# Luka140/paig_reproduction

Measured on AMD Instinct MI355X. Metric: video-seqs/sec (train step) spring_color B=100 @ 1/2/4/8 MI355X, higher is better.
Workload: dtype fp32; 1 GPU; spring_color PhysicsNet train step (get_batch gather+fwd+loss+bwd+allreduce+RMSprop), B=100/rank, 32x32x3, seq_len 50 (4 in / 6 pred / 40 extrap); global_batch=100, seq_len=50, parallelism=dp1, conv_math=split, split_graph=False, optimizer_in_graph=True, byte_targets=True, dataset_seqs=800

## Files before the change

include/paig_hip.h:

```cpp
#ifndef PAIG_HIP_H
#define PAIG_HIP_H
#include <stddef.h>

#ifdef __cplusplus
extern "C" {
#endif

#define PAIG_ABI_VERSION 12
const char* paig_last_error(void);
int paig_abi_version(void);
int paig_f16_range_status(int clear);

int paig_conv2d_fwd(const float* in, long long in_fs, int in_grp, long long in_gs, float* out, long long out_fs,
                    const float* aux, long long aux_fs, const float* w, const float* bias, int F, int Cin, int Cout,
                    int H, int W, int ks, int flags, void* stream);
#define PAIG_XMAX_SLOTS 2048
int paig_conv2d_fwd_ex(const float* in, long long in_fs, int in_grp, long long in_gs, float* out, long long out_fs,
                       const float* aux, long long aux_fs, const float* w, const float* bias, int F, int Cin,
                       int Cout, int H, int W, int ks, int flags, float* xmax, int xmax_n, void* stream);
int paig_conv2d_fwd_pw(const float* in, long long in_fs, int in_grp, long long in_gs, float* out, long long out_fs,
                       const float* aux, long long aux_fs, const float* w, const float* bias, int F, int Cin,
                       int Cout, int H, int W, int ks, int flags, float* xmax, int xmax_n, float* pool_out,
                       long long pool_fs, const void* wprep, void* stream);
int paig_conv2d_fwd_pwc(const float* in, long long in_fs, int in_grp, long long in_gs, float* out, long long out_fs,
                        const float* aux, long long aux_fs, const float* w, const float* bias, int F, int Cin,
                        int Cout, int H, int W, int ks, int flags, float* xmax, int xmax_n, float* pool_out,
                        long long pool_fs, unsigned char* pool_code, long long pool_code_fs, const void* wprep,
                        void* stream);
long long paig_conv_wprep_size(int cin, int cout, int ks);
int paig_conv_wprep(int n, const float* const* w, const int* cin, const int* cout, const int* ks, const int* dg,
                    void* const* out, void* stream);
int paig_conv_wprep_defer(int n, const float* const* w, const int* cin, const int* cout, const int* ks, const int* dg,
                          void* const* out, void* stream);
int paig_conv_wprep_flush(void* stream);
int paig_debug_fwd_block_cap(int cap);
int paig_conv2d_mfma_supported(int what, int Cin, int Cout, int H, int W, int ks, int flags);
int paig_conv2d_wgrad(const float* x, long long x_fs, int x_grp, long long x_gs, const float* dy, long long dy_fs,
                      float* slab, int nblk_max, int* nblk_out, int F, int Cin, int Cout, int H, int W, int ks,
                      int flags, void* stream);
int paig_conv2d_wgrad_ex(const float* x, long long x_fs, int x_grp, long long x_gs, const float* dy, long long dy_fs,
                         float* slab, int nblk_max, int* nblk_out, int F, int Cin, int Cout, int H, int W, int ks,
                         int flags, const float* xmax, int xmax_n, void* stream);
int paig_conv2d_bwd_supported(int Cin, int Cout, int H, int W, int ks, int flags);
int paig_conv2d_bwd(const float* x, long long x_fs, int x_grp, long long x_gs, const float* dy, long long dy_fs,
                    float* dx, long long dx_fs, const float* aux, long long aux_fs, const float* w, float* slab,
                    int nblk_max, int* nblk_out, int F, int Cin, int Cout, int H, int W, int ks, int flags,
                    const float* xmax, int xmax_n, const float* dpool, long long dpool_fs,
                    const unsigned char* pcode, long long pcode_fs, const void* wprep, void* stream);

size_t paig_unet_workspace(int net, int F, int H, int K, int math);
int paig_unet_fwd(int net, int F, int H, int K, int math, const float* x, long long x_fs, int x_grp, long long x_gs,
                  const float* const* w, const float* const* b, float* logits, void* ws, size_t ws_bytes,
                  void* stream);
int paig_unet_bwd(int net, int F, int H, int K, int math, const float* x, long long x_fs, int x_grp, long long x_gs,
                  const float* const* w, const float* logits, const float* dlogits, float* const* dwb, void* ws,
                  size_t ws_bytes, void* stream);
#define PAIG_UNET_HEAD_FUSED 1
#define PAIG_UNET_SEPARATE_BWD 2
#define PAIG_UNET_INFERENCE 4
#define PAIG_UNET_EXT_WPREP 8
#define PAIG_UNET_STANDALONE_UP 16
#define PAIG_UNET_STANDALONE_POOL 32
#define PAIG_PROBE_CONV_FWD 0
#define PAIG_PROBE_CONV_BWD 1
#define PAIG_PROBE_CONV_WGRAD 2
#define PAIG_PROBE_CONV_DGRAD 3
typedef void (*paig_unet_probe_fn)(void* ctx, int event, int op, int conv, int kind, int cin, int cout, int H,
                                   int flags);
size_t paig_unet_workspace_ex(int net, int F, int H, int K, int math, int flags);
long long paig_unet_buffer(int net, int F, int H, int K, int math, int flags, int which, int buf);
int paig_unet_query(int net, int K, int what);
int paig_unet_fwd_ex(int net, int F, int H, int K, int math, int flags, const float* x, long long x_fs, int x_grp,
                     long long x_gs, const float* const* w, const float* const* b, float* logits,
                     const void* const* wprep_fwd, const void* const* wprep_dg, void* ws, size_t ws_bytes,
                     paig_unet_probe_fn probe, void* probe_ctx, void* stream);
int paig_unet_bwd_ex(int net, int F, int H, int K, int math, int flags, const float* x, long long x_fs, int x_grp,
                     long long x_gs, const float* const* w, const float* logits, const float* dlogits,
                     float* const* dwb, int n_extra, const float* const* extra_src, const int* extra_nblk,
                     const int* extra_len, float* const* extra_dst, const void* const* wprep_dg, void* ws,
                     size_t ws_bytes, paig_unet_probe_fn probe, void* probe_ctx, void* stream);

int paig_conv2d_wgrad_pf(const float* x, long long x_fs, int x_grp, long long x_gs, const float* dy, long long dy_fs,
                         const float* dpool, long long dpool_fs, const unsigned char* pcode, long long pcode_fs,
                         float* slab, int nblk_max, int* nblk_out, int F, int Cin, int Cout, int H, int W, int ks,
                         int flags, const float* xmax, int xmax_n, void* stream);

int paig_maxpool2_fwd(const float* x, long long x_fs, float* y, long long y_fs, int F, int C, int H, int W,
                      void* stream);
int paig_maxpool2_fwd_codes(const float* x, long long x_fs, float* y, long long y_fs, unsigned char* code,
                            long long code_fs, int F, int C, int H, int W, void* stream);
int paig_maxpool2_bwd_relu(const float* x, long long x_fs, const float* dy, long long dy_fs, float* dx, long long dx_fs,
                           int F, int C, int H, int W, void* stream);
int paig_upsample2_fwd(const float* s, long long s_fs, float* u, long long u_fs, int F, int C, int Hs, int Ws, int Ho,
                       int Wo, void* stream);
int paig_upsample2_bwd(const float* du, long long du_fs, const float* s, long long s_fs, float* ds, long long ds_fs,
                       int F, int C, int Hs, int Ws, int Ho, int Wo, int relu_mask, void* stream);

int paig_mask_softmax_fwd(const float* logits, const float* x, long long x_fs, int x_grp, long long x_gs, float* masks,
                          float* objs, float* pobjs, int F, int K, int C, int H, int W, void* stream);
int paig_mask_softmax_bwd(const float* logits, const float* x, long long x_fs, int x_grp, long long x_gs,
                          const float* masks, const float* dobjs, float* dlogits, int F, int K, int C, int H, int W,
                          int flags, void* stream);
int paig_head_mask_blocks(int F, int H, int W);
int paig_head_mask_fwd(const float* x12, const float* w, const float* b, const float* x, long long x_fs, int x_grp,
                       long long x_gs, float* masks, float* objs, int F, int K, int H, int W, void* stream);
int paig_head_mask_bwd(const float* x12, const float* w, const float* b, const float* x, long long x_fs, int x_grp,
                       long long x_gs, const float* masks, const float* dobjs, float* dx12, float* slab, int F, int K,
                       int H, int W, void* stream);
int paig_head_mask_fwd_ex(const float* xl, const float* w, const float* b, const float* x, long long x_fs, int x_grp,
                          long long x_gs, float* masks, float* objs, float* pobjs, int F, int K, int CI, int H, int W,
                          int flags, void* stream);
int paig_head_mask_bwd_ex(const float* xl, const float* w, const float* b, const float* x, long long x_fs, int x_grp,
                          long long x_gs, const float* masks, const float* dobjs, float* dxl, float* slab, int F, int K,
                          int CI, int H, int W, int flags, void* stream);
int paig_pos_head_fwd(const float* h3, float* pos, int N, int K, float half, void* stream);
int paig_pos_head_bwd(const float* h3, const float* dpos, float* dh3, int N, int K, float half, void* stream);

size_t paig_gemm_workspace(int M, int N, int K);
int paig_gemm_defer_epilogue(int on);
int paig_gemm_flush(void* stream);
int paig_gemm(int ta, int tb, int M, int N, int K, float alpha, const float* A, long long lda, const float* B,
              long long ldb, float beta, float* C, long long ldc, const float* bias, int act, int auxm,
              const float* aux, long long ldaux, float* rowsum, float* ws, size_t ws_floats, void* stream);
int paig_gemm_ex(int ta, int tb, int M, int N, int K, float alpha, const float* A, long long lda, const float* B,
                 long long ldb, float beta, float* C, long long ldc, const float* bias, int act, int auxm,
                 const float* aux, long long ldaux, float* rowsum, float* ws, size_t ws_floats, int math,
                 void* stream);
size_t paig_gemm_parts_size(int M, int N, int K, int math);
int paig_gemm_parts(int ta, int tb, int M, int N, int K, const float* A, long long lda, const float* B,
                    long long ldb, float* part, size_t part_floats, int math, void* stream);
size_t paig_colsum_workspace(int M, int N);
int paig_colsum(const float* X, int M, int N, long long ld, float* out, int accumulate, float* ws, void* stream);
int paig_slab_reduce(const float* slab, int nblk, long long ld, int len, float* out, int accumulate, void* stream);
int paig_slab_reduce_multi(int ntask, const float* const* src, const int* nblk, const int* len, float* const* dst,
                           int accumulate, void* stream);
int paig_axpby(const float* x, float* y, long long n, float a, float b, void* stream);

int paig_vfn_fwd(const float* W1, const float* b1, const float* W2, const float* b2, float* hout, float* y,
                 float* ypost, int P, void* stream);
int paig_vfn_bwd_blocks(int P);
int paig_vfn_bwd(const float* d, const float* y, int sig, const float* h, const float* W2, float* dW1, float* db1,
                 float* dW2, float* db2, float* part, int P, void* stream);
int paig_vfn_fwd_multi(int n, const float* const* W1, const float* const* b1, const float* const* W2,
                       const float* const* b2, float* const* hout, float* const* y, float* const* ypost, const int* P,
                       void* stream);
int paig_vfn_bwd_multi(int n, const float* const* d, const float* const* y, const int* sig, const float* const* h,
                       const float* const* W2, float* const* dW1, float* const* db1, float* const* dW2,
                       float* const* db2, float* const* part, const int* P, void* stream);
int paig_vfn_bwd1_multi(int n, const float* const* d, const float* const* y, const int* sig, const float* const* h,
                        const float* const* W2, float* const* dW1, float* const* db1, float* const* dW2,
                        float* const* db2, float* const* part, const int* P, void* stream);

int paig_velmlp_fwd(const float* pos, int B, int Te, int K, int S, const float* W0, const float* b0, const float* W2,
                    const float* b2, const float* W4, const float* b4, float* X, float* h1, float* h2, float* vel,
                    void* stream);
int paig_velmlp_vfn_fwd(const float* pos, int B, int Te, int K, int S, const float* W0, const float* b0,
                        const float* W2, const float* b2, const float* W4, const float* b4, float* X, float* h1,
                        float* h2, float* vel, int n, const float* const* vW1, const float* const* vb1,
                        const float* const* vW2, const float* const* vb2, float* const* hout, float* const* y,
                        float* const* ypost, const int* P, void* stream);
int paig_velmlp_bwd_blocks(int rows);
int paig_velmlp_slab_len(int S);
int paig_velmlp_bwd(const float* dvel, const float* X, const float* h1, const float* h2, const float* W0,
                    const float* W2, const float* W4, float* dX, float* slab, int rows, int S, void* stream);

int paig_head_fwd(const float* h2, const float* W3, const float* b3, float* h3, float* pos, int F, int K, int IN,
                  float half, void* stream);
int paig_head_bwd_blocks(int rows);
int paig_head_bwd(const float* h2, const float* h3, const float* dpos, const float* W3, float* dh2, float* slab, int F,
                  int K, int IN, float half, void* stream);
int paig_head_bwd_vel(const float* h2, const float* h3, const float* dpos, const float* W3, float* dh2, float* slab,
                      int F, int K, int IN, float half, const float* dX, const float* dpos0, int B, int Te, int S,
                      int alt, void* stream);
int paig_head_bwd_vel_vfn2(const float* h2, const float* h3, const float* dpos, const float* W3, float* dh2,
                           float* slab, int F, int K, int IN, float half, const float* dX, const float* dpos0, int B,
                           int Te, int S, int alt, int n, const float* const* d, const float* const* y,
                           const int* sig, const float* const* h, const float* const* W2, float* const* dW1,
                           float* const* db1, float* const* dW2, float* const* db2, float* const* part, const int* P,
                           void* stream);

int paig_dense_tail_fwd(const float* part, int S, const float* b1, float* h1, const float* W2, float* W2t,
                        const float* b2, float* h2, const float* W3, const float* b3, float* h3, float* pos, int F,
                        int K, int IN, float half, void* stream);
int paig_head_l2_bwd_blocks(int rows);
int paig_head_l2_bwd(const float* h2, const float* h3, const float* dpos, const float* W3, float* dh2, float* slab,
                     int F, int K, int IN, float half, const float* dX, const float* dpos0, int B, int Te, int S,
                     int alt, const float* W2, const float* h1, float* dh1, int n, const float* const* d,
                     const float* const* y, const int* sig, const float* const* h, const float* const* vW2,
                     float* const* dW1, float* const* db1, float* const* dW2, float* const* db2, float* const* part,
                     const int* P, void* stream);

size_t paig_localiser_workspace(int F, int K, int n1, int IN, int math);
int paig_localiser_fwd(const float* x1, const float* W1, const float* b1, const float* W2, const float* b2,
                       const float* W3, const float* b3, float* h1, float* h2, float* h3, float* pos, int F, int K,
                       int n1, int IN, float half, int math, void* ws, size_t ws_bytes, void* stream);
int paig_localiser_bwd(const float* dpos, const float* x1, const float* h1, const float* h2, const float* h3,
                       const float* W1, const float* W2, const float* W3, float* dl1, float* dl2, float* dl3,
                       float* dx1, int F, int K, int n1, int IN, float half, int math, void* ws, size_t ws_bytes,
                       void* stream);
int paig_velmlp_rollout_fwd(int cell, const float* pos, int B, int Te, int K, int S, const float* W0, const float* b0,
                            const float* W2, const float* b2, const float* W4, const float* b4, float* X, float* h1,
                            float* h2, float* vel0, const float* dt, const double* p0, const double* p1, float* pvs,
                            int R, void* stream);
size_t paig_velmlp_rollout_bwd_workspace(int B, int K, int S);
int paig_velmlp_rollout_bwd(int cell, const float* pvs, const float* dpos_roll, const float* dpvs, const float* dt,
                            const double* p0, const double* p1, const float* X, const float* h1, const float* h2,
                            const float* W0, const float* W2, const float* W4, float* dpos, float* dmlp,
                            double* gparam0, double* gparam1, int B, int Te, int K, int S, int R, void* ws,
                            size_t ws_bytes, void* stream);

int paig_vel_pack(const float* pos, float* X, int B, int Te, int K, int S, int alt, void* stream);
int paig_vel_unpack_add(const float* dX, const float* dpos0, float* dpos, int B, int Te, int K, int S, int alt,
                        void* stream);

int paig_rollout_fwd(int cell, const float* pos0, long long pos0_ld, const float* vel0, const float* dt,
                     const double* p0, const double* p1, float* pvs, int B, int D, int R, void* stream);
int paig_rollout_bwd_blocks(int B);
int paig_rollout_bwd(int cell, const float* pvs, const float* dpos_roll, const float* dpvs, const float* dt,
                     const double* p0, const double* p1, float* dpos0, float* dvel0, double* part, double* gparam0,
                     double* gparam1, int accumulate, int B, int D, int R, void* stream);

int paig_decoder_fwd(const float* pos, long long pos_outer, long long pos_inner, int pos_grp, const float* tmpl,
                     const float* cont, const float* bg, float* out, long long out_fs, const float* tgt,
                     long long tgt_fs, int tgt_grp, long long tgt_gs, float* sse, int F, int K, int h, int H,
                     void* stream);
int paig_decoder_fwd_rollout(int cell, const float* pos0, long long pos0_ld, const float* vel0, const float* dt,
                             const double* p0, const double* p1, float* pvs, int B, int D, int R, const float* pos,
                             long long pos_outer, long long pos_inner, int pos_grp, const float* tmpl,
                             const float* cont, const float* bg, float* out, long long out_fs, const float* tgt,
                             long long tgt_fs, int tgt_grp, long long tgt_gs, float* sse, int F, int K, int h, int H,
                             void* stream);
int paig_decoder_fwd_t8(const float* pos, long long pos_outer, long long pos_inner, int pos_grp, const float* tmpl,
                        const float* cont, const float* bg, float* out, long long out_fs, const unsigned char* tgt,
                        const long long* tgt_idx, long long tgt_fs, int tgt_grp, long long tgt_gs, float* sse, int F,
                        int K, int h, int H, void* stream);
int paig_decoder_bwd_blocks(int F, int pos_grp, int live, int K, int h, int H);
size_t paig_decoder_slab_len(int K, int h, int H);
size_t paig_decoder_bwd_scratch(int F, int K, int h, int H);
int paig_decoder_bwd(const float* pos, long long pos_outer, long long pos_inner, int pos_grp, const float* tmpl,
                     const float* cont, const float* bg, const float* tgt, long long tgt_fs, int tgt_grp,
                     long long tgt_gs, const float* dsse, const float* dout, long long dout_fs, float* dpos,
                     float* slab, float* scratch, int F, int live, int K, int h, int H, void* stream);
int paig_decoder_bwd_ex(const float* pos, long long pos_outer, long long pos_inner, int pos_grp, const float* tmpl,
                        const float* cont, const float* bg, const float* tgt, const unsigned char* tgt8,
                        const long long* tgt_idx, long long tgt_fs, int tgt_grp, long long tgt_gs, const float* dsse,
                        int lw_mode, const float* dt, const float* de, const float* dr, float ae, int lB, int lTe,
                        int lR, int lpred, const float* dout, long long dout_fs, float* dpos, float* slab,
                        float* scratch, int F, int live, int K, int h, int H, void* stream);
int paig_decoder_bwd_t8(const float* pos, long long pos_outer, long long pos_inner, int pos_grp, const float* tmpl,
                        const float* cont, const float* bg, const unsigned char* tgt, const long long* tgt_idx,
                        long long tgt_fs, int tgt_grp, long long tgt_gs, const float* dsse, const float* dout,
                        long long dout_fs, float* dpos, float* slab, float* scratch, int F, int live, int K, int h,
                        int H, void* stream);

int paig_decoder_fwd_sigma(const float* pos, long long pos_outer, long long pos_inner, int pos_grp, const float* tmpl,
                           const float* cont, const float* bg, float* out, long long out_fs, const float* tgt,
                           long long tgt_fs, int tgt_grp, long long tgt_gs, float* sse, int F, int K, int h, int H,
                           double sigma, void* stream);
int paig_decoder_fwd_rollout_sigma(int cell, const float* pos0, long long pos0_ld, const float* vel0, const float* dt,
                                   const double* p0, const double* p1, float* pvs, int B, int D, int R,
                                   const float* pos, long long pos_outer, long long pos_inner, int pos_grp,
                                   const float* tmpl, const float* cont, const float* bg, float* out, long long out_fs,
                                   const float* tgt, long long tgt_fs, int tgt_grp, long long tgt_gs, float* sse, int F,
                                   int K, int h, int H, double sigma, void* stream);
int paig_decoder_fwd_t8_sigma(const float* pos, long long pos_outer, long long pos_inner, int pos_grp,
                              const float* tmpl, const float* cont, const float* bg, float* out, long long out_fs,
                              const unsigned char* tgt, const long long* tgt_idx, long long tgt_fs, int tgt_grp,
                              long long tgt_gs, float* sse, int F, int K, int h, int H, double sigma, void* stream);
int paig_decoder_bwd_blocks_sigma(int F, int pos_grp, int live, int K, int h, int H, double sigma);
size_t paig_decoder_bwd_scratch_sigma(int F, int K, int h, int H, double sigma);
int paig_decoder_bwd_ex_sigma(const float* pos, long long pos_outer, long long pos_inner, int pos_grp,
                              const float* tmpl, const float* cont, const float* bg, const float* tgt,
                              const unsigned char* tgt8, const long long* tgt_idx, long long tgt_fs, int tgt_grp,
                              long long tgt_gs, const float* dsse, int lw_mode, const float* dt, const float* de,
                              const float* dr, float ae, int lB, int lTe, int lR, int lpred, const float* dout,
                              long long dout_fs, float* dpos, float* slab, float* scratch, int F, int live, int K,
                              int h, int H, double sigma, void* stream);
int paig_decoder_parts_sigma(const float* pos, long long pos_inner, const float* tmpl, const float* cont,
                             const float* bg, float* contents, float* masks, int F, int K, int h, int H, double sigma,
                             void* stream);

int paig_sigma_from_u(const float* u, double* sigma_dev, void* stream);
int paig_sigma_grad(const double* dsig_a, int na, const double* dsig_b, int nb, const float* u, float* gu,
                    int accumulate, void* stream);
int paig_decoder_fwd_sigma_dev(const float* pos, long long pos_outer, long long pos_inner, int pos_grp,
                               const float* tmpl, const float* cont, const float* bg, float* out, long long out_fs,
                               const float* tgt, long long tgt_fs, int tgt_grp, long long tgt_gs, float* sse, int F,
                               int K, int h, int H, const double* sigma_dev, void* stream);
int paig_decoder_fwd_rollout_sigma_dev(int cell, const float* pos0, long long pos0_ld, const float* vel0,
                                       const float* dt, const double* p0, const double* p1, float* pvs, int B, int D,
                                       int R, const float* pos, long long pos_outer, long long pos_inner, int pos_grp,
                                       const float* tmpl, const float* cont, const float* bg, float* out,
                                       long long out_fs, const float* tgt, long long tgt_fs, int tgt_grp,
                                       long long tgt_gs, float* sse, int F, int K, int h, int H,
                                       const double* sigma_dev, void* stream);
int paig_decoder_fwd_t8_sigma_dev(const float* pos, long long pos_outer, long long pos_inner, int pos_grp,
                                  const float* tmpl, const float* cont, const float* bg, float* out, long long out_fs,
                                  const unsigned char* tgt, const long long* tgt_idx, long long tgt_fs, int tgt_grp,
                                  long long tgt_gs, float* sse, int F, int K, int h, int H, const double* sigma_dev,
                                  void* stream);
int paig_decoder_bwd_blocks_sigma_dev(int F, int K, int h, int H);
size_t paig_decoder_bwd_scratch_sigma_dev(int F, int K, int h, int H);
int paig_decoder_bwd_ex_sigma_dev(const float* pos, long long pos_outer, long long pos_inner, int pos_grp,
                                  const float* tmpl, const float* cont, const float* bg, const float* tgt,
                                  const unsigned char* tgt8, const long long* tgt_idx, long long tgt_fs, int tgt_grp,
                                  long long tgt_gs, const float* dsse, int lw_mode, const float* dt, const float* de,
                                  const float* dr, float ae, int lB, int lTe, int lR, int lpred, const float* dout,
                                  long long dout_fs, float* dpos, float* slab, float* scratch, int F, int live, int K,
                                  int h, int H, const double* sigma_dev, double* dsig, void* stream);
int paig_decoder_parts_sigma_dev(const float* pos, long long pos_inner, const float* tmpl, const float* cont,
                                 const float* bg, float* contents, float* masks, int F, int K, int h, int H,
                                 const double* sigma_dev, void* stream);

int paig_decoder_parts(const float* pos, long long pos_inner, const float* tmpl, const float* cont, const float* bg,
                       float* contents, float* masks, int F, int K, int h, int H, void* stream);
int paig_stn_fwd(const float* U, const float* theta, float* out, int N, int C, int Hi, int Wi, int Ho, int Wo,
                 void* stream);
int paig_stn_bwd(const float* U, const float* theta, const float* dout, float* dU, float* dtheta, int N, int C,
                 int Hi, int Wi, int Ho, int Wo, void* stream);
int paig_stn_fwd_f64(const float* U, const double* theta, float* out, int N, int C, int Hi, int Wi, int Ho, int Wo,
                     void* stream);
int paig_stn_bwd_f64(const float* U, const double* theta, const float* dout, float* dU, double* dtheta, int N, int C,
                     int Hi, int Wi, int Ho, int Wo, void* stream);
int paig_relu_mask(const float* y, float* d, long long n, void* stream);

int paig_loss_reduce(const float* sse_rec, const float* sse_roll, int B, int Te, int R, int pred, float ae,
                     float* pred_out, float* extrap_out, float* recons_out, void* stream);
int paig_loss_bwd(const float* dpred, const float* dext, const float* drec, float ae, float* wrec, float* wroll, int B,
                  int Te, int R, int pred, void* stream);
int paig_frame_sse(const float* a, long long a_fs, int a_grp, long long a_gs, const float* b, long long b_fs, int b_grp,
                   long long b_gs, float* sse, int F, int n, void* stream);
int paig_frame_sse_bwd(const float* a, long long a_fs, int a_grp, long long a_gs, const float* b, long long b_fs,
                       int b_grp, long long b_gs, const float* w, float* da, int F, int n, void* stream);

int paig_gather_u8_f32(const unsigned char* src, const long long* idx, float* out, int B, long long row, void* stream);
int paig_gather_u8_f32_ex(const unsigned char* src, const long long* idx, float* out, int B, long long row,
                          long long head, long long* idx_out, void* stream);

int paig_synth_integrate(int phys, const double* p0, const double* v0, long long m, int K, int T, int sub, double dt,
                         double size, double radius, double c0, double c1, double* pos, int* valid, void* stream);
int paig_synth_raster(const double* pos, const long long* rows, long long n, int T, int K, int size, double radius,
                      const float* bg, unsigned char* out, void* stream);
int paig_synth_raster_ex(const double* pos, const long long* rows, long long m, long long n, int T, int K, int size,
                         double radius, const float* bg, unsigned char* out, void* stream);
int paig_synth_draw(int phys, long long seed, long long stream_id, long long round, long long m, int K, int half,
                    double size, double radius, double c0, double c1, double vmax, double* p0, double* v0, double* u,
                    void* stream);
int paig_synth_background(long long seed, long long stream_id, long long round, long long n, int size, float* bg,
                          void* stream);
int paig_synth_compact(const int* valid, long long m, long long* rows, long long n, int* count, long long* totals,
                       void* stream);

int paig_rmsprop_f32(float* p, const float* g, float* sa, long long n, float lr, float alpha, float eps, void* stream);
int paig_rmsprop_mixed(float* p32, const float* g32, float* s32, long long n32, double* p64, const double* g64,
                       double* s64, long long n64, double lr, double alpha, double eps, void* stream);
int paig_rmsprop_f64(double* p, const double* g, double* sa, long long n, double lr, double alpha, double eps,
                     void* stream);
int paig_adam_f32(float* p, const float* g, float* m, float* v, long long n, float lr, float b1, float b2, float eps,
                  float bc1, float bc2sqrt, void* stream);
int paig_adam_f64(double* p, const double* g, double* m, double* v, long long n, double lr, double b1, double b2,
                  double eps, double bc1, double bc2sqrt, void* stream);
int paig_sgd_f32(float* p, const float* g, float* buf, long long n, float lr, float mom, int first, void* stream);
int paig_sgd_f64(double* p, const double* g, double* buf, long long n, double lr, double mom, int first, void* stream);

#define PAIG_GN_COLS 5
#define PAIG_GN_GROUPS 8
#define PAIG_GN_NORM 0
#define PAIG_GN_COEF 1
#define PAIG_GN_NONFINITE 2
#define PAIG_GN_TOTAL_SQ 3
#define PAIG_GN_GROUP0 4
#define PAIG_GN_SQ0 12
#define PAIG_GN_MAX_SEGMENTS 4096
int paig_grad_norm_chunk(void);
size_t paig_grad_norm_scratch(long long nchunks);
int paig_grad_norm(const float* g32, long long n32, const double* g64, long long n64, const long long* seg, int nseg,
                   long long nchunks, const unsigned char* mask, double max_norm, double* stats, void* scratch,
                   size_t scratch_bytes, void* stream);
int paig_rmsprop_mixed_clip(float* p32, const float* g32, float* s32, long long n32, double* p64, const double* g64,
                            double* s64, long long n64, double lr, double lr64, double alpha, double eps,
                            const double* coef, void* stream);
int paig_adam_f32_clip(float* p, const float* g, float* m, float* v, long long n, float lr, float b1, float b2,
                       float eps, float bc1, float bc2sqrt, const double* coef, void* stream);
int paig_adam_f64_clip(double* p, const double* g, double* m, double* v, long long n, double lr, double b1, double b2,
                       double eps, double bc1, double bc2sqrt, const double* coef, void* stream);
int paig_sgd_f32_clip(float* p, const float* g, float* buf, long long n, float lr, float mom, int first,
                      const double* coef, void* stream);
int paig_sgd_f64_clip(double* p, const double* g, double* buf, long long n, double lr, double mom, int first,
                      const double* coef, void* stream);

#ifdef __cplusplus
}
#endif
#endif
```

paig_reproduction_amd/_lib.py:

```python
import ctypes
import os

import torch

_HERE = os.path.dirname(os.path.abspath(__file__))
LIB_PATH = os.path.join(_HERE, "libpaig_hip.so")
XMAX_SLOTS = 2048

AB_PATH = os.environ.get("PAIG_AB_LIB")
ABI_VERSION = 12

P = ctypes.c_void_p
I = ctypes.c_int
LL = ctypes.c_longlong
F32 = ctypes.c_float
F64 = ctypes.c_double
SZ = ctypes.c_size_t

SIGNATURES = {
    "paig_last_error": (ctypes.c_char_p, []),
    "paig_abi_version": (I, []),
    "paig_f16_range_status": (I, [I]),
    "paig_conv2d_fwd": (I, [P, LL, I, LL, P, LL, P, LL, P, P, I, I, I, I, I, I, I, P]),
    "paig_conv2d_wgrad": (I, [P, LL, I, LL, P, LL, P, I, P, I, I, I, I, I, I, I, P]),
    "paig_conv2d_fwd_ex": (I, [P, LL, I, LL, P, LL, P, LL, P, P, I, I, I, I, I, I, I, P, I, P]),
    "paig_conv2d_fwd_pw": (I, [P, LL, I, LL, P, LL, P, LL, P, P, I, I, I, I, I, I, I, P, I, P, LL, P, P]),
    "paig_conv_wprep_size": (LL, [I, I, I]),
    "paig_conv_wprep": (I, [I, P, P, P, P, P, P, P]),
    "paig_conv_wprep_defer": (I, [I, P, P, P, P, P, P, P]),
    "paig_conv_wprep_flush": (I, [P]),
    "paig_conv2d_wgrad_ex": (I, [P, LL, I, LL, P, LL, P, I, P, I, I, I, I, I, I, I, P, I, P]),
    "paig_conv2d_wgrad_pf": (I, [P, LL, I, LL, P, LL, P, LL, P, LL, P, I, P, I, I, I, I, I, I, I, P, I, P]),
    "paig_conv2d_mfma_supported": (I, [I, I, I, I, I, I, I]),
    "paig_debug_fwd_block_cap": (I, [I]),
    "paig_conv2d_bwd_supported": (I, [I, I, I, I, I, I]),
    "paig_conv2d_bwd": (I, [P, LL, I, LL, P, LL, P, LL, P, LL, P, P, I, P, I, I, I, I, I, I, I, P, I, P, LL, P, LL,
                            P, P]),
    "paig_conv2d_fwd_pwc": (I, [P, LL, I, LL, P, LL, P, LL, P, P, I, I, I, I, I, I, I, P, I, P, LL, P, LL, P, P]),
    "paig_gather_u8_f32": (I, [P, P, P, I, LL, P]),
    "paig_gather_u8_f32_ex": (I, [P, P, P, I, LL, LL, P, P]),
    "paig_velmlp_fwd": (I, [P, I, I, I, I, P, P, P, P, P, P, P, P, P, P, P]),
    "paig_velmlp_vfn_fwd": (I, [P, I, I, I, I, P, P, P, P, P, P, P, P, P, P, I, P, P, P, P, P, P, P, P, P]),
    "paig_velmlp_bwd_blocks": (I, [I]),
    "paig_velmlp_slab_len": (I, [I]),
    "paig_velmlp_bwd": (I, [P, P, P, P, P, P, P, P, P, I, I, P]),
    "paig_head_fwd": (I, [P, P, P, P, P, I, I, I, F32, P]),
    "paig_dense_tail_fwd": (I, [P, I, P, P, P, P, P, P, P, P, P, P, I, I, I, F32, P]),
    "paig_head_l2_bwd": (I, [P, P, P, P, P, P, I, I, I, F32, P, P, I, I, I, I, P, P, P, I, P, P, P, P, P, P, P, P, P,
                             P, P, P]),
    "paig_head_bwd_blocks": (I, [I]),
    "paig_head_l2_bwd_blocks": (I, [I]),
    "paig_head_bwd": (I, [P, P, P, P, P, P, I, I, I, F32, P]),
    "paig_head_bwd_vel": (I, [P, P, P, P, P, P, I, I, I, F32, P, P, I, I, I, I, P]),
    "paig_head_bwd_vel_vfn2": (I, [P, P, P, P, P, P, I, I, I, F32, P, P, I, I, I, I, I, P, P, P, P, P, P, P, P, P, P, P,
                                   P]),
    "paig_unet_workspace": (SZ, [I, I, I, I, I]),
    "paig_localiser_workspace": (SZ, [I, I, I, I, I]),
    "paig_localiser_fwd": (I, [P, P, P, P, P, P, P, P, P, P, P, I, I, I, I, F32, I, P, SZ, P]),
    "paig_localiser_bwd": (I, [P, P, P, P, P, P, P, P, P, P, P, P, I, I, I, I, F32, I, P, SZ, P]),
    "paig_velmlp_rollout_fwd": (I, [I, P, I, I, I, I, P, P, P, P, P, P, P, P, P, P, P, P, P, P, I, P]),
    "paig_velmlp_rollout_bwd_workspace": (SZ, [I, I, I]),
    "paig_velmlp_rollout_bwd": (I, [I, P, P, P, P, P, P, P, P, P, P, P, P, P, P, P, P, I, I, I, I, I, P, SZ, P]),
    "paig_unet_fwd": (I, [I, I, I, I, I, P, LL, I, LL, P, P, P, P, SZ, P]),
    "paig_unet_bwd": (I, [I, I, I, I, I, P, LL, I, LL, P, P, P, P, P, SZ, P]),
    "paig_unet_workspace_ex": (SZ, [I, I, I, I, I, I]),
    "paig_unet_buffer": (LL, [I, I, I, I, I, I, I, I]),
    "paig_unet_query": (I, [I, I, I]),
    "paig_unet_fwd_ex": (I, [I, I, I, I, I, I, P, LL, I, LL, P, P, P, P, P, P, SZ, P, P, P]),
    "paig_unet_bwd_ex": (I, [I, I, I, I, I, I, P, LL, I, LL, P, P, P, P, I, P, P, P, P, P, P, SZ, P, P, P]),
    "paig_maxpool2_fwd": (I, [P, LL, P, LL, I, I, I, I, P]),
    "paig_maxpool2_fwd_codes": (I, [P, LL, P, LL, P, LL, I, I, I, I, P]),
    "paig_maxpool2_bwd_relu": (I, [P, LL, P, LL, P, LL, I, I, I, I, P]),
    "paig_upsample2_fwd": (I, [P, LL, P, LL, I, I, I, I, I, I, P]),
    "paig_upsample2_bwd": (I, [P, LL, P, LL, P, LL, I, I, I, I, I, I, I, P]),
    "paig_mask_softmax_fwd": (I, [P, P, LL, I, LL, P, P, P, I, I, I, I, I, P]),
    "paig_mask_softmax_bwd": (I, [P, P, LL, I, LL, P, P, P, I, I, I, I, I, I, P]),
    "paig_head_mask_blocks": (I, [I, I, I]),
    "paig_head_mask_fwd": (I, [P, P, P, P, LL, I, LL, P, P, I, I, I, I, P]),
    "paig_head_mask_bwd": (I, [P, P, P, P, LL, I, LL, P, P, P, P, I, I, I, I, P]),
    "paig_head_mask_fwd_ex": (I, [P, P, P, P, LL, I, LL, P, P, P, I, I, I, I, I, I, P]),
    "paig_head_mask_bwd_ex": (I, [P, P, P, P, LL, I, LL, P, P, P, P, I, I, I, I, I, I, P]),
    "paig_pos_head_fwd": (I, [P, P, I, I, F32, P]),
    "paig_pos_head_bwd": (I, [P, P, P, I, I, F32, P]),
    "paig_gemm_workspace": (SZ, [I, I, I]),
    "paig_gemm_parts_size": (SZ, [I, I, I, I]),
    "paig_gemm_parts": (I, [I, I, I, I, I, P, LL, P, LL, P, SZ, I, P]),
    "paig_gemm_defer_epilogue": (I, [I]),
    "paig_gemm_flush": (I, [P]),
    "paig_gemm": (I, [I, I, I, I, I, F32, P, LL, P, LL, F32, P, LL, P, I, I, P, LL, P, P, SZ, P]),
    "paig_gemm_ex": (I, [I, I, I, I, I, F32, P, LL, P, LL, F32, P, LL, P, I, I, P, LL, P, P, SZ, I, P]),
    "paig_colsum_workspace": (SZ, [I, I]),
    "paig_colsum": (I, [P, I, I, LL, P, I, P, P]),
    "paig_slab_reduce": (I, [P, I, LL, I, P, I, P]),
    "paig_slab_reduce_multi": (I, [I, P, P, P, P, I, P]),
    "paig_axpby": (I, [P, P, LL, F32, F32, P]),
    "paig_vfn_fwd": (I, [P, P, P, P, P, P, P, I, P]),
    "paig_vfn_bwd_blocks": (I, [I]),
    "paig_vfn_bwd": (I, [P, P, I, P, P, P, P, P, P, P, I, P]),
    "paig_vfn_fwd_multi": (I, [I, P, P, P, P, P, P, P, P, P]),
    "paig_vfn_bwd_multi": (I, [I, P, P, P, P, P, P, P, P, P, P, P, P]),
    "paig_vfn_bwd1_multi": (I, [I, P, P, P, P, P, P, P, P, P, P, P, P]),
    "paig_vel_pack": (I, [P, P, I, I, I, I, I, P]),
    "paig_vel_unpack_add": (I, [P, P, P, I, I, I, I, I, P]),
    "paig_rollout_fwd": (I, [I, P, LL, P, P, P, P, P, I, I, I, P]),
    "paig_rollout_bwd_blocks": (I, [I]),
    "paig_rollout_bwd": (I, [I, P, P, P, P, P, P, P, P, P, P, P, I, I, I, I, P]),
    "paig_decoder_fwd": (I, [P, LL, LL, I, P, P, P, P, LL, P, LL, I, LL, P, I, I, I, I, P]),
    "paig_decoder_fwd_rollout": (I, [I, P, LL, P, P, P, P, P, I, I, I, P, LL, LL, I, P, P, P, P, LL, P, LL, I, LL, P, I, I,
                                      I, I, P]),
    "paig_decoder_fwd_t8": (I, [P, LL, LL, I, P, P, P, P, LL, P, P, LL, I, LL, P, I, I, I, I, P]),
    "paig_decoder_bwd_blocks": (I, [I, I, I, I, I, I]),
    "paig_decoder_slab_len": (SZ, [I, I, I]),
    "paig_decoder_bwd_scratch": (SZ, [I, I, I, I]),
    "paig_decoder_bwd": (I, [P, LL, LL, I, P, P, P, P, LL, I, LL, P, P, LL, P, P, P, I, I, I, I, I, P]),
    "paig_decoder_bwd_ex": (I, [P, LL, LL, I, P, P, P, P, P, P, LL, I, LL, P, I, P, P, P, F32, I, I, I, I, P, LL, P, P, P,
                                 I, I, I, I, I, P]),
    "paig_decoder_bwd_t8": (I, [P, LL, LL, I, P, P, P, P, P, LL, I, LL, P, P, LL, P, P, P, I, I, I, I, I, P]),
    "paig_decoder_parts": (I, [P, LL, P, P, P, P, P, I, I, I, I, P]),
    "paig_decoder_fwd_sigma": (I, [P, LL, LL, I, P, P, P, P, LL, P, LL, I, LL, P, I, I, I, I, F64, P]),
    "paig_decoder_fwd_rollout_sigma": (I, [I, P, LL, P, P, P, P, P, I, I, I, P, LL, LL, I, P, P, P, P, LL, P, LL, I, LL,
                                            P, I, I, I, I, F64, P]),
    "paig_decoder_fwd_t8_sigma": (I, [P, LL, LL, I, P, P, P, P, LL, P, P, LL, I, LL, P, I, I, I, I, F64, P]),
    "paig_decoder_bwd_blocks_sigma": (I, [I, I, I, I, I, I, F64]),
    "paig_decoder_bwd_scratch_sigma": (SZ, [I, I, I, I, F64]),
    "paig_decoder_bwd_ex_sigma": (I, [P, LL, LL, I, P, P, P, P, P, P, LL, I, LL, P, I, P, P, P, F32, I, I, I, I, P, LL, P,
                                       P, P, I, I, I, I, I, F64, P]),
    "paig_decoder_parts_sigma": (I, [P, LL, P, P, P, P, P, I, I, I, I, F64, P]),
    "paig_sigma_from_u": (I, [P, P, P]),
    "paig_sigma_grad": (I, [P, I, P, I, P, P, I, P]),
    "paig_decoder_fwd_sigma_dev": (I, [P, LL, LL, I, P, P, P, P, LL, P, LL, I, LL, P, I, I, I, I, P, P]),
    "paig_decoder_fwd_rollout_sigma_dev": (I, [I, P, LL, P, P, P, P, P, I, I, I, P, LL, LL, I, P, P, P, P, LL, P, LL, I,
                                                LL, P, I, I, I, I, P, P]),
    "paig_decoder_fwd_t8_sigma_dev": (I, [P, LL, LL, I, P, P, P, P, LL, P, P, LL, I, LL, P, I, I, I, I, P, P]),
    "paig_decoder_bwd_blocks_sigma_dev": (I, [I, I, I, I]),
    "paig_decoder_bwd_scratch_sigma_dev": (SZ, [I, I, I, I]),
    "paig_decoder_bwd_ex_sigma_dev": (I, [P, LL, LL, I, P, P, P, P, P, P, LL, I, LL, P, I, P, P, P, F32, I, I, I, I, P,
                                           LL, P, P, P, I, I, I, I, I, P, P, P]),
    "paig_decoder_parts_sigma_dev": (I, [P, LL, P, P, P, P, P, I, I, I, I, P, P]),
    "paig_stn_fwd": (I, [P, P, P, I, I, I, I, I, I, P]),
    "paig_stn_bwd": (I, [P, P, P, P, P, I, I, I, I, I, I, P]),
    "paig_stn_fwd_f64": (I, [P, P, P, I, I, I, I, I, I, P]),
    "paig_stn_bwd_f64": (I, [P, P, P, P, P, I, I, I, I, I, I, P]),
    "paig_relu_mask": (I, [P, P, LL, P]),
    "paig_loss_reduce": (I, [P, P, I, I, I, I, F32, P, P, P, P]),
    "paig_loss_bwd": (I, [P, P, P, F32, P, P, I, I, I, I, P]),
    "paig_frame_sse": (I, [P, LL, I, LL, P, LL, I, LL, P, I, I, P]),
    "paig_frame_sse_bwd": (I, [P, LL, I, LL, P, LL, I, LL, P, P, I, I, P]),
    "paig_synth_integrate": (I, [I, P, P, LL, I, I, I, F64, F64, F64, F64, F64, P, P, P]),
    "paig_synth_raster": (I, [P, P, LL, I, I, I, F64, P, P, P]),
    "paig_synth_raster_ex": (I, [P, P, LL, LL, I, I, I, F64, P, P, P]),
    "paig_synth_draw": (I, [I, LL, LL, LL, LL, I, I, F64, F64, F64, F64, F64, P, P, P, P]),
    "paig_synth_background": (I, [LL, LL, LL, LL, I, P, P]),
    "paig_synth_compact": (I, [P, LL, P, LL, P, P, P]),
    "paig_rmsprop_f32": (I, [P, P, P, LL, F32, F32, F32, P]),
    "paig_rmsprop_f64": (I, [P, P, P, LL, F64, F64, F64, P]),
    "paig_rmsprop_mixed": (I, [P, P, P, LL, P, P, P, LL, F64, F64, F64, P]),
    "paig_adam_f32": (I, [P, P, P, P, LL, F32, F32, F32, F32, F32, F32, P]),
    "paig_adam_f64": (I, [P, P, P, P, LL, F64, F64, F64, F64, F64, F64, P]),
    "paig_sgd_f32": (I, [P, P, P, LL, F32, F32, I, P]),
    "paig_sgd_f64": (I, [P, P, P, LL, F64, F64, I, P]),
    "paig_grad_norm_chunk": (I, []),
    "paig_grad_norm_scratch": (SZ, [LL]),
    "paig_grad_norm": (I, [P, LL, P, LL, P, I, LL, P, F64, P, P, SZ, P]),
    "paig_rmsprop_mixed_clip": (I, [P, P, P, LL, P, P, P, LL, F64, F64, F64, F64, P, P]),
    "paig_adam_f32_clip": (I, [P, P, P, P, LL, F32, F32, F32, F32, F32, F32, P, P]),
    "paig_adam_f64_clip": (I, [P, P, P, P, LL, F64, F64, F64, F64, F64, F64, P, P]),
    "paig_sgd_f32_clip": (I, [P, P, P, LL, F32, F32, I, P, P]),
    "paig_sgd_f64_clip": (I, [P, P, P, LL, F64, F64, I, P, P]),
}

GN_COLS, GN_GROUPS = 5, 8
GN_NORM, GN_COEF, GN_NONFINITE, GN_TOTAL_SQ, GN_GROUP0, GN_SQ0 = 0, 1, 2, 3, 4, 12

_QUERY = {"paig_last_error", "paig_abi_version", "paig_f16_range_status", "paig_conv2d_mfma_supported",
          "paig_debug_fwd_block_cap",
          "paig_conv2d_bwd_supported", "paig_velmlp_bwd_blocks",
          "paig_velmlp_slab_len", "paig_head_bwd_blocks", "paig_head_l2_bwd_blocks", "paig_head_mask_blocks", "paig_conv_wprep_size", "paig_gemm_workspace", "paig_colsum_workspace",
          "paig_gemm_parts_size", "paig_gemm_parts", "paig_unet_workspace", "paig_unet_workspace_ex",
          "paig_unet_buffer", "paig_unet_query", "paig_localiser_workspace",
          "paig_velmlp_rollout_bwd_workspace",
          "paig_vfn_bwd_blocks", "paig_rollout_bwd_blocks", "paig_decoder_bwd_blocks", "paig_decoder_slab_len",
          "paig_decoder_bwd_scratch", "paig_decoder_bwd_blocks_sigma", "paig_decoder_bwd_scratch_sigma",
          "paig_decoder_bwd_blocks_sigma_dev", "paig_decoder_bwd_scratch_sigma_dev",
          "paig_grad_norm_chunk", "paig_grad_norm_scratch"}


class PaigError(RuntimeError):
    pass


class _Lib:
    def __init__(self, path=LIB_PATH):
        if not os.path.exists(path):
            raise PaigError(f"libpaig_hip.so not built at {path}: run `make -C paig_reproduction_amd/csrc` "
                            "(or __graft_entry__.build()); there is no CPU fallback")
        self.path = path
        self.dll = ctypes.CDLL(path)
        self.dll.paig_abi_version.restype = I
        self.dll.paig_abi_version.argtypes = []
        ver = self.dll.paig_abi_version()
        if ver != ABI_VERSION:
            raise PaigError(f"{path}: C ABI version {ver}, this binding is version {ABI_VERSION}")
        self.fns = {}
        for name, (rt, args) in SIGNATURES.items():
            if path != LIB_PATH and not hasattr(self.dll, name):
                continue
            f = getattr(self.dll, name)
            f.restype = rt
            f.argtypes = args
            self.fns[name] = f

    def __getattr__(self, name):
        fns = self.__dict__.get("fns")
        if fns is None or name not in fns:
            raise AttributeError(name)
        f = fns[name]
        if name in _QUERY:
            return f

        def call(*a):
            rc = f(*a)
            if rc != 0:
                msg = self.fns["paig_last_error"]().decode(errors="replace")
                raise PaigError(f"{name} failed (rc={rc}): {msg}")
            return rc

        call.__name__ = name
        return call


_lib = None


def lib():
    global _lib
    if _lib is None:
        _lib = _Lib(AB_PATH or LIB_PATH)
    return _lib


def ptr(t):
    return None if t is None else t.data_ptr()


def stream_handle(device=None):
    return torch.cuda.current_stream(device).cuda_stream


def require_device(t):
    if not (torch.is_tensor(t) and t.is_cuda):
        raise PaigError("paig_reproduction_amd runs only on a HIP device (MI355X); got a "
                        f"{'CPU' if torch.is_tensor(t) else type(t).__name__} tensor. There is no CPU fallback.")
```

paig_reproduction_amd/csrc/conv_bwd.hip:

```cpp
#include "split_common.h"

#include <stdlib.h>

#ifndef PAIG_BWD_MINW
#define PAIG_BWD_MINW 0
#endif
#ifndef PAIG_BWD_UPS2
#define PAIG_BWD_UPS2 1
#endif
#ifndef PAIG_BWD_TPX_C10
#define PAIG_BWD_TPX_C10 0
#define PAIG_BWD_MINW_C10 0
#endif
#ifndef PAIG_BWD_PSD_EVEN_C10
#define PAIG_BWD_PSD_EVEN_C10 0
#endif
#ifndef PAIG_BWD_AUXP
#define PAIG_BWD_AUXP 1
#endif

#ifdef PAIG_BWD_STAMPS
__device__ unsigned long long paig_bwd_stamps[4096][4][13];
#define PAIG_BSTAMP(k)                                      \
  do {                                                      \
    const unsigned long long t_ = __builtin_amdgcn_s_memtime(); \
    st_acc[k] += t_ - st_last;                              \
    st_last = t_;                                           \
  } while (0)
#else
#define PAIG_BSTAMP(k) \
  do {                 \
  } while (0)
#endif

namespace {

constexpr int sbwd_lds(int CIN, int COUT, int H, int W, bool UPS, int PM, int tpx) {
  const int FPT = H * W <= tpx ? tpx / (H * W) : 1, RT = H * W <= tpx ? H : rows_fit(H, W, tpx);
  const bool pe = PAIG_BWD_PSD_EVEN_C10 && UPS && CIN == 16 && COUT == 16 && H == 32;
  const int ROWS = RT + 2, ROWSD = ROWS + (UPS ? 2 : 0), CCD = rup(COUT, 8) / 8,
            PSD = CCD % 2 == 0 && !pe ? CCD + 1 : CCD;
  const int RPD = W == 8 ? to_mod16((W + 2) * PSD, 8) : (W + 2) * PSD;
  const int IMGD = (FPT * ROWSD * RPD + 2) * 8, WIMG = ceil_div(9 * CCD, 4) * ceil_div(CIN, 16) * 64 * 8;
  const int XIMG = rup(CIN, 4) / 4 * rup(FPT * ROWS * (W + 4) * 4 + 80, 128) * 2 * (PM == 2 ? 1 : 2);
  const int UPB = UPS ? CIN * (rup(FPT * (RT + 2) * W, 64) + 4) * 4 : 0;
  const int XREG = XIMG > UPB ? XIMG : UPB;
  return (IMGD + WIMG) * 2 * (PM == 2 ? 1 : 2) + XREG + (UPS ? up_window_floats(CIN, FPT, RT, W) * 4 : 0);
}
constexpr int sbwd_tpx(int CIN, int COUT, int H, int W, bool UPS, int PM) {
  if (PAIG_BWD_TPX_C10 && UPS && CIN == 16 && COUT == 16 && H == 32) return PAIG_BWD_TPX_C10;
  for (int pass = 0; pass < 2; ++pass)
    for (int t = 256; t >= 64; t /= 2) {
      const int rt = H * W <= t ? H : rows_fit(H, W, t);
      if (UPS && (rt % 2 != 0 || H * W < t)) continue;
      if (sbwd_lds(CIN, COUT, H, W, UPS, PM, t) <= (pass == 0 ? LDS_MAX / 2 : LDS_MAX)) return t;
    }
  return 64;
}

constexpr int sbwd_minw(int CIN, int COUT, int H, int PM, bool PF) {
  if (PAIG_BWD_MINW_C10 && CIN == 16 && COUT == 16 && H == 32) return PAIG_BWD_MINW_C10;
  if (CIN == 8 && COUT == 8 && H == 32) return PF || PAIG_BWD_AUXP == 2 ? 3 : 4;
  if (PM == 2 && CIN == 8 && COUT == 16 && H == 16) return 3;
  if (PM == 2 && CIN == 24 && COUT == 8 && H == 32) return 3;
  if (CIN == 8 && COUT == 8 && H == 36) return PF ? 2 : 3;
  if (CIN == 8 && COUT == 16 && H == 18) return PM == 2 ? 4 : 3;
  if (CIN == 16 && COUT == 16 && H == 18) return PF && PM != 2 ? 2 : 3;
  return 2;
}

constexpr bool sbwd_auxp(int CIN, int COUT, int H, int PM, bool UPS, bool PF) {
  if (PAIG_BWD_AUXP == 2) return true;
  if (CIN == 8 && COUT == 8 && (H == 32 || H == 36) && !PF) return false;
  if (CIN == 24 && COUT == 8 && (H == 36 || PM == 2)) return false;
  if (UPS && H == 36) return false;
  if (PM == 0) return !(PF && CIN == 16 && COUT == 16 && H == 16);
  return !((UPS && CIN == 32 && H == 16) || (CIN == 8 && COUT == 16 && H == 16));
}

constexpr bool sbwd_hoist(int CIN, int COUT, int H, int PM, bool PF) {
  if (PF && PM == 0 && ((CIN == 8 && H == 32) || H == 64)) return false;
  if (PF && PM == 2 && H == 18) return false;
  if (CIN == 24 && H == 36 && PM == 0) return false;
  if (H == 18 && ((CIN == 8 && PM == 2) || (CIN == 16 && COUT == 16 && PM == 0))) return false;
  return true;
}

template <int CIN, int COUT, int H, int W, int KS, bool UPS, int PM, bool PF = false>
struct SBwdCfg {
  static constexpr int KK = KS * KS, PADL = KS / 2;
  static constexpr int NIMG = PM == 2 ? 1 : 2;
  static constexpr int TPX = sbwd_tpx(CIN, COUT, H, W, UPS, PM);
  static constexpr int FPT = H * W <= TPX ? TPX / (H * W) : 1;
  static constexpr int RT = H * W <= TPX ? H : rows_fit(H, W, TPX);
  static constexpr int TPXV = FPT * RT * W;
  static constexpr int ROWS = RT + KS - 1;
  static constexpr int EXT = UPS ? 1 : 0;
  static constexpr int RTD = RT + 2 * EXT, ROWSD = ROWS + 2 * EXT;
  static constexpr int TPXD = FPT * RTD * W;
  static constexpr int CCD = rup(COUT, 8) / 8;
  static constexpr bool PSDE = PAIG_BWD_PSD_EVEN_C10 && UPS && CIN == 16 && COUT == 16 && H == 32;
  static constexpr int PSD = CCD % 2 == 0 && !PSDE ? CCD + 1 : CCD;
  static constexpr int TWPX = W + 2 * PADL;
  static constexpr int RPD = W == 8 ? to_mod16(TWPX * PSD, 8) : TWPX * PSD;
  static constexpr int ZSLOT = FPT * ROWSD * RPD;
  static constexpr int IMGD = (ZSLOT + 2) * 8;
  static constexpr int KC = KK * CCD, NS = ceil_div(KC, 4);
  static constexpr int NTD = ceil_div(CIN, 16);
  static constexpr int NMT = ceil_div(TPXD, 16), MW = ceil_div(NMT, 4);
  static constexpr int WIMG = NS * NTD * 64 * 8;
  static constexpr int CQ = rup(CIN, 4) / 4, NQ = KK * CQ, NTX = ceil_div(NQ, 4);
  static constexpr int OFFX = PADL > 0 ? 2 : 0, TWX = W + 2 * OFFX;
  static constexpr int XPL = rup(FPT * ROWS * TWX * 4 + 80, 128);
  static constexpr int XIMG = CQ * XPL;
  static constexpr int MT = ceil_div(COUT, 16), NTW = ceil_div(NTX, 4);
  static constexpr bool BAL = !(PM == 2 && (CIN == 24 || (UPS && CIN == 32) || H == 36 || H == 18)) && !(H == 36 && !UPS && !PF);
  static constexpr int NTF = BAL ? NTX / 4 : ceil_div(NTX, 4), NTR = BAL ? NTX % 4 : 0;
  static constexpr int KB = ceil_div(TPXV, 32);
  static constexpr int NCOL = CIN * KK, SLAB = COUT * NCOL + COUT;
  static constexpr int UPX = W % 2 == 0 ? 2 : 1, W2 = W / UPX;
  static constexpr int NID = FPT * ROWSD * W2 * CCD, NLD = ceil_div(NID, 256);
  static constexpr int NIX = FPT * ROWS * W2 * CQ, NLX = ceil_div(NIX, 256);
  static constexpr int UPW = up_window_floats(CIN, FPT, RT, W);
  static constexpr int UPB = UPS ? CIN * (rup(FPT * (RT + 2) * W, 64) + 4) * 4 : 0;
  static constexpr int XREG = XIMG * 2 * NIMG > UPB ? XIMG * 2 * NIMG : UPB;
  static constexpr int LDS = (IMGD + WIMG) * 2 * NIMG + XREG + (UPS ? UPW * 4 : 0);
  static constexpr bool VEC4 = W % 4 == 0;
  static constexpr bool HOIST = sbwd_hoist(CIN, COUT, H, PM, PF);
  static constexpr bool XPIPE = !UPS && NLX * 8 <= 32;
  static constexpr int LDSB = LDS_MAX / (LDS > (NLD * 256 * 8 + 256) * 4 ? LDS : (NLD * 256 * 8 + 256) * 4);
  static constexpr int MW0 = PAIG_BWD_MINW > 0 ? PAIG_BWD_MINW : sbwd_minw(CIN, COUT, H, PM, PF);
  static constexpr int MINW = MW0 < LDSB ? MW0 : LDSB;
  static_assert(H % RT == 0, "RT divides H");
  static_assert(KS == 3, "3x3 layers (the 1x1 heads are fused elsewhere)");
  static_assert(COUT % 8 == 0 && CIN % 4 == 0, "staging units of 8 dY / 4 X channels");
  static_assert(!UPS || (FPT == 1 && RT % 2 == 0 && W % 2 == 0), "fused upsample: whole even row blocks of one frame");
  static_assert(!PF || (!UPS && UPX == 2 && COUT % 8 == 0 && H % 2 == 0), "pool fold: even widths, 8-channel chunks");
  static constexpr int UPP = rup(TPXD, 64) + 4;
  static_assert(!UPS || CIN * UPP * 4 <= XREG, "fused upsample: dX tile does not fit the X region");
  static constexpr int WSU = W / 2, IKU = WSU % 4 == 0 ? 4 : (WSU % 2 == 0 ? 2 : 1), WQU = WSU / IKU;
  static constexpr int NOU = UPS ? CIN * (RT / 2) * WQU : 0, NOI = NOU > 0 ? ceil_div(NOU, 256) : 1;
  static constexpr bool AUXP =
      PAIG_BWD_AUXP && (UPS || (VEC4 && MW * NTD <= 8)) && sbwd_auxp(CIN, COUT, H, PM, UPS, PF);
};

template <int CIN, int COUT, int H, int W, int KS, bool UPS, int PM, bool PF>
__global__ void __launch_bounds__(256, (SBwdCfg<CIN, COUT, H, W, KS, UPS, PM, PF>::MINW))
conv_bwd_split_k(FView x, FView dy, FViewW dx, FView aux, const float* __restrict__ w, int flags,
                 float* __restrict__ slab, int F, int ntiles, XMax xm, const s16x8* __restrict__ wp, FView dpool,
                 const unsigned char* __restrict__ pcode, long long pcode_fs) {
  using C = SBwdCfg<CIN, COUT, H, W, KS, UPS, PM, PF>;
  constexpr int KK = C::KK, PADL = C::PADL, RT = C::RT, FPT = C::FPT, ROWS = C::ROWS, TPXV = C::TPXV;
  constexpr int EXT = C::EXT, RTD = C::RTD, ROWSD = C::ROWSD, TPXD = C::TPXD;
  constexpr int CCD = C::CCD, PSD = C::PSD, RPD = C::RPD, KC = C::KC, NS = C::NS, NTD = C::NTD, MW = C::MW;
  constexpr int CQ = C::CQ, NQ = C::NQ, NTX = C::NTX, OFFX = C::OFFX, TWX = C::TWX, XPL = C::XPL;
  constexpr int MT = C::MT, NTF = C::NTF, NTR = C::NTR, KB = C::KB, NCOL = C::NCOL, UPX = C::UPX, W2 = C::W2;
  constexpr int NF1 = NTF > 0 ? NTF : 1, NR1 = NTR > 0 ? NTR : 1;
  constexpr int NID = C::NID, NLD = C::NLD, NIX = C::NIX, NLX = C::NLX;
  constexpr long long HW = (long long)H * W;
  constexpr long long XPLANE = UPS ? (long long)(H / 2) * (W / 2) : HW;
  constexpr int NRB = H / RT;
  extern __shared__ __attribute__((aligned(16))) short lds16[];
  short* Dh = lds16;
  short* Dl = Dh + (C::NIMG == 2 ? C::IMGD : 0);
  short* Wh = lds16 + C::NIMG * C::IMGD;
  short* Wl = Wh + (C::NIMG == 2 ? C::WIMG : 0);
  short* Xh = lds16 + C::NIMG * (C::IMGD + C::WIMG);
  short* Xl = Xh + (C::NIMG == 2 ? C::XIMG : 0);
  float* Sl = reinterpret_cast<float*>(reinterpret_cast<char*>(Xh) + C::XREG);
  const int tid = threadIdx.x, lane = tid & 63, wv = tid >> 6, g = lane >> 4;
  __shared__ float smax[4];
#ifdef PAIG_BWD_STAMPS
  unsigned long long st_acc[12] = {0, 0, 0, 0, 0, 0, 0, 0, 0, 0, 0, 0}, st_last = __builtin_amdgcn_s_memtime(), st_n = 0;
#endif

  auto xplane = [](int cq) { return cq * XPL + ((cq & 1) ? 16 : 0) + ((cq & 2) ? 64 : 0); };
  for (int i = tid; i < FPT * ROWSD * 2 * PADL * CCD; i += 256) {
    const int cc = i % CCD, hc = (i / CCD) % (2 * PADL), r = i / (CCD * 2 * PADL);
    const int xc = hc < PADL ? hc : W + hc;
    const int o = (r * RPD + xc * PSD + cc) * 8;
    *reinterpret_cast<s16x8*>(Dh + o) = s16x8{0, 0, 0, 0, 0, 0, 0, 0};
    if (PM != 2) *reinterpret_cast<s16x8*>(Dl + o) = s16x8{0, 0, 0, 0, 0, 0, 0, 0};
  }
  if (tid < 2) {
    *reinterpret_cast<s16x8*>(Dh + (C::ZSLOT + tid) * 8) = s16x8{0, 0, 0, 0, 0, 0, 0, 0};
    if (PM != 2) *reinterpret_cast<s16x8*>(Dl + (C::ZSLOT + tid) * 8) = s16x8{0, 0, 0, 0, 0, 0, 0, 0};
  }
  auto zero_xhalo = [&]() {
    for (int i = tid; i < FPT * ROWS * 2 * OFFX * CQ; i += 256) {
      const int cq = i % CQ, hc = (i / CQ) % (2 * OFFX), r = i / (CQ * 2 * OFFX);
      const int xc = hc < OFFX ? hc : W + hc;
      *reinterpret_cast<s16x4*>(Xh + xplane(cq) + (r * TWX + xc) * 4) = s16x4{0, 0, 0, 0};
      if (PM != 2) *reinterpret_cast<s16x4*>(Xl + xplane(cq) + (r * TWX + xc) * 4) = s16x4{0, 0, 0, 0};
    }
  };
  zero_xhalo();

  int ecx = PAIG_A_EXP, ecd = PM == 0 && PAIG_SCALE_MODE < 2 ? 100 : 0;
  float xsc = 1.f, dsc = __builtin_amdgcn_ldexpf(1.f, ecd);
  float rmax = 0.f;
  int ewn[NTD];
#pragma unroll
  for (int nt = 0; nt < NTD; ++nt) ewn[nt] = 0;

  auto wval = [&](int idx, int j) {
    const int ln = idx & 63, snt = idx >> 6, nt = snt % NTD, s = snt / NTD;
    const int kc = 4 * s + (ln >> 4), ci = nt * 16 + (ln & 15);
    float v = 0.f;
    if (kc < KC && ci < CIN) {
      const int tap = kc / CCD, co = (kc % CCD) * 8 + j;
      if (co < COUT) v = w[(co * CIN + ci) * KK + (KK - 1 - tap)];
    }
    return v;
  };
  __shared__ int sew[PM == 0 ? NTD * 16 : 1];
  if (PM == 0 && wp != nullptr) {
    const int* hdr = reinterpret_cast<const int*>(wp);
    constexpr int HDR = NTD * 16 * 4 / 16;
#pragma unroll
    for (int nt = 0; nt < NTD; ++nt) ewn[nt] = hdr[nt * 16 + (lane & 15)];
    const s16x8* img = wp + HDR;
    constexpr int WLO = NS * NTD * 64;
    for (int idx = tid; idx < NS * NTD * 64; idx += 256) {
      *reinterpret_cast<s16x8*>(Wh + idx * 8) = img[idx];
      *reinterpret_cast<s16x8*>(Wl + idx * 8) = img[WLO + idx];
    }
  } else {
    if constexpr (PM == 0) {
      for (int i = tid; i < NTD * 16; i += 256) sew[i] = 0;
      __syncthreads();
      float pm[NTD];
#pragma unroll
      for (int nt = 0; nt < NTD; ++nt) pm[nt] = 0.f;
      for (int idx = tid; idx < NS * NTD * 64; idx += 256) {
        const int nt = (idx >> 6) % NTD;
#pragma unroll
        for (int j = 0; j < 8; ++j) pm[nt] = fmaxf(pm[nt], fabsf(wval(idx, j)));
      }
#pragma unroll
      for (int nt = 0; nt < NTD; ++nt) atomicMax(&sew[nt * 16 + (tid & 15)], __builtin_bit_cast(int, pm[nt]));
      __syncthreads();
      for (int i = tid; i < NTD * 16; i += 256) sew[i] = f16_scale_exp_v(__builtin_bit_cast(float, sew[i]));
      __syncthreads();
#pragma unroll
      for (int nt = 0; nt < NTD; ++nt) ewn[nt] = sew[nt * 16 + (lane & 15)];
    }
    for (int idx = tid; idx < NS * NTD * 64; idx += 256) {
      const int cl = ((idx >> 6) % NTD) * 16 + (idx & 15);
      const int e = PM == 0 ? sew[cl] : 0;
      s16x8 vh, vl;
#pragma unroll
      for (int j = 0; j < 8; ++j) {
        short h, l;
        float rm = 0.f;
        split<PM>(__builtin_amdgcn_ldexpf(wval(idx, j), e), h, l, rm);
        vh[j] = h;
        vl[j] = l;
      }
      *reinterpret_cast<s16x8*>(Wh + idx * 8) = vh;
      if (PM != 2) *reinterpret_cast<s16x8*>(Wl + idx * 8) = vl;
    }
  }

  int pbase[MW];
#pragma unroll
  for (int mt = 0; mt < MW; ++mt) {
    int pix = (wv * MW + mt) * 16 + (lane & 15);
    if (pix >= TPXD) pix = 0;
    const int fi = pix / (RTD * W), rem = pix % (RTD * W);
    pbase[mt] = (fi * ROWSD + rem / W) * RPD + (rem % W) * PSD;
  }
  int soff[NS];
#pragma unroll
  for (int s = 0; s < NS; ++s) {
    int kc = 4 * s + g;
    if (kc >= KC) kc = 0;
    const int tap = kc / CCD, cc = kc % CCD;
    soff[s] = (tap / KS) * RPD + (tap % KS) * PSD + cc;
  }
  const int qq = (lane >> 2) & 3, pl = lane & 3;
  auto colt_of = [&](int nt) {
    int cq = nt * 4 + pl;
    if (cq >= NQ) cq = 0;
    const int tap = cq / CQ, ciq = cq % CQ;
    return xplane(ciq) + ((tap / KS) * TWX + tap % KS) * 4;
  };
  int colt[NF1], coltr[NR1];
#pragma unroll
  for (int jn = 0; jn < NTF; ++jn) colt[jn] = colt_of(wv + jn * 4);
#pragma unroll
  for (int t = 0; t < NTR; ++t) coltr[t] = colt_of(NTF * 4 + t);
  auto dslot = [&](int j) {
    if (TPXV % 32 != 0 && j >= TPXV) return C::ZSLOT;
    const int fi = j / (RT * W), rem = j % (RT * W);
    return (fi * ROWSD + rem / W + PADL + EXT) * RPD + (rem % W + PADL) * PSD;
  };
  auto xpos = [&](int j) {
    if (TPXV % 32 != 0 && j >= TPXV) j = 0;
    const int fi = j / (RT * W), rem = j % (RT * W);
    return ((fi * ROWS + rem / W) * TWX + rem % W + (OFFX - PADL)) * 4;
  };

  f32x4 accw[MT][NF1], accr[MT][NR1];
#pragma unroll
  for (int m = 0; m < MT; ++m) {
#pragma unroll
    for (int j = 0; j < NF1; ++j) accw[m][j] = f32x4{0.f, 0.f, 0.f, 0.f};
#pragma unroll
    for (int t = 0; t < NR1; ++t) accr[m][t] = f32x4{0.f, 0.f, 0.f, 0.f};
  }
  float bacc[NLD][8];
#pragma unroll
  for (int l = 0; l < NLD; ++l)
#pragma unroll
    for (int c = 0; c < 8; ++c) bacc[l][c] = 0.f;

  float2 pd[NLD][8];
  float2 px[C::XPIPE ? NLX : 1][4];
  float dpv[PF ? NLD : 1][8];
  uint2 pcv[PF ? NLD : 1];
  constexpr int HP = H / 2, WP = W / 2;
  using UP = UpStage<UPS ? CIN : 1, H, W, FPT, RT>;
  UP up;
  auto row_ok = [&](int gy) { return (unsigned)gy < (unsigned)H; };
  auto d_unit = [&](int i, int& vo, int& row, int& so) {
    const int xp = UPX * (i % W2), r = (i / W2) % ROWSD, cc = (i / (W2 * ROWSD)) % CCD, fi = i / (W2 * ROWSD * CCD);
#ifdef PAIG_BWD_NOLOAD
    const bool in = false;
#else
    const bool in = i < NID;
#endif
    row = in ? r - PADL - EXT : -(1 << 20);
    vo = (fi * (int)dy.fs + cc * 8 * (int)HW + (r - PADL - EXT) * W + xp) * 4;
    if (NRB == 1 && !row_ok(row)) vo = BUF_OOR;
    so = ((fi * ROWSD + r) * RPD + (xp + PADL) * PSD + cc) * 8;
  };
  constexpr int NLH = C::HOIST ? NLD : 1;
  int dvo[NLH], drow[NLH], dso[NLH];
  if constexpr (C::HOIST) {
#pragma unroll
    for (int l = 0; l < NLD; ++l) d_unit(tid + l * 256, dvo[l], drow[l], dso[l]);
  }
  auto d_get = [&](int l, int& vo, int& row, int& so) {
    if constexpr (C::HOIST) {
      vo = dvo[l];
      row = drow[l];
      so = dso[l];
    } else {
      d_unit(opaque(tid) + l * 256, vo, row, so);
    }
  };
  auto pf_unit = [&](int i, int& po, int& co) {
    const int xp = UPX * (i % W2), cc = (i / (W2 * ROWSD)) % CCD, fi = i / (W2 * ROWSD * CCD);
    po = (fi * (int)dpool.fs + cc * 8 * (HP * WP) + (xp >> 1)) * 4;
    co = fi * (int)pcode_fs + (cc * (HP * WP) + (xp >> 1)) * 8;
  };
  auto x_unit = [&](int i, int& vo, int& row, int& so) {
    const int xp = UPX * (i % W2), r = (i / W2) % ROWS, cq = (i / (W2 * ROWS)) % CQ, fi = i / (W2 * ROWS * CQ);
    row = i < NIX ? r - PADL : -(1 << 20);
    vo = (fi * (int)x.fs + cq * 4 * (int)XPLANE + (r - PADL) * W + xp) * 4;
    if (NRB == 1 && !row_ok(row)) vo = BUF_OOR;
    so = xplane(cq) + ((fi * ROWS + r) * TWX + xp + OFFX) * 4;
  };
  constexpr int NXH = C::XPIPE && C::HOIST ? NLX : 1;
  int xvo[NXH], xrow[NXH], xso[NXH];
  if constexpr (C::XPIPE && C::HOIST) {
#pragma unroll
    for (int l = 0; l < NLX; ++l) x_unit(tid + l * 256, xvo[l], xrow[l], xso[l]);
  }
  auto x_get = [&](int l, int& vo, int& row, int& so) {
    if constexpr (C::HOIST) {
      vo = xvo[l];
      row = xrow[l];
      so = xso[l];
    } else {
      x_unit(opaque(tid) + l * 256, vo, row, so);
    }
  };
  int uvo[UPS ? UP::NLS : 1], urow[UPS ? UP::NLS : 1];
  if constexpr (UPS) {
#pragma unroll
    for (int l = 0; l < UP::NLS; ++l) UP::unit(tid + l * 256, (int)x.fs, uvo[l], urow[l]);
  }
  auto tile_nf = [&](int f0) {
    const int n = F - f0;
    return n < FPT ? n : FPT;
  };
  auto tile_vo = [&](int vo, int row, int y0) {
    if constexpr (NRB == 1) return vo;
    else return row_ok(y0 + row) ? vo + y0 * W * 4 : BUF_OOR;
  };
  auto load_d = [&](int t) {
    const int f0 = (t / NRB) * FPT, y0 = (t % NRB) * RT, nf = tile_nf(f0);
    const brsrc rd = tile_rsrc(dy.frame(f0), dy.fs, nf, COUT * (int)HW);
    brsrc rp, rc;
    if constexpr (PF) {
      rp = tile_rsrc(dpool.frame(f0), dpool.fs, nf, COUT * HP * WP);
      rc = tile_rsrc(pcode + (long long)f0 * pcode_fs, pcode_fs, nf, CCD * HP * WP * 8, 1);
    }
#pragma unroll
    for (int l = 0; l < NLD; ++l) {
      int vo0, row, so;
      d_get(l, vo0, row, so);
      const int vo = tile_vo(vo0, row, y0);
#pragma unroll
      for (int c = 0; c < 8; ++c) {
        pd[l][c] = UPX == 2 ? buf_ld2(rd, vo, c * (int)HW * 4) : make_float2(buf_ld1(rd, vo, c * (int)HW * 4), 0.f);
      }
      if constexpr (PF) {
        const int wr = ((y0 + row) >> 1) * WP;
        const bool ok = NRB == 1 ? vo != BUF_OOR : row_ok(y0 + row);
        int po, co;
        pf_unit(opaque(tid) + l * 256, po, co);
        const int vp = ok ? po + wr * 4 : BUF_OOR;
#pragma unroll
        for (int c = 0; c < 8; ++c) dpv[l][c] = buf_ld1(rp, vp, c * (HP * WP) * 4);
        const u32x2 cv = __builtin_amdgcn_raw_buffer_load_b64(rc, ok ? co + wr * 8 : BUF_OOR, 0, 0);
        pcv[l] = make_uint2(cv.x, cv.y);
      }
    }
  };
  auto fold = [&](int t) {
    const int y0 = (t % NRB) * RT;
#pragma unroll
    for (int l = 0; l < NLD; ++l) {
      int vo, row, so;
      d_get(l, vo, row, so);
      const int pr = ((y0 + row) & 1) * 2;
#pragma unroll
      for (int c = 0; c < 8; ++c) {
        const unsigned b = ((c < 4 ? pcv[l].x : pcv[l].y) >> (8 * (c & 3))) & 255u;
        const int am = (int)(b >> 4) & 3;
        const float vx = pd[l][c].x + (am == pr ? dpv[l][c] : 0.f);
        const float vy = pd[l][c].y + (am == pr + 1 ? dpv[l][c] : 0.f);
        pd[l][c].x = (b >> pr) & 1u ? vx : 0.f;
        pd[l][c].y = (b >> (pr + 1)) & 1u ? vy : 0.f;
      }
    }
  };
  auto x_rsrc = [&](int t) {
    const int f0 = (t / NRB) * FPT;
    return tile_rsrc(x.frame(f0), x.fs, tile_nf(f0), CIN * (int)XPLANE);
  };
  auto load_x = [&](brsrc rx, int t, int vo0, int row, float2* v) {
    const int vo = tile_vo(vo0, row, (t % NRB) * RT);
#pragma unroll
    for (int c = 0; c < 4; ++c)
      v[c] = UPX == 2 ? buf_ld2(rx, vo, c * (int)XPLANE * 4) : make_float2(buf_ld1(rx, vo, c * (int)XPLANE * 4), 0.f);
  };
  auto issue = [&](int t) {
    if (t >= ntiles) return;
    load_d(t);
    if constexpr (UPS) {
      up.issue(x_rsrc(t), (t % NRB) * RT, uvo, urow);
    } else if constexpr (C::XPIPE) {
      const brsrc rx = x_rsrc(t);
#pragma unroll
      for (int l = 0; l < NLX; ++l) {
        int vo, row, so;
        x_get(l, vo, row, so);
        load_x(rx, t, vo, row, px[l]);
      }
    }
  };
  auto put_d = [&](int o, const float2* v) {
    s16x8 h0, l0, h1, l1;
    if constexpr (PM == 0) {
      pf32x2 sv[8];
#pragma unroll
      for (int c = 0; c < 8; ++c) sv[c] = pf32x2{v[c].x, v[c].y} * dsc;
      u32x4 a0, b0, a1, b1;
#pragma unroll
      for (int k = 0; k < 4; ++k) {
        { const HiLo q_ = split_pk(sv[2 * k].x, sv[2 * k + 1].x); a0[k] = q_.h; b0[k] = q_.l; }
        { const HiLo q_ = split_pk(sv[2 * k].y, sv[2 * k + 1].y); a1[k] = q_.h; b1[k] = q_.l; }
      }
      h0 = __builtin_bit_cast(s16x8, a0);
      l0 = __builtin_bit_cast(s16x8, b0);
      h1 = __builtin_bit_cast(s16x8, a1);
      l1 = __builtin_bit_cast(s16x8, b1);
    } else {
      float rm = 0.f;
#pragma unroll
      for (int c = 0; c < 8; ++c) {
        short h, lo;
        split<PM>(v[c].x, h, lo, rm);
        h0[c] = h;
        l0[c] = lo;
        split<PM>(v[c].y, h, lo, rm);
        h1[c] = h;
        l1[c] = lo;
      }
    }
    *reinterpret_cast<s16x8*>(Dh + o) = h0;
    if (PM != 2) *reinterpret_cast<s16x8*>(Dl + o) = l0;
    if constexpr (UPX == 2) {
      *reinterpret_cast<s16x8*>(Dh + o + PSD * 8) = h1;
      if (PM != 2) *reinterpret_cast<s16x8*>(Dl + o + PSD * 8) = l1;
    }
  };
  auto put_x_at = [&](int o, const float2* v) {
    s16x8 hv, lv;
    if constexpr (PM == 0) {
      pf32x2 sv[4];
#pragma unroll
      for (int c = 0; c < 4; ++c) {
        sv[c] = pf32x2{v[c].x, v[c].y} * xsc;
        rmax = amax2(rmax, sv[c].x, sv[c].y);
      }
      u32x4 a, b;
      { const HiLo q_ = split_pk(sv[0].x, sv[1].x); a[0] = q_.h; b[0] = q_.l; }
      { const HiLo q_ = split_pk(sv[2].x, sv[3].x); a[1] = q_.h; b[1] = q_.l; }
      { const HiLo q_ = split_pk(sv[0].y, sv[1].y); a[2] = q_.h; b[2] = q_.l; }
      { const HiLo q_ = split_pk(sv[2].y, sv[3].y); a[3] = q_.h; b[3] = q_.l; }
      hv = __builtin_bit_cast(s16x8, a);
      lv = __builtin_bit_cast(s16x8, b);
    } else {
#pragma unroll
      for (int c = 0; c < 4; ++c) {
        short h, lo;
        split<PM>(v[c].x, h, lo, rmax);
        hv[c] = h;
        lv[c] = lo;
        split<PM>(v[c].y, h, lo, rmax);
        hv[4 + c] = h;
        lv[4 + c] = lo;
      }
    }
    if constexpr (UPX == 2) {
      *reinterpret_cast<s16x8*>(Xh + o) = hv;
      if (PM != 2) *reinterpret_cast<s16x8*>(Xl + o) = lv;
    } else {
      *reinterpret_cast<s16x4*>(Xh + o) = s16x4{hv[0], hv[1], hv[2], hv[3]};
      if (PM != 2) *reinterpret_cast<s16x4*>(Xl + o) = s16x4{lv[0], lv[1], lv[2], lv[3]};
    }
  };
  auto put_x = [&](int i, const float2* v) {
    const int xp = UPX * (i % W2), r = (i / W2) % ROWS, cq = (i / (W2 * ROWS)) % CQ, fi = i / (W2 * ROWS * CQ);
    put_x_at(xplane(cq) + ((fi * ROWS + r) * TWX + xp + OFFX) * 4, v);
  };
  auto tile_max = [&]() {
    float m = 0.f;
#pragma unroll
    for (int l = 0; l < NLD; ++l)
#pragma unroll
      for (int c = 0; c < 8; ++c) m = amax2(m, pd[l][c].x, pd[l][c].y);
    m = wave_max_u(m);
    if (lane == 0) smax[wv] = m;
  };
  auto commit = [&](int t) {
    if constexpr (PM == 0 && PAIG_SCALE_MODE < 2) {
      const int te = f16_scale_exp(fmaxf(fmaxf(smax[0], smax[1]), fmaxf(smax[2], smax[3])));
      const int td = te < ecd + 64 ? te : ecd + 64;
      if (td != ecd) {
#pragma unroll
        for (int m = 0; m < MT; ++m)
#pragma unroll
          for (int r = 0; r < 4; ++r) {
#pragma unroll
            for (int j = 0; j < NF1; ++j) accw[m][j][r] = __builtin_amdgcn_ldexpf(accw[m][j][r], td - ecd);
#pragma unroll
            for (int t = 0; t < NR1; ++t) accr[m][t][r] = __builtin_amdgcn_ldexpf(accr[m][t][r], td - ecd);
          }
        ecd = td;
        dsc = __builtin_amdgcn_ldexpf(1.f, ecd);
      }
    }
    const int f0 = (t / NRB) * FPT;
#pragma unroll
    for (int l = 0; l < NLD; ++l) {
      const int i = tid + l * 256;
      if (NID % 256 != 0 && i >= NID) break;
      int vo, row, so;
      d_get(l, vo, row, so);
      put_d(so, pd[l]);
      if ((unsigned)row < (unsigned)RT) {
#pragma unroll
        for (int c = 0; c < 8; ++c) bacc[l][c] += pd[l][c].x + pd[l][c].y;
      }
    }
    PAIG_BSTAMP(8);
    if constexpr (UPS) {
      const int y0 = (t % NRB) * RT;
      up.commit(Sl, tid);
      zero_xhalo();
      PAIG_BSTAMP(9);
      __syncthreads();
      PAIG_BSTAMP(10);
      if constexpr (W % 4 == 0 && ROWS % 2 == 0 && PAIG_BWD_UPS2 && PM == 0 && H != 36) {
        constexpr int W4 = W / 4, RP2 = ROWS / 2;
#pragma unroll 1
        for (int i = tid; i < CQ * RP2 * W4; i += 256) {
          const int q = i % W4, rp = (i / W4) % RP2, cq = i / (W4 * RP2);
          const int gy = y0 + 2 * rp - PADL;
          const bool ok0 = f0 < F && gy >= 0 && gy < H, ok1 = f0 < F && gy + 1 >= 0 && gy + 1 < H;
          f32x4 o0[4], o1[4];
#pragma unroll
          for (int c = 0; c < 4; ++c) {
            if (cq * 4 + c < CIN) {
              UP::row4x2(Sl, 0, cq * 4 + c, gy, y0, q, ok0, ok1, o0[c], o1[c]);
            } else {
              o0[c] = f32x4{0.f, 0.f, 0.f, 0.f};
              o1[c] = o0[c];
            }
          }
#pragma unroll
          for (int h2 = 0; h2 < 2; ++h2) {
            const int ia = (cq * ROWS + 2 * rp + h2) * W2 + 2 * q;
            const f32x4* o = h2 ? o1 : o0;
            float2 v[4];
#pragma unroll
            for (int c = 0; c < 4; ++c) v[c] = make_float2(o[c][0], o[c][1]);
            put_x(ia, v);
#pragma unroll
            for (int c = 0; c < 4; ++c) v[c] = make_float2(o[c][2], o[c][3]);
            put_x(ia + 1, v);
          }
        }
        PAIG_BSTAMP(11);
      } else if constexpr (W % 4 == 0) {
        constexpr int W4 = W / 4;
#pragma unroll 1
        for (int i = tid; i < NIX / 2; i += 256) {
#ifdef PAIG_BWD_NOUPS
          if (i >= 0) break;
#endif
          const int q = i % W4, r = (i / W4) % ROWS, cq = (i / (W4 * ROWS)) % CQ;
          const int gy = y0 + r - PADL;
          const bool ok = f0 < F && gy >= 0 && gy < H;
          f32x4 o[4];
#pragma unroll
          for (int c = 0; c < 4; ++c)
            o[c] = (ok && cq * 4 + c < CIN) ? UP::row4(Sl, 0, cq * 4 + c, gy, y0, q) : f32x4{0.f, 0.f, 0.f, 0.f};
          const int ia = (cq * ROWS + r) * W2 + 2 * q;
          float2 v[4];
#pragma unroll
          for (int c = 0; c < 4; ++c) v[c] = make_float2(o[c][0], o[c][1]);
          put_x(ia, v);
#pragma unroll
          for (int c = 0; c < 4; ++c) v[c] = make_float2(o[c][2], o[c][3]);
          put_x(ia + 1, v);
        }
        PAIG_BSTAMP(11);
      } else {
#pragma unroll 1
        for (int i = tid; i < NIX; i += 256) {
          const int xp = UPX * (i % W2), r = (i / W2) % ROWS, cq = (i / (W2 * ROWS)) % CQ;
          const int gy = y0 + r - PADL;
          const bool ok = f0 < F && gy >= 0 && gy < H;
          float2 v[4];
#pragma unroll
          for (int c = 0; c < 4; ++c)
            v[c] = (ok && cq * 4 + c < CIN)
                       ? make_float2(UP::px1(Sl, 0, cq * 4 + c, gy, y0, xp), UP::px1(Sl, 0, cq * 4 + c, gy, y0, xp + 1))
                       : make_float2(0.f, 0.f);
          put_x(i, v);
        }
      }
    } else if constexpr (C::XPIPE) {
#pragma unroll
      for (int l = 0; l < NLX; ++l) {
        const int i = tid + l * 256;
        if (NIX % 256 != 0 && i >= NIX) break;
        int vo, row, so;
        x_get(l, vo, row, so);
        put_x_at(so, px[l]);
      }
    } else {
      const brsrc rx = x_rsrc(t);
#pragma unroll 1
      for (int i = tid; i < NIX; i += 256) {
        float2 v[4];
        int vo, row, so;
        x_unit(i, vo, row, so);
        load_x(rx, t, vo, row, v);
        put_x_at(so, v);
      }
    }
  };

  int avo[C::AUXP ? (UPS ? C::NOI : MW) : 1];
  if constexpr (C::AUXP && UPS) {
#pragma unroll
    for (int k = 0; k < C::NOI; ++k) {
      const int o = tid + 256 * k;
      const int q = o % C::WQU, sr = (o / C::WQU) % (RT / 2), ci = o / (C::WQU * (RT / 2));
      avo[k] = o < C::NOU ? ((ci * (H / 2) + sr) * C::WSU + C::IKU * q) * 4 : BUF_OOR;
    }
  } else if constexpr (C::AUXP) {
#pragma unroll
    for (int mt = 0; mt < MW; ++mt) {
      const int pix = (wv * MW + mt) * 16 + (lane >> 4) * 4;
      const int fi = pix / (RT * W), rem = pix % (RT * W);
      avo[mt] = pix < TPXV ? (fi * (int)aux.fs + (lane & 15) * (int)HW + rem) * 4 : BUF_OOR;
    }
  }

  int lt = blockIdx.x;
  auto tile_of =[&](int l) { return l < ntiles ? xcd_tile(l, ntiles) : ntiles; };
  issue(tile_of(lt));
  if (PM == 0 && xm.p) {
    float m = 0.f;
    for (int i = tid * 4; i < xm.n; i += 1024) {
      const f32x4 v = *reinterpret_cast<const f32x4*>(xm.p + i);
      m = fmaxf(m, fmaxf(fmaxf(v[0], v[1]), fmaxf(v[2], v[3])));
    }
    m = wave_max_u(m);
    if (lane == 0) smax[wv] = m;
    __syncthreads();
    m = fmaxf(fmaxf(smax[0], smax[1]), fmaxf(smax[2], smax[3]));
    if (m > 0.f) ecx = f16_scale_exp(m);
    __syncthreads();
  }
  if constexpr (PM == 0) xsc = __builtin_amdgcn_ldexpf(1.f, ecx);
  else ecx = 0;

  PAIG_BSTAMP(0);
  for (; lt < ntiles; lt += gridDim.x) {
    const int tile = xcd_tile(lt, ntiles);
    const int f0 = (tile / NRB) * FPT, y0 = (tile % NRB) * RT;
    if constexpr (PF) fold(tile);
    if constexpr (PM == 0 && PAIG_SCALE_MODE < 2) tile_max();
    __syncthreads();
    PAIG_BSTAMP(1);
    commit(tile);
    __syncthreads();
    PAIG_BSTAMP(2);
    typedef float fIKU __attribute__((ext_vector_type(C::IKU)));
    f32x4 auxv[C::AUXP && !UPS ? MW : 1][C::AUXP && !UPS ? NTD : 1];
    fIKU auxu[C::AUXP && UPS ? C::NOI : 1];
    if constexpr (C::AUXP) {
      if (flags & 2) {
        const brsrc ra = tile_rsrc(aux.frame(f0), aux.fs, tile_nf(f0), CIN * (int)XPLANE);
        if constexpr (UPS) {
#pragma unroll
          for (int k = 0; k < C::NOI; ++k) {
            const int so = (y0 / 2) * C::WSU * 4;
            if constexpr (C::IKU == 4) auxu[k] = buf_ld4(ra, avo[k], so);
            else if constexpr (C::IKU == 2) auxu[k] = __builtin_bit_cast(fIKU, buf_ld2(ra, avo[k], so));
            else auxu[k] = __builtin_bit_cast(fIKU, buf_ld1(ra, avo[k], so));
          }
        } else {
#pragma unroll
          for (int nt = 0; nt < NTD; ++nt) {
            const bool cok = CIN % 16 == 0 || nt * 16 + (lane & 15) < CIN;
#pragma unroll
            for (int mt = 0; mt < MW; ++mt)
              auxv[mt][nt] = buf_ld4(ra, cok ? avo[mt] : BUF_OOR, (nt * 16 * (int)HW + y0 * W) * 4);
          }
        }
      }
    }
    issue(tile_of(lt + gridDim.x));
    PAIG_BSTAMP(3);

#pragma unroll 2
    for (int kb = 0; kb < KB; ++kb) {
      const int p0 = kb * 32;
      s16x8 ah[MT], al[MT];
      const int d0 = dslot(p0 + 8 * g + qq), d1 = dslot(p0 + 8 * g + 4 + qq);
#pragma unroll
      for (int m = 0; m < MT; ++m) {
        const int co = 2 * m + (pl >> 1), hoff = (pl & 1) * 4;
        const int a0 = (d0 + co) * 8 + hoff, a1 = (d1 + co) * 8 + hoff;
        ah[m] = __builtin_shufflevector(tr_read(Dh + a0), tr_read(Dh + a1), 0, 1, 2, 3, 4, 5, 6, 7);
        al[m] = PM != 2 ? __builtin_shufflevector(tr_read(Dl + a0), tr_read(Dl + a1), 0, 1, 2, 3, 4, 5, 6, 7) : ah[m];
      }
      const int r0 = xpos(p0 + 8 * g + qq), r1 = xpos(p0 + 8 * g + 4 + qq);
      auto ntile = [&](int ct, f32x4* acc) __attribute__((always_inline)) {
        const s16x8 bh = __builtin_shufflevector(tr_read(Xh + r0 + ct), tr_read(Xh + r1 + ct), 0, 1, 2, 3, 4, 5, 6, 7);
        const s16x8 bl =
            PM != 2 ? __builtin_shufflevector(tr_read(Xl + r0 + ct), tr_read(Xl + r1 + ct), 0, 1, 2, 3, 4, 5, 6, 7) : bh;
#pragma unroll
        for (int m = 0; m < MT; ++m) acc[m] = mma3<PM>(ah[m], al[m], bh, bl, acc[m]);
      };
#pragma unroll
      for (int jn = 0; jn < NTF; ++jn) {
        if (!C::BAL && wv + jn * 4 >= NTX) continue;
        f32x4 a[MT];
#pragma unroll
        for (int m = 0; m < MT; ++m) a[m] = accw[m][jn];
        ntile(colt[jn], a);
#pragma unroll
        for (int m = 0; m < MT; ++m) accw[m][jn] = a[m];
      }
      if (NTR > 0 && (kb & 3) == wv) {
#pragma unroll
        for (int t = 0; t < NTR; ++t) {
          f32x4 a[MT];
#pragma unroll
          for (int m = 0; m < MT; ++m) a[m] = accr[m][t];
          ntile(coltr[t], a);
#pragma unroll
          for (int m = 0; m < MT; ++m) accr[m][t] = a[m];
        }
      }
    }

    PAIG_BSTAMP(4);
    f32x4 accd[MW][NTD];
#pragma unroll
    for (int mt = 0; mt < MW; ++mt)
#pragma unroll
      for (int nt = 0; nt < NTD; ++nt) accd[mt][nt] = f32x4{0.f, 0.f, 0.f, 0.f};
#pragma unroll
    for (int s = 0; s < NS; ++s) {
      s16x8 bh[NTD], bl[NTD];
#pragma unroll
      for (int nt = 0; nt < NTD; ++nt) {
        const int o = ((s * NTD + nt) * 64 + lane) * 8;
        bh[nt] = *reinterpret_cast<const s16x8*>(Wh + o);
        bl[nt] = PM != 2 ? *reinterpret_cast<const s16x8*>(Wl + o) : bh[nt];
      }
#pragma unroll
      for (int mt = 0; mt < MW; ++mt) {
        const int o = (pbase[mt] + soff[s]) * 8;
        const s16x8 ah = *reinterpret_cast<const s16x8*>(Dh + o);
        const s16x8 al = PM != 2 ? *reinterpret_cast<const s16x8*>(Dl + o) : ah;
#pragma unroll
        for (int nt = 0; nt < NTD; ++nt) accd[mt][nt] = mma3<PM>(ah, al, bh[nt], bl[nt], accd[mt][nt]);
      }
    }
    PAIG_BSTAMP(5);
    if constexpr (UPS) {
      float* U = reinterpret_cast<float*>(Xh);
      __syncthreads();
#pragma unroll
      for (int nt = 0; nt < NTD; ++nt) {
        const int ci = nt * 16 + (lane & 15);
        if (ci >= CIN) continue;
        const float tinv = PM == 0 ? __builtin_amdgcn_ldexpf(1.f, -(ecd + ewn[nt])) : 1.f;
#pragma unroll
        for (int mt = 0; mt < MW; ++mt) {
          const int pix = (wv * MW + mt) * 16 + (lane >> 4) * 4;
          if (pix < TPXD) *reinterpret_cast<f32x4*>(U + ci * C::UPP + pix) = accd[mt][nt] * tinv;
        }
      }
      __syncthreads();
      constexpr int HS = H / 2, WS = W / 2, IK = C::IKU, WQ = C::WQU;
      constexpr int NO = C::NOU;
      static_assert(WS % IK == 0, "IK-pixel source items");
      typedef fIKU fIK;
      auto item = [&](int o, const fIK& mp) __attribute__((always_inline)) {
        const int q = o % WQ, sr = (o / WQ) % (RT / 2), ci = o / (WQ * (RT / 2));
        const int sy = y0 / 2 + sr;
        float wy[4];
        wy[0] = sy >= 1 ? 0.25f : 0.f;
        wy[1] = sy == 0 ? 1.f : 0.75f;
        wy[2] = sy == HS - 1 ? 1.f : 0.75f;
        wy[3] = sy <= HS - 2 ? 0.25f : 0.f;
        fIK acc;
#pragma unroll
        for (int k = 0; k < IK; ++k) acc[k] = 0.f;
#pragma unroll
        for (int a = 0; a < 4; ++a) {
          if (wy[a] == 0.f) continue;
          const float* rp = U + ci * C::UPP + (2 * sr + a) * W + 2 * IK * q;
          float c[2 * IK + 2];
          c[0] = q > 0 ? rp[-1] : 0.f;
          c[2 * IK + 1] = q < WQ - 1 ? rp[2 * IK] : 0.f;
          if constexpr (IK == 1) {
            c[1] = rp[0];
            c[2] = rp[1];
          } else {
#pragma unroll
            for (int h = 0; h < IK / 2; ++h) {
              const f32x4 m = *reinterpret_cast<const f32x4*>(rp + 4 * h);
#pragma unroll
              for (int e = 0; e < 4; ++e) c[1 + 4 * h + e] = m[e];
            }
          }
          fIK row;
#pragma unroll
          for (int k = 0; k < IK; ++k) {
            const int sx = IK * q + k;
            float wx[4];
            wx[0] = sx >= 1 ? 0.25f : 0.f;
            wx[1] = sx == 0 ? 1.f : 0.75f;
            wx[2] = sx == WS - 1 ? 1.f : 0.75f;
            wx[3] = sx <= WS - 2 ? 0.25f : 0.f;
            float v = 0.f;
#pragma unroll
            for (int b = 0; b < 4; ++b)
              if (wx[b] != 0.f) v = fmaf(wx[b], c[2 * k + b], v);
            row[k] = v;
          }
#pragma unroll
          for (int k = 0; k < IK; ++k) acc[k] = fmaf(wy[a], row[k], acc[k]);
        }
        if (f0 < F) {
          const long long off = ((long long)ci * HS + sy) * WS + IK * q;
          float* op = dx.frame(f0) + off;
          if (flags & 4) acc += *reinterpret_cast<const fIK*>(op);
          if (flags & 2) {
            fIK m;
            if constexpr (C::AUXP) m = mp;
            else m = *reinterpret_cast<const fIK*>(aux.frame(f0) + off);
#pragma unroll
            for (int k = 0; k < IK; ++k) acc[k] = m[k] > 0.f ? acc[k] : 0.f;
          }
          *reinterpret_cast<fIK*>(op) = acc;
        }
      };
      if constexpr (C::AUXP) {
#pragma unroll
        for (int it = 0; it < C::NOI; ++it) {
          const int o = tid + 256 * it;
          if (NO % 256 != 0 && o >= NO) break;
          item(o, auxu[it]);
        }
      } else {
        for (int o = tid; o < NO; o += 256) item(o, auxu[0]);
      }
    } else {
#pragma unroll
    for (int nt = 0; nt < NTD; ++nt) {
      const int ci = nt * 16 + (lane & 15);
      if (ci >= CIN) continue;
      const float tinv = PM == 0 ? __builtin_amdgcn_ldexpf(1.f, -(ecd + ewn[nt])) : 1.f;
#pragma unroll
      for (int mt = 0; mt < MW; ++mt) {
        const int pix = (wv * MW + mt) * 16 + (lane >> 4) * 4;
        if constexpr (C::VEC4) {
          if (pix >= TPXV) continue;
          const int fi = pix / (RT * W), rem = pix % (RT * W);
          const int y = y0 + rem / W, xx = rem % W, f = f0 + fi;
          if (f >= F) continue;
          float* op = dx.frame(f) + ci * HW + (long long)y * W + xx;
          f32x4 v = accd[mt][nt] * tinv;
          if (flags & 4) v += *reinterpret_cast<const f32x4*>(op);
          if (flags & 2) {
            f32x4 a;
            if constexpr (C::AUXP) a = auxv[mt][nt];
            else a = *reinterpret_cast<const f32x4*>(aux.frame(f) + ci * HW + (long long)y * W + xx);
#pragma unroll
            for (int r = 0; r < 4; ++r) v[r] = a[r] > 0.f ? v[r] : 0.f;
          }
          *reinterpret_cast<f32x4*>(op) = v;
        } else {
#pragma unroll
          for (int r = 0; r < 4; ++r) {
            const int pr = pix + r;
            if (pr >= TPXV) break;
            const int fi = pr / (RT * W), rem = pr % (RT * W);
            const int y = y0 + rem / W, xx = rem % W, f = f0 + fi;
            if (f >= F) continue;
            float* op = dx.frame(f) + ci * HW + (long long)y * W + xx;
            float v = accd[mt][nt][r] * tinv;
            if (flags & 4) v += *op;
            if (flags & 2) v = aux.frame(f)[ci * HW + (long long)y * W + xx] > 0.f ? v : 0.f;
            *op = v;
          }
        }
      }
    }
    }
    PAIG_BSTAMP(6);
#ifdef PAIG_BWD_STAMPS
    ++st_n;
#endif
  }

  float* s = slab + (long long)blockIdx.x * C::SLAB;
  auto put_w = [&](int m, int nt, const f32x4& acc) __attribute__((always_inline)) {
    const int col = nt * 16 + (lane & 15), cq = col >> 2;
    const int tap = cq / CQ, ci = (cq % CQ) * 4 + (col & 3);
#pragma unroll
    for (int r = 0; r < 4; ++r) {
      const int co = m * 16 + (lane >> 4) * 4 + r;
      float v = acc[r];
      if constexpr (PM == 0) v = __builtin_amdgcn_ldexpf(v, -(ecx + ecd));
      if (co < COUT && cq < NQ && ci < CIN) s[co * NCOL + ci * KK + tap] = v;
    }
  };
#pragma unroll
  for (int m = 0; m < MT; ++m)
#pragma unroll
    for (int j = 0; j < NTF; ++j)
      if (wv + j * 4 < NTX) put_w(m, wv + j * 4, accw[m][j]);
  if constexpr (NTR > 0) {
    f32x4* Rt = reinterpret_cast<f32x4*>(lds16);
    __syncthreads();
#pragma unroll
    for (int m = 0; m < MT; ++m)
#pragma unroll
      for (int t = 0; t < NTR; ++t) Rt[((wv * MT + m) * NTR + t) * 64 + lane] = accr[m][t];
    __syncthreads();
    for (int u = wv; u < MT * NTR; u += 4) {
      f32x4 v = Rt[u * 64 + lane];
#pragma unroll
      for (int w = 1; w < 4; ++w) v += Rt[(w * MT * NTR + u) * 64 + lane];
      put_w(u / NTR, NTF * 4 + u % NTR, v);
    }
  }
  __syncthreads();
  float* Rb = reinterpret_cast<float*>(lds16);
  constexpr int NP = 256 / COUT, NU = FPT * ROWSD * W2;
  float* Rp = Rb + NLD * 256 * 8;
#pragma unroll
  for (int l = 0; l < NLD; ++l)
#pragma unroll
    for (int c = 0; c < 8; ++c) Rb[(l * 256 + tid) * 8 + c] = bacc[l][c];
  __syncthreads();
  if (tid < NP * COUT) {
    const int co = tid % COUT, q = tid / COUT, cc = co / 8, c = co % 8;
    float v = 0.f;
    for (int j = q; j < NU; j += NP) {
      const int xpi = j % W2, r = (j / W2) % ROWSD, fi = j / (W2 * ROWSD);
      v += Rb[((((fi * CCD + cc) * ROWSD) + r) * W2 + xpi) * 8 + c];
    }
    Rp[co * NP + q] = v;
  }
  __syncthreads();
  if (tid < COUT) {
    float v = 0.f;
    for (int q = 0; q < NP; ++q) v += Rp[tid * NP + q];
    s[COUT * NCOL + tid] = v;
  }
  if constexpr (PM == 0) f16_range_note(rmax);
#ifdef PAIG_BWD_STAMPS
  PAIG_BSTAMP(7);
  if (lane == 0 && blockIdx.x < 4096) {
#pragma unroll
    for (int k = 0; k < 12; ++k) paig_bwd_stamps[blockIdx.x][wv][k] = st_acc[k];
    paig_bwd_stamps[blockIdx.x][wv][12] = st_n;
  }
#endif
}

template <int CIN, int COUT, int H, int W, int KS, bool UPS, int PM, bool PF = false>
static int sbwd_launch(FView x, FView dy, FViewW dx, FView aux, const float* w, int flags, float* slab, int nblk_max,
                       int* nblk_out, int F, hipStream_t st, XMax xm, const void* wp,
                       FView dpool = FView{nullptr, 0, 0, 0}, const unsigned char* pcode = nullptr,
                       long long pcode_fs = 0) {
  using C = SBwdCfg<CIN, COUT, H, W, KS, UPS, PM, PF>;
  constexpr int RED = (C::NLD * 256 * 8 + 256) * 4;
  constexpr int LDS0 = C::LDS > RED ? C::LDS : RED;
  static_assert(LDS0 <= LDS_MAX, "fused backward: staging exceeds the LDS");
  static const int lds_pad = [] {
    const char* e = getenv("PAIG_BWD_LDS_PAD");
    return e ? atoi(e) : 0;
  }();
  const int LDS = LDS0 + lds_pad <= LDS_MAX ? LDS0 + lds_pad : LDS0;
  const int ntiles = cdiv(F, C::FPT) * (H / C::RT);
  auto k = conv_bwd_split_k<CIN, COUT, H, W, KS, UPS, PM, PF>;
  static int resident = 0;
  if (!resident) {
    if (LDS > 64 * 1024) (void)hipFuncSetAttribute((const void*)k, hipFuncAttributeMaxDynamicSharedMemorySize, LDS);
    resident = persistent_grid((const void*)k, LDS);
  }
  int nb = ntiles < nblk_max ? ntiles : nblk_max;
  if (nb > resident) nb = resident;
  {
    static int mt = -1;
    if (mt < 0) {
      const char* e = getenv("PAIG_BWD_MIN_TPB");
      mt = e ? atoi(e) : 0;
    }
    if (mt > 1 && nb > cdiv(ntiles, mt)) nb = cdiv(ntiles, mt);
  }
  if (nb < 1) nb = 1;
  *nblk_out = nb;
  PAIG_REQUIRE(!xm.p || (xm.n % 4 == 0 && (reinterpret_cast<uintptr_t>(xm.p) & 15) == 0),
               "conv split bwd: xmax needs 16-byte alignment and a multiple of 4 slots (%d)", xm.n);
  PAIG_REQUIRE(!(flags & 2) || aux.p, "conv split bwd: ReLU' mask (flags & 2) without aux");
  constexpr long long SPAN = (1ll << 31) / (4 * C::FPT) - 8 * 4096;
  PAIG_REQUIRE(x.fs < SPAN && dy.fs < SPAN && aux.fs < SPAN && dpool.fs < SPAN && pcode_fs < 4 * SPAN &&
                   x.fs >= 0 && dy.fs >= 0 && aux.fs >= 0 && dpool.fs >= 0 && pcode_fs >= 0,
               "conv split bwd: a frame stride does not fit the tile's 32-bit byte offsets");
  PAIG_REQUIRE(!PF || (dpool.p && pcode && (reinterpret_cast<uintptr_t>(pcode) & 7) == 0 && pcode_fs % 8 == 0),
               "conv split bwd: pool fold needs the pooled gradient and 8-byte aligned window codes");
  hipLaunchKernelGGL(k, dim3(nb), dim3(256), LDS, st, x, dy, dx, aux, w, flags, slab, F, ntiles, xm,
                     PM == 0 ? static_cast<const s16x8*>(wp) : nullptr, dpool, pcode, pcode_fs);
  PAIG_CHECK_LAUNCH();
  return 0;
}

#define PAIG_BWD_UP_SHAPES(X) X(32, 16, 16) X(16, 16, 32) X(16, 16, 36) X(32, 16, 18)
#define PAIG_BWD_POOL_SHAPES(X) X(8, 8, 32) X(16, 16, 16) X(16, 16, 64) X(8, 8, 36) X(16, 16, 18)
#define PAIG_BWD_SHAPES(X)                                                                  \
  X(8, 8, 32) X(8, 16, 16) X(16, 16, 16) X(16, 32, 8) X(32, 32, 8) X(32, 16, 16) X(24, 8, 32) \
  X(8, 8, 36) X(8, 16, 18) X(16, 16, 18) X(32, 16, 18) X(24, 8, 36)                            \
  X(16, 16, 64) X(16, 32, 32)

}

extern "C" {

int paig_conv2d_bwd_supported(int Cin, int Cout, int H, int W, int ks, int flags) {
  if (H != W || ks != 3 || !(flags & (128 | 256))) return 0;
#define PAIG_CASE(CI, CO, HH) \
  if (Cin == CI && Cout == CO && H == HH) return 1;
  if (flags & 64) {
    if (flags & 32) return 0;
    PAIG_BWD_POOL_SHAPES(PAIG_CASE)
    return 0;
  }
  if (flags & 32) {
    PAIG_BWD_UP_SHAPES(PAIG_CASE)
    return 0;
  }
  PAIG_BWD_SHAPES(PAIG_CASE)
#undef PAIG_CASE
  return 0;
}

int paig_conv2d_bwd(const float* x, long long x_fs, int x_grp, long long x_gs, const float* dy, long long dy_fs,
                    float* dx, long long dx_fs, const float* aux, long long aux_fs, const float* w, float* slab,
                    int nblk_max, int* nblk_out, int F, int Cin, int Cout, int H, int W, int ks, int flags,
                    const float* xmax, int xmax_n, const float* dpool, long long dpool_fs,
                    const unsigned char* pcode, long long pcode_fs, const void* wprep, void* stream) {
  *nblk_out = 0;
  if (F <= 0) return 0;
  PAIG_REQUIRE(paig_conv2d_bwd_supported(Cin, Cout, H, W, ks, flags),
               "paig_conv2d_bwd: no fused kernel for Cin=%d Cout=%d H=%d W=%d ks=%d flags=%d", Cin, Cout, H, W, ks,
               flags);
  PAIG_REQUIRE(x_grp == 0 || H * W >= 256, "paig_conv2d_bwd: multi-frame tiles need a plain frame stride");
  PAIG_REQUIRE(nblk_max > 0 && slab && dx && dy && x && w, "paig_conv2d_bwd: null operand or no slab rows");
  hipStream_t st = (hipStream_t)stream;
  FView vx{x, x_fs, x_gs, x_grp}, vd{dy, dy_fs, 0, 0}, va{aux, aux_fs, 0, 0};
  FViewW vdx{dx, dx_fs};
  XMax xm{const_cast<float*>(xmax), xmax_n};
  const bool b16 = (flags & 256) != 0;
  const int fl = flags & 6;
  if (flags & 64) {
    const FView vp{dpool, dpool_fs, 0, 0};
#define PAIG_CASE(CI, CO, HH)                                                                                     \
  if (Cin == CI && Cout == CO && H == HH)                                                                         \
    return b16 ? sbwd_launch<CI, CO, HH, HH, 3, false, 2, true>(vx, vd, vdx, va, w, fl, slab, nblk_max, nblk_out,  \
                                                                 F, st, xm, wprep, vp, pcode, pcode_fs)            \
               : sbwd_launch<CI, CO, HH, HH, 3, false, 0, true>(vx, vd, vdx, va, w, fl, slab, nblk_max, nblk_out,  \
                                                                 F, st, xm, wprep, vp, pcode, pcode_fs);
    PAIG_BWD_POOL_SHAPES(PAIG_CASE)
#undef PAIG_CASE
    return PAIG_E_UNSUPPORTED;
  }
  if (flags & 32) {
#define PAIG_CASE(CI, CO, HH)                                                                                     \
  if (Cin == CI && Cout == CO && H == HH)                                                                         \
    return b16 ? sbwd_launch<CI, CO, HH, HH, 3, true, 2>(vx, vd, vdx, va, w, fl, slab, nblk_max, nblk_out, F, st, \
                                                           xm, wprep)                                             \
               : sbwd_launch<CI, CO, HH, HH, 3, true, 0>(vx, vd, vdx, va, w, fl, slab, nblk_max, nblk_out, F, st, \
                                                           xm, wprep);
    PAIG_BWD_UP_SHAPES(PAIG_CASE)
#undef PAIG_CASE
    return PAIG_E_UNSUPPORTED;
  }
#define PAIG_CASE(CI, CO, HH)                                                                                      \
  if (Cin == CI && Cout == CO && H == HH)                                                                          \
    return b16 ? sbwd_launch<CI, CO, HH, HH, 3, false, 2>(vx, vd, vdx, va, w, fl, slab, nblk_max, nblk_out, F, st, \
                                                            xm, wprep)                                             \
               : sbwd_launch<CI, CO, HH, HH, 3, false, 0>(vx, vd, vdx, va, w, fl, slab, nblk_max, nblk_out, F, st, \
                                                            xm, wprep);
  PAIG_BWD_SHAPES(PAIG_CASE)
#undef PAIG_CASE
  return PAIG_E_UNSUPPORTED;
}

#ifdef PAIG_BWD_STAMPS
int paig_bwd_stamps_read(void* host, size_t bytes) {
  return (int)hipMemcpyFromSymbol(host, HIP_SYMBOL(paig_bwd_stamps), bytes);
}
#endif

}

PAIG_F16_RANGE_ACCESSOR(paig_f16_range_bwd)
```

paig_reproduction_amd/csrc/unet.hip:

```cpp
#include "common.h"

#include <vector>

#define UNET_HIP(call)                                                  \
  do {                                                                  \
    const hipError_t _e = (call);                                       \
    if (_e != hipSuccess) {                                             \
      paig_set_error("%s: %s", __func__, hipGetErrorString(_e));        \
      return (int)_e;                                                   \
    }                                                                   \
  } while (0)

namespace {

enum { U_CONV = 0, U_POOL = 1, U_UP = 2 };

struct Reg {
  int buf, off, n;
  bool operator==(const Reg& o) const { return buf == o.buf && off == o.off && n == o.n; }
};
struct UOp {
  int kind;
  int conv;
  Reg src, dst;
  bool relu;
  int ks;
};
struct UBuf {
  int C, lvl;
};

struct UPlan {
  std::vector<UBuf> bufs;
  std::vector<UOp> ops;
  int nconv = 0, X0 = 0, LG = 0;
  std::vector<std::vector<std::pair<Reg, bool>>> fin;
  std::vector<int> fused_up;
  std::vector<bool> fused_buf;
};

void build_plan(UPlan& p, int net, int K) {
  auto buf = [&](int C, int lvl) {
    p.bufs.push_back(UBuf{C, lvl});
    return (int)p.bufs.size() - 1;
  };
  auto conv = [&](Reg s, Reg d, bool relu, int ks = 3) { p.ops.push_back(UOp{U_CONV, p.nconv++, s, d, relu, ks}); };
  auto pool = [&](Reg s, Reg d) { p.ops.push_back(UOp{U_POOL, -1, s, d, false, 0}); };
  auto up = [&](Reg s, Reg d) { p.ops.push_back(UOp{U_UP, -1, s, d, false, 0}); };
  if (net == 0) {
    const int c = 8;
    const int X0 = buf(3, 1), A1 = buf(c, 1), CAT2 = buf(3 * c, 1), P1 = buf(c, 2), A3 = buf(2 * c, 2),
              CAT1 = buf(4 * c, 2), P2 = buf(2 * c, 4), A5 = buf(4 * c, 4), A6 = buf(4 * c, 4), U1 = buf(4 * c, 2),
              A8 = buf(2 * c, 2), A9 = buf(2 * c, 2), U2 = buf(2 * c, 1), A11 = buf(c, 1), A12 = buf(c, 1),
              LG = buf(K, 1);
    p.X0 = X0;
    p.LG = LG;
    conv({X0, 0, 3}, {A1, 0, c}, true);
    conv({A1, 0, c}, {CAT2, 2 * c, c}, true);
    pool({CAT2, 2 * c, c}, {P1, 0, c});
    conv({P1, 0, c}, {A3, 0, 2 * c}, true);
    conv({A3, 0, 2 * c}, {CAT1, 2 * c, 2 * c}, true);
    pool({CAT1, 2 * c, 2 * c}, {P2, 0, 2 * c});
    conv({P2, 0, 2 * c}, {A5, 0, 4 * c}, true);
    conv({A5, 0, 4 * c}, {A6, 0, 4 * c}, true);
    up({A6, 0, 4 * c}, {U1, 0, 4 * c});
    conv({U1, 0, 4 * c}, {CAT1, 0, 2 * c}, false);
    conv({CAT1, 0, 4 * c}, {A8, 0, 2 * c}, true);
    conv({A8, 0, 2 * c}, {A9, 0, 2 * c}, true);
    up({A9, 0, 2 * c}, {U2, 0, 2 * c});
    conv({U2, 0, 2 * c}, {CAT2, 0, 2 * c}, false);
    conv({CAT2, 0, 3 * c}, {A11, 0, c}, true);
    conv({A11, 0, c}, {A12, 0, c}, true);
    conv({A12, 0, c}, {LG, 0, K}, true, 1);
  } else {
    const int h = 16;
    const int X0 = buf(3, 1), A1 = buf(h, 1), CAT3 = buf(3 * h, 1), P1 = buf(h, 2), A3 = buf(2 * h, 2),
              CAT2 = buf(4 * h, 2), P2 = buf(2 * h, 4), A5 = buf(4 * h, 4), CAT1 = buf(6 * h, 4), P3 = buf(4 * h, 8),
              A7 = buf(8 * h, 8), A8 = buf(8 * h, 8), U1 = buf(8 * h, 4), A10 = buf(4 * h, 4), A11 = buf(4 * h, 4),
              U2 = buf(4 * h, 2), A13 = buf(2 * h, 2), A14 = buf(2 * h, 2), U3 = buf(2 * h, 1), A16 = buf(h, 1),
              A17 = buf(h, 1), LG = buf(K, 1);
    p.X0 = X0;
    p.LG = LG;
    conv({X0, 0, 3}, {A1, 0, h}, true);
    conv({A1, 0, h}, {CAT3, 2 * h, h}, true);
    pool({CAT3, 2 * h, h}, {P1, 0, h});
    conv({P1, 0, h}, {A3, 0, 2 * h}, true);
    conv({A3, 0, 2 * h}, {CAT2, 2 * h, 2 * h}, true);
    pool({CAT2, 2 * h, 2 * h}, {P2, 0, 2 * h});
    conv({P2, 0, 2 * h}, {A5, 0, 4 * h}, true);
    conv({A5, 0, 4 * h}, {CAT1, 2 * h, 4 * h}, true);
    pool({CAT1, 2 * h, 4 * h}, {P3, 0, 4 * h});
    conv({P3, 0, 4 * h}, {A7, 0, 8 * h}, true);
    conv({A7, 0, 8 * h}, {A8, 0, 8 * h}, true);
    up({A8, 0, 8 * h}, {U1, 0, 8 * h});
    conv({U1, 0, 8 * h}, {CAT1, 0, 2 * h}, false);
    conv({CAT1, 0, 6 * h}, {A10, 0, 4 * h}, true);
    conv({A10, 0, 4 * h}, {A11, 0, 4 * h}, true);
    up({A11, 0, 4 * h}, {U2, 0, 4 * h});
    conv({U2, 0, 4 * h}, {CAT2, 0, 2 * h}, false);
    conv({CAT2, 0, 4 * h}, {A13, 0, 2 * h}, true);
    conv({A13, 0, 2 * h}, {A14, 0, 2 * h}, true);
    up({A14, 0, 2 * h}, {U3, 0, 2 * h});
    conv({U3, 0, 2 * h}, {CAT3, 0, 2 * h}, false);
    conv({CAT3, 0, 3 * h}, {A16, 0, h}, true);
    conv({A16, 0, h}, {A17, 0, h}, true);
    conv({A17, 0, h}, {LG, 0, K}, false, 1);
  }
}

bool overlap(const Reg& a, const Reg& b) { return a.buf == b.buf && a.off < b.off + b.n && b.off < a.off + a.n; }

void derive(UPlan& p, int H, int cm) {
  const int n = (int)p.ops.size();
  p.fin.assign(n, {});
  for (int pi = 0; pi < n; ++pi) {
    int first = -1;
    for (int i = pi + 1; i < n && first < 0; ++i)
      if (overlap(p.ops[i].src, p.ops[pi].dst)) first = i;
    if (first >= 0) p.fin[first].push_back({p.ops[pi].dst, p.ops[pi].kind == U_CONV && p.ops[pi].relu});
  }
  p.fused_up.assign(n, -1);
  p.fused_buf.assign(p.bufs.size(), false);
  for (int i = 0; i < n; ++i) {
    const UOp& u = p.ops[i];
    if (u.kind != U_UP) continue;
    int cons = -1, ncons = 0;
    for (int j = 0; j < n; ++j)
      if (p.ops[j].src.buf == u.dst.buf) {
        cons = j;
        ++ncons;
      }
    if (ncons != 1 || p.ops[cons].kind != U_CONV) continue;
    const UOp& c = p.ops[cons];
    const int Hc = H / p.bufs[u.dst.buf].lvl;
    bool ok = true;
    for (int w = 0; w < 2; ++w)
      ok = ok && paig_conv2d_mfma_supported(w, c.src.n, c.dst.n, Hc, Hc, c.ks, 32 | cm);
    if (ok) {
      p.fused_up[cons] = i;
      p.fused_buf[u.dst.buf] = true;
    }
  }
}

bool pool_fused(const UPlan& p, int i, int H, int cm) {
  const UOp& op = p.ops[i];
  if (op.kind != U_CONV || i + 1 >= (int)p.ops.size() || cm == 0 || p.fused_up[i] >= 0) return false;
  const UOp& nx = p.ops[i + 1];
  const int Hl = H / p.bufs[op.dst.buf].lvl;
  return nx.kind == U_POOL && nx.src == op.dst &&
         paig_conv2d_mfma_supported(0, op.src.n, op.dst.n, Hl, Hl, op.ks, cm | 64);
}
bool pool_fold_fused(const UPlan& p, int i, int H, int cm) {
  const UOp& op = p.ops[i];
  const int Hl = H / p.bufs[op.dst.buf].lvl;
  return paig_conv2d_bwd_supported(op.src.n, op.dst.n, Hl, Hl, op.ks, cm | 64);
}
bool pool_fold_split(const UPlan& p, int i, int H, int cm, int flags) {
  const UOp& op = p.ops[i];
  const int Hl = H / p.bufs[op.dst.buf].lvl;
  return cm == 128 && !(flags & PAIG_UNET_STANDALONE_POOL) && op.src.buf != p.X0 && !pool_fold_fused(p, i, H, cm) &&
         !paig_conv2d_bwd_supported(op.src.n, op.dst.n, Hl, Hl, op.ks, cm) &&
         paig_conv2d_mfma_supported(1, op.src.n, op.dst.n, Hl, Hl, op.ks, 128 | 64) &&
         paig_conv2d_mfma_supported(0, op.dst.n, op.src.n, Hl, Hl, op.ks, 8 | 128 | 64);
}
bool pool_folded(const UPlan& p, int i, int H, int cm, int flags) {
  const UOp& op = p.ops[i];
  if (flags & (PAIG_UNET_SEPARATE_BWD | PAIG_UNET_INFERENCE)) return false;
  if (op.kind != U_CONV || i + 1 >= (int)p.ops.size() || cm == 0 || p.fused_up[i] >= 0) return false;
  const UOp& nx = p.ops[i + 1];
  const int Hl = H / p.bufs[op.dst.buf].lvl;
  return nx.kind == U_POOL && nx.src == op.dst && (pool_fold_fused(p, i, H, cm) || pool_fold_split(p, i, H, cm, flags));
}

constexpr int NBLK_MAX = 1024;
size_t a256(size_t b) { return (b + 255) & ~(size_t)255; }

struct ULayout {
  std::vector<size_t> act, grad, slab, wprep0, wprep1, pcode;
  std::vector<long long> pcode_fs;
  size_t xmax = 0, total = 0;
};

void layout(const UPlan& p, ULayout& L, int F, int H, int cm, int flags) {
  const bool train = !(flags & PAIG_UNET_INFERENCE);
  const size_t NONE = (size_t)-1;
  size_t off = 0;
  auto take = [&](size_t bytes) {
    const size_t o = off;
    off += a256(bytes);
    return o;
  };
  const int nb = (int)p.bufs.size(), no = (int)p.ops.size();
  L.act.assign(nb, NONE);
  L.grad.assign(nb, NONE);
  for (int b = 0; b < nb; ++b) {
    const size_t hw = (size_t)(H / p.bufs[b].lvl) * (H / p.bufs[b].lvl);
    const size_t bytes = (size_t)F * p.bufs[b].C * hw * 4;
    if (b != p.X0 && b != p.LG && !p.fused_buf[b]) L.act[b] = take(bytes);
    if (b != p.X0 && train) L.grad[b] = take(bytes);
  }
  L.xmax = take((size_t)no * PAIG_XMAX_SLOTS * 4);
  L.slab.assign(no, NONE);
  L.wprep0.assign(no, NONE);
  L.wprep1.assign(no, NONE);
  L.pcode.assign(no, NONE);
  L.pcode_fs.assign(no, 0);
  for (int i = 0; i < no; ++i) {
    const UOp& op = p.ops[i];
    if (op.kind != U_CONV) continue;
    const int cin = op.src.n, cout = op.dst.n, ks = op.ks;
    if (train) L.slab[i] = take((size_t)NBLK_MAX * (cout * cin * ks * ks + cout) * 4);
    if (cm == 128 && !(flags & PAIG_UNET_EXT_WPREP)) {
      L.wprep0[i] = take((size_t)paig_conv_wprep_size(cin, cout, ks) * 2);
      if (op.src.buf != p.X0) L.wprep1[i] = take((size_t)paig_conv_wprep_size(cout, cin, ks) * 2);
    }
    if (pool_folded(p, i, H, cm, flags)) {
      const int Hl = H / p.bufs[op.dst.buf].lvl;
      L.pcode_fs[i + 1] = (long long)((cout + 7) / 8 * 8) * (Hl / 2) * (Hl / 2);
      L.pcode[i + 1] = take((size_t)F * L.pcode_fs[i + 1]);
    }
  }
  L.total = off;
}

struct View {
  const float* p;
  long long fs;
  int grp;
  long long gs;
};

int check_args(int net, int F, int H, int K, int cm) {
  PAIG_REQUIRE(net == 0 || net == 1, "paig_unet: net %d (0 ShallowUNet, 1 UNet)", net);
  PAIG_REQUIRE(F > 0 && H > 0 && H % (net == 0 ? 4 : 8) == 0 && K > 0, "paig_unet: F=%d H=%d K=%d", F, H, K);
  PAIG_REQUIRE(cm == 0 || cm == 128 || cm == 256, "paig_unet: conv math %d (0 fp32, 128 split, 256 bf16)", cm);
  return 0;
}

struct UProbe {
  paig_unet_probe_fn fn;
  void* ctx;
  void operator()(int ev, int op, int conv, int kind, int cin, int cout, int Hl, int fl) const {
    if (fn) fn(ctx, ev, op, conv, kind, cin, cout, Hl, fl);
  }
};

int fwd_impl(int net, int F, int H, int K, int math, int flags, const float* x, long long x_fs, int x_grp,
             long long x_gs, const float* const* w, const float* const* b, float* logits, const void* const* wpf,
             const void* const* wpd, void* ws, size_t ws_bytes, UProbe pr, void* stream) {
  struct WprepFlush {
    void* st;
    ~WprepFlush() { (void)paig_conv_wprep_flush(st); }
  } wflush{stream};
  if (int rc = check_args(net, F, H, K, math)) return rc;
  UPlan p;
  build_plan(p, net, K);
  derive(p, H, math);
  ULayout L;
  layout(p, L, F, H, math, flags);
  const bool head = (flags & PAIG_UNET_HEAD_FUSED) != 0, ext = (flags & PAIG_UNET_EXT_WPREP) != 0;
  PAIG_REQUIRE(ws && ws_bytes >= L.total && x && (logits || head) && w && b && (!ext || math != 128 || (wpf && wpd)),
               "paig_unet_fwd: workspace %zu bytes < %zu, or a null operand", ws_bytes, L.total);
  char* base = static_cast<char*>(ws);
  const int cm = math;
  auto view = [&](const Reg& r, int& lvl) {
    lvl = p.bufs[r.buf].lvl;
    const long long hw = (long long)(H / lvl) * (H / lvl);
    if (r.buf == p.X0) return View{x + r.off * hw, x_fs, x_grp, x_gs};
    float* t = r.buf == p.LG ? logits : reinterpret_cast<float*>(base + L.act[r.buf]);
    return View{t + r.off * hw, p.bufs[r.buf].C * hw, 0, 0};
  };
  float* xmax = reinterpret_cast<float*>(base + L.xmax);
  const size_t xmax_n = p.ops.size() * PAIG_XMAX_SLOTS;
  static const bool memset_ab = getenv("PAIG_XMAX_MEMSET") != nullptr;
  const bool prezero =
      !memset_ab && !p.ops.empty() && p.ops[0].kind == U_CONV && p.fused_up[0] < 0 && p.ops.size() > 1;
  if (prezero) paig_conv_fwd_prezero(xmax + PAIG_XMAX_SLOTS, (int)(xmax_n - PAIG_XMAX_SLOTS));
  else UNET_HIP(hipMemsetAsync(xmax, 0, xmax_n * 4, (hipStream_t)stream));
  const int no = (int)p.ops.size(), nrun = head ? no - 1 : no;
  auto wimg0 = [&](int i) -> const void* {
    return cm != 128 ? nullptr : (ext ? wpf[p.ops[i].conv] : base + L.wprep0[i]);
  };
  if (cm == 128 && !ext) {
    std::vector<const float*> jw;
    std::vector<int> jci, jco, jks, jdg;
    std::vector<void*> jout;
    for (int i = 0; i < no; ++i) {
      const UOp& op = p.ops[i];
      if (op.kind != U_CONV) continue;
      jw.push_back(w[op.conv]), jci.push_back(op.src.n), jco.push_back(op.dst.n), jks.push_back(op.ks),
          jdg.push_back(0), jout.push_back(base + L.wprep0[i]);
      if (op.src.buf != p.X0)
        jw.push_back(w[op.conv]), jci.push_back(op.dst.n), jco.push_back(op.src.n), jks.push_back(op.ks),
            jdg.push_back(1), jout.push_back(base + L.wprep1[i]);
    }
    if (int rc = paig_conv_wprep((int)jw.size(), jw.data(), jci.data(), jco.data(), jks.data(), jdg.data(),
                                 jout.data(), stream))
      return rc;
  }
  std::vector<bool> pooled(no, false);
  for (int i = 0; i < nrun; ++i) {
    const UOp& op = p.ops[i];
    if ((op.kind == U_UP && p.fused_buf[op.dst.buf]) || pooled[i]) continue;
    int dlvl;
    const View dv = view(op.dst, dlvl);
    int rc = 0;
    if (op.kind == U_CONV) {
      int slvl, xfl = 0;
      View sv;
      if (p.fused_up[i] >= 0) {
        sv = view(p.ops[p.fused_up[i]].src, slvl);
        slvl /= 2;
        xfl = 32;
      } else {
        sv = view(op.src, slvl);
      }
      const int Hl = H / slvl;
      float* pool_out = nullptr;
      long long pool_fs = 0;
      unsigned char* pcode = nullptr;
      long long pcode_fs = 0;
      if (pool_fused(p, i, H, cm) && i + 1 < nrun) {
        int pl;
        const View pv = view(p.ops[i + 1].dst, pl);
        pool_out = const_cast<float*>(pv.p);
        pool_fs = pv.fs;
        pooled[i + 1] = true;
        if (L.pcode[i + 1] != (size_t)-1) {
          pcode = reinterpret_cast<unsigned char*>(base + L.pcode[i + 1]);
          pcode_fs = L.pcode_fs[i + 1];
        }
      }
      const int fl = (op.relu ? 1 : 0) | xfl | cm | (pool_out ? 64 : 0);
      pr(0, i, op.conv, PAIG_PROBE_CONV_FWD, op.src.n, op.dst.n, Hl, fl);
      rc = paig_conv2d_fwd_pwc(sv.p, sv.fs, sv.grp, sv.gs, const_cast<float*>(dv.p), dv.fs, nullptr, 0, w[op.conv],
                               b[op.conv], F, op.src.n, op.dst.n, Hl, Hl, op.ks, fl,
                               xmax + (size_t)i * PAIG_XMAX_SLOTS, PAIG_XMAX_SLOTS, pool_out, pool_fs, pcode, pcode_fs,
                               wimg0(i), stream);
      pr(1, i, op.conv, PAIG_PROBE_CONV_FWD, op.src.n, op.dst.n, Hl, fl);
      if (i == 0 && prezero && paig_conv_fwd_prezero_pending()) {
        if (rc) return rc;
        UNET_HIP(hipMemsetAsync(xmax, 0, xmax_n * 4, (hipStream_t)stream));
      }
    } else if (op.kind == U_POOL) {
      int slvl;
      const View sv = view(op.src, slvl);
      const int Hl = H / slvl;
      rc = L.pcode[i] != (size_t)-1
               ? paig_maxpool2_fwd_codes(sv.p, sv.fs, const_cast<float*>(dv.p), dv.fs,
                                         reinterpret_cast<unsigned char*>(base + L.pcode[i]), L.pcode_fs[i], F,
                                         op.src.n, Hl, Hl, stream)
               : paig_maxpool2_fwd(sv.p, sv.fs, const_cast<float*>(dv.p), dv.fs, F, op.src.n, Hl, Hl, stream);
    } else {
      int slvl;
      const View sv = view(op.src, slvl);
      const int Hs = H / slvl, Ho = H / dlvl;
      rc = paig_upsample2_fwd(sv.p, sv.fs, const_cast<float*>(dv.p), dv.fs, F, op.src.n, Hs, Hs, Ho, Ho, stream);
    }
    if (rc) return rc;
  }
  return 0;
}

int bwd_impl(int net, int F, int H, int K, int math, int flags, const float* x, long long x_fs, int x_grp,
             long long x_gs, const float* const* w, const float* logits, const float* dlogits, float* const* dwb,
             int n_extra, const float* const* e_src, const int* e_nb, const int* e_len, float* const* e_dst,
             const void* const* wpd, void* ws, size_t ws_bytes, UProbe pr, void* stream) {
  if (int rc = check_args(net, F, H, K, math)) return rc;
  UPlan p;
  build_plan(p, net, K);
  derive(p, H, math);
  ULayout L;
  layout(p, L, F, H, math, flags);
  const bool head = (flags & PAIG_UNET_HEAD_FUSED) != 0, ext = (flags & PAIG_UNET_EXT_WPREP) != 0;
  const bool sep = (flags & PAIG_UNET_SEPARATE_BWD) != 0;
  PAIG_REQUIRE(!(flags & PAIG_UNET_INFERENCE), "paig_unet_bwd: the forward ran in inference mode (no gradients)");
  PAIG_REQUIRE(ws && ws_bytes >= L.total && x && (head || (logits && dlogits)) && w && dwb &&
                   (!ext || math != 128 || wpd) && n_extra >= 0 && (n_extra == 0 || (e_src && e_nb && e_len && e_dst)),
               "paig_unet_bwd: workspace %zu bytes < %zu, or a null operand", ws_bytes, L.total);
  char* base = static_cast<char*>(ws);
  hipStream_t st = (hipStream_t)stream;
  const int cm = math, no = (int)p.ops.size();
  float* xmax = reinterpret_cast<float*>(base + L.xmax);
  auto view = [&](const Reg& r, int& lvl) {
    lvl = p.bufs[r.buf].lvl;
    const long long hw = (long long)(H / lvl) * (H / lvl);
    if (r.buf == p.X0) return View{x + r.off * hw, x_fs, x_grp, x_gs};
    const float* t = r.buf == p.LG ? logits : reinterpret_cast<const float*>(base + L.act[r.buf]);
    return View{t + r.off * hw, p.bufs[r.buf].C * hw, 0, 0};
  };
  auto dview = [&](const Reg& r) {
    const long long hw = (long long)(H / p.bufs[r.buf].lvl) * (H / p.bufs[r.buf].lvl);
    float* t = reinterpret_cast<float*>(base + L.grad[r.buf]);
    return View{t + r.off * hw, p.bufs[r.buf].C * hw, 0, 0};
  };
  std::vector<std::vector<std::pair<int, int>>> written(p.bufs.size());
  int first;
  if (head) {
    const Reg hs = p.ops[no - 1].src;
    written[hs.buf].push_back({hs.off, hs.n});
    first = no - 2;
  } else {
    float* dlg = reinterpret_cast<float*>(base + L.grad[p.LG]);
    const long long nlg = (long long)F * K * H * H;
    UNET_HIP(hipMemcpyAsync(dlg, dlogits, nlg * 4, hipMemcpyDeviceToDevice, st));
    if (net == 0)
      if (int rc = paig_relu_mask(logits, dlg, nlg, stream)) return rc;
    written[p.LG].push_back({0, K});
    first = no - 1;
  }
  auto state = [&](const Reg& r) {
    int cov = 0;
    for (auto& s : written[r.buf]) {
      const int lo = r.off > s.first ? r.off : s.first, hi = r.off + r.n < s.first + s.second ? r.off + r.n
                                                                                           : s.first + s.second;
      if (hi > lo) cov += hi - lo;
    }
    return cov == 0 ? 0 : (cov == r.n ? 1 : -1);
  };
  auto mark = [&](const Reg& r) { written[r.buf].push_back({r.off, r.n}); };
  std::vector<const float*> s_src;
  std::vector<int> s_nb, s_len;
  std::vector<float*> s_dst;
  std::vector<bool> folded_up(no, false);
  for (int i = first; i >= 0; --i) {
    if (folded_up[i]) continue;
    const UOp& op = p.ops[i];
    if (op.kind == U_POOL && L.pcode[i] != (size_t)-1) continue;
    bool relu_fin = false;
    for (auto& f : p.fin[i]) relu_fin = relu_fin || f.second;
    const View dyv = dview(op.dst);
    int rc = 0;
    if (op.kind == U_CONV) {
      int slvl, xfl = 0;
      View sv;
      if (p.fused_up[i] >= 0) {
        sv = view(p.ops[p.fused_up[i]].src, slvl);
        slvl /= 2;
        xfl = 32;
      } else {
        sv = view(op.src, slvl);
      }
      const int Hl = H / slvl, cin = op.src.n, cout = op.dst.n, ks = op.ks;
      float* slab = reinterpret_cast<float*>(base + L.slab[i]);
      const int n_w = cout * cin * ks * ks;
      int nb = 0;
      const float* xm = xmax + (size_t)i * PAIG_XMAX_SLOTS;
      const void* wp1 = cm != 128 || op.src.buf == p.X0 ? nullptr : (ext ? wpd[op.conv] : base + L.wprep1[i]);
      if (xfl && cm && !sep && paig_conv2d_bwd_supported(cin, cout, Hl, Hl, ks, cm | 32)) {
        const int ui = p.fused_up[i];
        const Reg usrc = p.ops[ui].src;
        const View dxv = dview(usrc);
        PAIG_REQUIRE(state(usrc) == 0, "paig_unet_bwd: upsample source gradient already written (op %d)", i);
        int flags2 = cm | 32, alvl;
        const float* aux = nullptr;
        long long aux_fs = 0;
        for (auto& f : p.fin[ui])
          if (f.first == usrc && f.second) {
            const View a = view(usrc, alvl);
            aux = a.p;
            aux_fs = a.fs;
            flags2 |= 2;
          }
        pr(0, i, op.conv, PAIG_PROBE_CONV_BWD, cin, cout, Hl, flags2);
        rc = paig_conv2d_bwd(sv.p, sv.fs, sv.grp, sv.gs, dyv.p, dyv.fs, const_cast<float*>(dxv.p), dxv.fs, aux, aux_fs,
                             w[op.conv], slab, NBLK_MAX, &nb, F, cin, cout, Hl, Hl, ks, flags2, xm, PAIG_XMAX_SLOTS,
                             nullptr, 0, nullptr, 0, wp1, stream);
        pr(1, i, op.conv, PAIG_PROBE_CONV_BWD, cin, cout, Hl, flags2);
        if (rc) return rc;
        s_src.push_back(slab), s_nb.push_back(nb), s_len.push_back(n_w + cout), s_dst.push_back(dwb[op.conv]);
        mark(usrc);
        folded_up[ui] = true;
        continue;
      }
      if (op.src.buf != p.X0 && !xfl && cm && !sep && paig_conv2d_bwd_supported(cin, cout, Hl, Hl, ks, cm)) {
        const View dxv = dview(op.src);
        const int mode = state(op.src);
        PAIG_REQUIRE(mode >= 0, "paig_unet_bwd: partially written gradient region (op %d)", i);
        int flags2 = cm | (mode == 1 ? 4 : 0), alvl;
        const float* aux = nullptr;
        long long aux_fs = 0;
        if (relu_fin) {
          PAIG_REQUIRE(p.fin[i].size() == 1 && p.fin[i][0].first == op.src, "paig_unet_bwd: mixed ReLU (op %d)", i);
          const View a = view(op.src, alvl);
          aux = a.p;
          aux_fs = a.fs;
          flags2 |= 2;
        }
        const float* dpool = nullptr;
        long long dpool_fs = 0;
        const unsigned char* pcode = nullptr;
        long long pcode_fs = 0;
        if (i + 1 < no && L.pcode[i + 1] != (size_t)-1) {
          PAIG_REQUIRE(state(op.dst) == 1, "paig_unet_bwd: pool fold before the skip gradient (op %d)", i);
          const View pdv = dview(p.ops[i + 1].dst);
          dpool = pdv.p;
          dpool_fs = pdv.fs;
          pcode = reinterpret_cast<const unsigned char*>(base + L.pcode[i + 1]);
          pcode_fs = L.pcode_fs[i + 1];
          flags2 |= 64;
        }
        pr(0, i, op.conv, PAIG_PROBE_CONV_BWD, cin, cout, Hl, flags2);
        rc = paig_conv2d_bwd(sv.p, sv.fs, sv.grp, sv.gs, dyv.p, dyv.fs, const_cast<float*>(dxv.p), dxv.fs, aux, aux_fs,
                             w[op.conv], slab, NBLK_MAX, &nb, F, cin, cout, Hl, Hl, ks, cm | (flags2 & 70), xm,
                             PAIG_XMAX_SLOTS, dpool, dpool_fs, pcode, pcode_fs, wp1, stream);
        pr(1, i, op.conv, PAIG_PROBE_CONV_BWD, cin, cout, Hl, flags2);
        if (rc) return rc;
        s_src.push_back(slab), s_nb.push_back(nb), s_len.push_back(n_w + cout), s_dst.push_back(dwb[op.conv]);
        mark(op.src);
        continue;
      }
      const bool pf = !xfl && i + 1 < no && L.pcode[i + 1] != (size_t)-1;
      const float* dpool = nullptr;
      long long dpool_fs = 0;
      const unsigned char* pcode = nullptr;
      long long pcode_fs = 0;
      if (pf) {
        PAIG_REQUIRE(state(op.dst) == 1, "paig_unet_bwd: pool fold before the skip gradient (op %d)", i);
        const View pdv = dview(p.ops[i + 1].dst);
        dpool = pdv.p;
        dpool_fs = pdv.fs;
        pcode = reinterpret_cast<const unsigned char*>(base + L.pcode[i + 1]);
        pcode_fs = L.pcode_fs[i + 1];
      }
      pr(0, i, op.conv, PAIG_PROBE_CONV_WGRAD, cin, cout, Hl, xfl | cm | (pf ? 64 : 0));
      rc = pf ? paig_conv2d_wgrad_pf(sv.p, sv.fs, sv.grp, sv.gs, dyv.p, dyv.fs, dpool, dpool_fs, pcode, pcode_fs, slab,
                                     NBLK_MAX, &nb, F, cin, cout, Hl, Hl, ks, cm | 64, xm, PAIG_XMAX_SLOTS, stream)
              : paig_conv2d_wgrad_ex(sv.p, sv.fs, sv.grp, sv.gs, dyv.p, dyv.fs, slab, NBLK_MAX, &nb, F, cin, cout, Hl, Hl,
                                     ks, xfl | cm, xm, PAIG_XMAX_SLOTS, stream);
      pr(1, i, op.conv, PAIG_PROBE_CONV_WGRAD, cin, cout, Hl, xfl | cm | (pf ? 64 : 0));
      if (rc) return rc;
      s_src.push_back(slab), s_nb.push_back(nb), s_len.push_back(n_w + cout), s_dst.push_back(dwb[op.conv]);
      PAIG_REQUIRE(!pf || op.src.buf != p.X0, "paig_unet_bwd: pool fold on the input layer (op %d)", i);
      if (op.src.buf == p.X0) continue;
      const int ui = p.fused_up[i];
      if (ui >= 0 && cm == 128 && !(flags & PAIG_UNET_STANDALONE_UP) &&
          paig_conv2d_mfma_supported(0, cout, cin, Hl, Hl, ks, 8 | 128 | 512)) {
        const Reg usrc = p.ops[ui].src;
        const View dxv = dview(usrc);
        PAIG_REQUIRE(state(usrc) == 0, "paig_unet_bwd: upsample source gradient already written (op %d)", i);
        int flags2 = 8 | 512, alvl;
        const float* aux = nullptr;
        long long aux_fs = 0;
        for (auto& f : p.fin[ui])
          if (f.first == usrc && f.second) {
            const View a = view(usrc, alvl);
            aux = a.p;
            aux_fs = a.fs;
            flags2 |= 2;
          }
        pr(0, i, op.conv, PAIG_PROBE_CONV_DGRAD, cin, cout, Hl, flags2 | cm);
        rc = paig_conv2d_fwd_pw(dyv.p, dyv.fs, 0, 0, const_cast<float*>(dxv.p), dxv.fs, aux, aux_fs, w[op.conv],
                                nullptr, F, cout, cin, Hl, Hl, ks, flags2 | cm, nullptr, 0, nullptr, 0, wp1, stream);
        pr(1, i, op.conv, PAIG_PROBE_CONV_DGRAD, cin, cout, Hl, flags2 | cm);
        if (rc) return rc;
        mark(usrc);
        folded_up[ui] = true;
        continue;
      }
      const View dxv = dview(op.src);
      const int mode = state(op.src);
      PAIG_REQUIRE(mode >= 0, "paig_unet_bwd: partially written gradient region (op %d)", i);
      int flags2 = 8 | (mode == 1 ? 4 : 0), alvl;
      const float* aux = nullptr;
      long long aux_fs = 0;
      if (relu_fin) {
        PAIG_REQUIRE(p.fin[i].size() == 1 && p.fin[i][0].first == op.src, "paig_unet_bwd: mixed ReLU (op %d)", i);
        const View a = view(op.src, alvl);
        aux = a.p;
        aux_fs = a.fs;
        flags2 |= 2;
      }
      if (pf) flags2 |= 64;
      pr(0, i, op.conv, PAIG_PROBE_CONV_DGRAD, cin, cout, Hl, flags2 | cm);
      rc = paig_conv2d_fwd_pwc(dyv.p, dyv.fs, 0, 0, const_cast<float*>(dxv.p), dxv.fs, aux, aux_fs, w[op.conv], nullptr,
                               F, cout, cin, Hl, Hl, ks, flags2 | cm, nullptr, 0, const_cast<float*>(dpool), dpool_fs,
                               const_cast<unsigned char*>(pcode), pcode_fs, wp1, stream);
      pr(1, i, op.conv, PAIG_PROBE_CONV_DGRAD, cin, cout, Hl, flags2 | cm);
      mark(op.src);
    } else if (op.kind == U_POOL) {
      int slvl;
      const View sv = view(op.src, slvl);
      const int Hl = H / slvl;
      const View dxv = dview(op.src);
      PAIG_REQUIRE(state(op.src) == 1, "paig_unet_bwd: max-pool backward before its concat partner (op %d)", i);
      rc = paig_maxpool2_bwd_relu(sv.p, sv.fs, dyv.p, dyv.fs, const_cast<float*>(dxv.p), dxv.fs, F, op.src.n, Hl, Hl,
                                  stream);
      mark(op.src);
    } else {
      int slvl, dlvl;
      const View sv = view(op.src, slvl);
      (void)view(op.dst, dlvl);
      const int Hs = H / slvl, Ho = H / dlvl;
      const View dxv = dview(op.src);
      PAIG_REQUIRE(state(op.src) == 0, "paig_unet_bwd: upsample source gradient already written (op %d)", i);
      bool relu = false;
      for (auto& f : p.fin[i]) relu = relu || (f.first == op.src && f.second);
      rc = paig_upsample2_bwd(dyv.p, dyv.fs, sv.p, sv.fs, const_cast<float*>(dxv.p), dxv.fs, F, op.src.n, Hs, Hs, Ho,
                              Ho, relu ? 1 : 0, stream);
      mark(op.src);
    }
    if (rc) return rc;
  }
  for (int e = 0; e < n_extra; ++e)
    s_src.push_back(e_src[e]), s_nb.push_back(e_nb[e]), s_len.push_back(e_len[e]), s_dst.push_back(e_dst[e]);
  return paig_slab_reduce_multi((int)s_src.size(), s_src.data(), s_nb.data(), s_len.data(), s_dst.data(), 0, stream);
}

}

extern "C" {

size_t paig_unet_workspace_ex(int net, int F, int H, int K, int math, int flags) {
  if (check_args(net, F, H, K, math)) return 0;
  UPlan p;
  build_plan(p, net, K);
  derive(p, H, math);
  ULayout L;
  layout(p, L, F, H, math, flags);
  return L.total;
}

size_t paig_unet_workspace(int net, int F, int H, int K, int math) {
  return paig_unet_workspace_ex(net, F, H, K, math, 0);
}

long long paig_unet_buffer(int net, int F, int H, int K, int math, int flags, int which, int buf) {
  if (check_args(net, F, H, K, math)) return -1;
  UPlan p;
  build_plan(p, net, K);
  derive(p, H, math);
  if (buf < 0 || buf >= (int)p.bufs.size() || (which != 0 && which != 1)) return -1;
  ULayout L;
  layout(p, L, F, H, math, flags);
  const size_t o = which == 0 ? L.act[buf] : L.grad[buf];
  return o == (size_t)-1 ? -1 : (long long)o;
}

int paig_unet_query(int net, int K, int what) {
  if (net != 0 && net != 1) return -1;
  UPlan p;
  build_plan(p, net, K);
  switch (what) {
    case 0: return p.nconv;
    case 1: return (int)p.bufs.size();
    case 2: return p.ops.back().src.buf;
    case 3: return p.ops.back().src.n;
    case 4: return p.LG;
    case 5: return p.ops.back().src.off;
    case 6: return p.bufs[p.ops.back().src.buf].C;
    default: return -1;
  }
}

int paig_unet_fwd_ex(int net, int F, int H, int K, int math, int flags, const float* x, long long x_fs, int x_grp,
                     long long x_gs, const float* const* w, const float* const* b, float* logits,
                     const void* const* wprep_fwd, const void* const* wprep_dg, void* ws, size_t ws_bytes,
                     paig_unet_probe_fn probe, void* probe_ctx, void* stream) {
  return fwd_impl(net, F, H, K, math, flags, x, x_fs, x_grp, x_gs, w, b, logits, wprep_fwd, wprep_dg, ws, ws_bytes,
                  UProbe{probe, probe_ctx}, stream);
}

int paig_unet_bwd_ex(int net, int F, int H, int K, int math, int flags, const float* x, long long x_fs, int x_grp,
                     long long x_gs, const float* const* w, const float* logits, const float* dlogits,
                     float* const* dwb, int n_extra, const float* const* extra_src, const int* extra_nblk,
                     const int* extra_len, float* const* extra_dst, const void* const* wprep_dg, void* ws,
                     size_t ws_bytes, paig_unet_probe_fn probe, void* probe_ctx, void* stream) {
  return bwd_impl(net, F, H, K, math, flags, x, x_fs, x_grp, x_gs, w, logits, dlogits, dwb, n_extra, extra_src,
                  extra_nblk, extra_len, extra_dst, wprep_dg, ws, ws_bytes, UProbe{probe, probe_ctx}, stream);
}

int paig_unet_fwd(int net, int F, int H, int K, int math, const float* x, long long x_fs, int x_grp, long long x_gs,
                  const float* const* w, const float* const* b, float* logits, void* ws, size_t ws_bytes,
                  void* stream) {
  return fwd_impl(net, F, H, K, math, 0, x, x_fs, x_grp, x_gs, w, b, logits, nullptr, nullptr, ws, ws_bytes,
                  UProbe{nullptr, nullptr}, stream);
}

int paig_unet_bwd(int net, int F, int H, int K, int math, const float* x, long long x_fs, int x_grp, long long x_gs,
                  const float* const* w, const float* logits, const float* dlogits, float* const* dwb, void* ws,
                  size_t ws_bytes, void* stream) {
  return bwd_impl(net, F, H, K, math, 0, x, x_fs, x_grp, x_gs, w, logits, dlogits, dwb, 0, nullptr, nullptr, nullptr,
                  nullptr, nullptr, ws, ws_bytes, UProbe{nullptr, nullptr}, stream);
}

}
```

paig_reproduction_amd/csrc/unet_ops.hip:

```cpp
#include "common.h"

#define PAIG_MAX_SLAB_TASKS 32

namespace {

template <typename I>
__global__ void maxpool_fwd_k(FView x, FViewW y, int F, int C, int H, int W) {
  const int Ho = H / 2, Wo = W / 2;
  const I n = (I)F * C * Ho * Wo;
  for (I i = blockIdx.x * (I)blockDim.x + threadIdx.x; i < n; i += (I)gridDim.x * blockDim.x) {
    int j = i % Wo;
    I t = i / Wo;
    int ii = t % Ho;
    t /= Ho;
    int c = t % C;
    int f = (int)(t / C);
    const float* xp = x.frame(f) + ((long long)c * H + 2 * ii) * W + 2 * j;
    float m = xp[0];
    float v = xp[1];
    if (v > m || v != v) m = v;
    v = xp[W];
    if (v > m || v != v) m = v;
    v = xp[W + 1];
    if (v > m || v != v) m = v;
// ... 436 lines not shown
__device__ __forceinline__ void head_logits(const float* __restrict__ w, const float* __restrict__ b, const m4* xv,
                                            m4* l) {
#pragma unroll
  for (int k = 0; k < K; ++k) {
    m4 a = m4{b[k], b[k], b[k], b[k]};
#pragma unroll
    for (int c = 0; c < CI; ++c)
#pragma unroll
      for (int j = 0; j < 4; ++j) a[j] = fmaf(w[k * CI + c], xv[c][j], a[j]);
    l[k] = a;
  }
}

template <int K, bool RELU>
__device__ __forceinline__ void head_softmax(m4* l, m4* mk) {
  m4 m = m4{1.f, 1.f, 1.f, 1.f}, e[K + 1];
#pragma unroll
  for (int k = 0; k < K; ++k)
#pragma unroll
    for (int j = 0; j < 4; ++j) {
      if (RELU) l[k][j] = l[k][j] < 0.f ? 0.f : l[k][j];
      m[j] = fmaxf(m[j], l[k][j]);
    }
  m4 s = m4{0.f, 0.f, 0.f, 0.f};
#pragma unroll
  for (int k = 0; k < K; ++k) {
#pragma unroll
    for (int j = 0; j < 4; ++j) e[k][j] = expf(l[k][j] - m[j]);
    s += e[k];
  }
#pragma unroll
  for (int j = 0; j < 4; ++j) e[K][j] = expf(1.f - m[j]);
  s += e[K];
#pragma unroll
  for (int k = 0; k <= K; ++k)
#pragma unroll
    for (int j = 0; j < 4; ++j) mk[k][j] = e[k][j] / s[j];
}

template <int K, int CI, bool RELU>
__global__ void __launch_bounds__(256) head_mask_fwd_k(const float* __restrict__ xl, const float* __restrict__ w,
                                                       const float* __restrict__ b, FView x, float* __restrict__ masks,
                                                       float* __restrict__ objs, int F, int HW) {
  const int Q = HW / 4;
  const long long n = (long long)F * Q;
  for (long long i = blockIdx.x * (long long)blockDim.x + threadIdx.x; i < n; i += (long long)gridDim.x * blockDim.x) {
    const int p = (int)(i % Q) * 4;
    const int f = (int)(i / Q);
    m4 hv[CI];
#pragma unroll
    for (int c = 0; c < CI; ++c) hv[c] = *reinterpret_cast<const m4*>(xl + ((long long)f * CI + c) * HW + p);
    const float* xp = x.frame(f);
    m4 xv[3];
#pragma unroll
    for (int c = 0; c < 3; ++c) xv[c] = *reinterpret_cast<const m4*>(xp + c * HW + p);
    m4 l[K], mk[K + 1];
    head_logits<K, CI>(w, b, hv, l);
    head_softmax<K, RELU>(l, mk);
#pragma unroll
    for (int k = 0; k <= K; ++k) {
      *reinterpret_cast<m4*>(masks + ((long long)f * (K + 1) + k) * HW + p) = mk[k];
      if (k < K)
#pragma unroll
        for (int c = 0; c < 3; ++c)
          *reinterpret_cast<m4*>(objs + ((long long)k * F + f) * 3 * HW + (long long)c * HW + p) = mk[k] * xv[c];
    }
  }
}

template <int K, int CI, bool RELU>
__global__ void __launch_bounds__(256) head_mask_pool_fwd_k(const float* __restrict__ xl, const float* __restrict__ w,
                                                            const float* __restrict__ b, FView x,
                                                            float* __restrict__ masks, float* __restrict__ objs,
                                                            float* __restrict__ pobjs, int F, int H, int W) {
  const int HW = H * W, W2 = W / 2, W4 = W / 4, HW4 = (H / 2) * W2;
  const long long n = (long long)F * (H / 2) * W4;
  for (long long i = blockIdx.x * (long long)blockDim.x + threadIdx.x; i < n; i += (long long)gridDim.x * blockDim.x) {
    const int u = (int)(i % W4), py = (int)((i / W4) % (H / 2)), f = (int)(i / ((long long)W4 * (H / 2)));
    const float* xp = x.frame(f);
    float2 pa[K][3];
#pragma unroll
    for (int k = 0; k < K; ++k)
#pragma unroll
      for (int c = 0; c < 3; ++c) pa[k][c] = make_float2(0.f, 0.f);
#pragma unroll
    for (int rr = 0; rr < 2; ++rr) {
      const int p = (2 * py + rr) * W + 4 * u;
      m4 hv[CI];
#pragma unroll
      for (int c = 0; c < CI; ++c) hv[c] = *reinterpret_cast<const m4*>(xl + ((long long)f * CI + c) * HW + p);
      m4 xv[3];
#pragma unroll
      for (int c = 0; c < 3; ++c) xv[c] = *reinterpret_cast<const m4*>(xp + c * HW + p);
      m4 l[K], mk[K + 1];
      head_logits<K, CI>(w, b, hv, l);
      head_softmax<K, RELU>(l, mk);
#pragma unroll
      for (int k = 0; k <= K; ++k) {
        *reinterpret_cast<m4*>(masks + ((long long)f * (K + 1) + k) * HW + p) = mk[k];
        if (k < K)
#pragma unroll
          for (int c = 0; c < 3; ++c) {
            const m4 o = mk[k] * xv[c];
            *reinterpret_cast<m4*>(objs + ((long long)k * F + f) * 3 * HW + (long long)c * HW + p) = o;
            pa[k][c].x += o[0];
            pa[k][c].x += o[1];
            pa[k][c].y += o[2];
            pa[k][c].y += o[3];
          }
      }
    }
#pragma unroll
    for (int k = 0; k < K; ++k)
#pragma unroll
      for (int c = 0; c < 3; ++c)
        *reinterpret_cast<float2*>(pobjs + ((long long)k * F + f) * 3 * HW4 + (long long)c * HW4 + py * W2 + 2 * u) =
            make_float2(pa[k][c].x * 0.25f, pa[k][c].y * 0.25f);
  }
}

template <int K, int CI, bool RELU, bool POOL>
__global__ void __launch_bounds__(256) head_mask_bwd_k(const float* __restrict__ xl, const float* __restrict__ w,
                                                       const float* __restrict__ b, FView x,
                                                       const float* __restrict__ masks, const float* __restrict__ dobjs,
                                                       float* __restrict__ dxl, float* __restrict__ slab, int F, int H,
                                                       int W) {
  constexpr int NW = K * CI + K;
  const int HW = H * W, W2 = W / 2, HW4 = (H / 2) * W2;
  const int DHW = POOL ? HW4 : HW;
  const int Q = HW / 4;
  const long long n = (long long)F * Q;
  float acc[NW];
#pragma unroll
  for (int t = 0; t < NW; ++t) acc[t] = 0.f;
  for (long long i = blockIdx.x * (long long)blockDim.x + threadIdx.x; i < n; i += (long long)gridDim.x * blockDim.x) {
    const int p = (int)(i % Q) * 4;
    const int f = (int)(i / Q);
    const int pq = POOL ? ((p / W) >> 1) * W2 + ((p % W) >> 1) : p;
    m4 hv[CI];
#pragma unroll
    for (int c = 0; c < CI; ++c) hv[c] = *reinterpret_cast<const m4*>(xl + ((long long)f * CI + c) * HW + p);
    const float* xp = x.frame(f);
    m4 xv[3];
#pragma unroll
    for (int c = 0; c < 3; ++c) xv[c] = *reinterpret_cast<const m4*>(xp + c * HW + p);
    m4 dm[K], mk[K];
    m4 dot = m4{0.f, 0.f, 0.f, 0.f};
#pragma unroll
    for (int k = 0; k < K; ++k) {
      m4 a = m4{0.f, 0.f, 0.f, 0.f};
#pragma unroll
      for (int c = 0; c < 3; ++c) {
        const float* dp = dobjs + ((long long)k * F + f) * 3 * DHW + (long long)c * DHW + pq;
        m4 d;
        if constexpr (POOL) {
          const float2 dq = *reinterpret_cast<const float2*>(dp);
          d = m4{dq.x, dq.x, dq.y, dq.y} * 0.25f;
        } else {
          d = *reinterpret_cast<const m4*>(dp);
        }
#pragma unroll
        for (int j = 0; j < 4; ++j) a[j] = fmaf(d[j], xv[c][j], a[j]);
      }
      dm[k] = a;
      mk[k] = *reinterpret_cast<const m4*>(masks + ((long long)f * (K + 1) + k) * HW + p);
#pragma unroll
      for (int j = 0; j < 4; ++j) dot[j] = fmaf(mk[k][j], a[j], dot[j]);
    }
    m4 g[K];
    if constexpr (RELU) {
      m4 l[K];
      head_logits<K, CI>(w, b, hv, l);
#pragma unroll
      for (int k = 0; k < K; ++k) {
        g[k] = mk[k] * (dm[k] - dot);
#pragma unroll
        for (int j = 0; j < 4; ++j) g[k][j] = l[k][j] > 0.f ? g[k][j] : 0.f;
      }
    } else {
#pragma unroll
      for (int k = 0; k < K; ++k) g[k] = mk[k] * (dm[k] - dot);
    }
#pragma unroll
    for (int c = 0; c < CI; ++c) {
      m4 d = m4{0.f, 0.f, 0.f, 0.f};
#pragma unroll
      for (int k = 0; k < K; ++k)
#pragma unroll
        for (int j = 0; j < 4; ++j) d[j] = fmaf(w[k * CI + c], g[k][j], d[j]);
#pragma unroll
      for (int j = 0; j < 4; ++j) d[j] = hv[c][j] > 0.f ? d[j] : 0.f;
      *reinterpret_cast<m4*>(dxl + ((long long)f * CI + c) * HW + p) = d;
    }
#pragma unroll
    for (int k = 0; k < K; ++k) {
#pragma unroll
      for (int c = 0; c < CI; ++c)
#pragma unroll
        for (int j = 0; j < 4; ++j) acc[k * CI + c] = fmaf(g[k][j], hv[c][j], acc[k * CI + c]);
#pragma unroll
      for (int j = 0; j < 4; ++j) acc[K * CI + k] += g[k][j];
    }
  }
  __shared__ float red[4][NW];
  const int lane = threadIdx.x & 63, wv = threadIdx.x >> 6;
#pragma unroll
  for (int t = 0; t < NW; ++t) {
    float v = acc[t];
#pragma unroll
    for (int o = 32; o >= 1; o >>= 1) v += __shfl_xor(v, o, 64);
    if (lane == 0) red[wv][t] = v;
  }
  __syncthreads();
  if (threadIdx.x < NW)
    slab[(long long)blockIdx.x * NW + threadIdx.x] =
        ((red[0][threadIdx.x] + red[1][threadIdx.x]) + red[2][threadIdx.x]) + red[3][threadIdx.x];
}

__global__ void pos_head_fwd_k(const float* __restrict__ h3, float* __restrict__ pos, int N, int K, float half) {
  const int n = N * K * 2;
  for (int i = blockIdx.x * blockDim.x + threadIdx.x; i < n; i += gridDim.x * blockDim.x) {
    const int j = i & 1;
    const int k = (i >> 1) % K;
    const int r = i / (2 * K);
    pos[i] = tanhf(h3[((long long)k * N + r) * 2 + j]) * half + half;
  }
}

__global__ void pos_head_bwd_k(const float* __restrict__ h3, const float* __restrict__ dpos, float* __restrict__ dh3,
                               int N, int K, float half) {
  const int n = N * K * 2;
  for (int i = blockIdx.x * blockDim.x + threadIdx.x; i < n; i += gridDim.x * blockDim.x) {
    const int j = i & 1;
    const int k = (i >> 1) % K;
    const int r = i / (2 * K);
    const long long o = ((long long)k * N + r) * 2 + j;
    const float t = tanhf(h3[o]);
    dh3[o] = dpos[i] * half * (1.f - t * t);
  }
}

__global__ void vel_pack_k(const float* __restrict__ pos, float* __restrict__ X, int B, int Te, int K, int S,
                           int alt) {
  const int cols = (alt ? S - 1 : S) * 2;
  const int n = K * B * cols;
  const int D = 2 * K;
  for (int i = blockIdx.x * blockDim.x + threadIdx.x; i < n; i += gridDim.x * blockDim.x) {
    const int col = i % cols;
    const int row = i / cols;
    const int k = row / B, b = row % B;
    const int t = col >> 1, j = col & 1;
    const float* pb = pos + (long long)b * Te * D + 2 * k + j;
    X[i] = alt ? pb[(t + 1) * D] - pb[t * D] : pb[t * D];
  }
}

__global__ void vel_unpack_add_k(const float* __restrict__ dX, const float* __restrict__ dpos0, float* __restrict__ dpos,
                                 int B, int Te, int K, int S, int alt) {
  const int D = 2 * K;
  const int cols = (alt ? S - 1 : S) * 2;
  const int n = B * S * D;
  for (int i = blockIdx.x * blockDim.x + threadIdx.x; i < n; i += gridDim.x * blockDim.x) {
    const int d = i % D;
    const int t = (i / D) % S;
    const int b = i / (D * S);
    const int k = d >> 1, j = d & 1;
    const float* xr = dX ? dX + (long long)(k * B + b) * cols : nullptr;
    float g = 0.f;
    if (xr) {
      if (alt) {
        if (t >= 1) g += xr[(t - 1) * 2 + j];
        if (t <= S - 2) g -= xr[t * 2 + j];
      } else {
        g += xr[t * 2 + j];
      }
    }
    if (dpos0 && t == S - 1) g += dpos0[(long long)b * D + d];
    dpos[((long long)b * Te + t) * D + d] += g;
  }
}

__global__ void __launch_bounds__(256) slab_reduce_k(const float* __restrict__ slab, int nblk, long long ld, int len,
                                                     float* __restrict__ out, int accumulate) {
  __shared__ float red[4][64];
  const int lane = threadIdx.x & 63, wv = threadIdx.x >> 6;
  const int i = blockIdx.x * 64 + lane;
  float s = 0.f;
  if (i < len)
    for (int b = wv; b < nblk; b += 4) s += slab[(long long)b * ld + i];
  red[wv][lane] = s;
  __syncthreads();
  if (wv == 0 && i < len) {
    float v = (red[0][lane] + red[1][lane]) + (red[2][lane] + red[3][lane]);
    out[i] = accumulate ? out[i] + v : v;
  }
}

struct SlabTasks {
  const float* src[PAIG_MAX_SLAB_TASKS];
  float* dst[PAIG_MAX_SLAB_TASKS];
  int nblk[PAIG_MAX_SLAB_TASKS];
  int len[PAIG_MAX_SLAB_TASKS];
  int vec[PAIG_MAX_SLAB_TASKS];
  int start[PAIG_MAX_SLAB_TASKS + 1];
  int ntask;
  int accumulate;
};

__device__ __forceinline__ void slab_cols_scalar(const float* __restrict__ src, float* dst, int len, int nblk,
                                                 int blk, int accumulate, float (*red)[64]) {
  constexpr int NW = 16;
  const int lane = threadIdx.x & 63, wv = threadIdx.x >> 6;
  const int i = blk * 64 + lane;
  float s0 = 0.f, s1 = 0.f, s2 = 0.f, s3 = 0.f;
  if (i < len) {
    int b = wv;
    for (; b + 3 * NW < nblk; b += 4 * NW) {
      s0 += src[(long long)b * len + i];
      s1 += src[(long long)(b + NW) * len + i];
      s2 += src[(long long)(b + 2 * NW) * len + i];
      s3 += src[(long long)(b + 3 * NW) * len + i];
    }
    for (; b < nblk; b += NW) s0 += src[(long long)b * len + i];
  }
  red[wv][lane] = (s0 + s1) + (s2 + s3);
  __syncthreads();
  if (wv == 0 && i < len) {
    float v = 0.f;
#pragma unroll
    for (int w = 0; w < NW; ++w) v += red[w][lane];
    dst[i] = accumulate ? dst[i] + v : v;
  }
}

__device__ __forceinline__ void slab_cols_vec(const float* __restrict__ src0, float* dst, int len, int nblk, int blk,
                                              int accumulate, float4 (*red)[8]) {
  constexpr int NR = 128;
  const int c4 = threadIdx.x & 7, r = threadIdx.x >> 3;
  const int col = blk * 32 + c4 * 4;
  float4 s0 = make_float4(0.f, 0.f, 0.f, 0.f), s1 = s0;
  if (col < len) {
    const float* src = src0 + col;
    int b = r;
    for (; b + NR < nblk; b += 2 * NR) {
      const float4 a = *reinterpret_cast<const float4*>(src + (long long)b * len);
      const float4 c = *reinterpret_cast<const float4*>(src + (long long)(b + NR) * len);
      s0.x += a.x; s0.y += a.y; s0.z += a.z; s0.w += a.w;
      s1.x += c.x; s1.y += c.y; s1.z += c.z; s1.w += c.w;
    }
    if (b < nblk) {
      const float4 a = *reinterpret_cast<const float4*>(src + (long long)b * len);
      s0.x += a.x; s0.y += a.y; s0.z += a.z; s0.w += a.w;
    }
  }
  red[r][c4] = make_float4(s0.x + s1.x, s0.y + s1.y, s0.z + s1.z, s0.w + s1.w);
  __syncthreads();
#pragma unroll
  for (int h = NR / 2; h >= 1; h >>= 1) {
    if (r < h) {
      const float4 a = red[r][c4], c = red[r + h][c4];
      red[r][c4] = make_float4(a.x + c.x, a.y + c.y, a.z + c.z, a.w + c.w);
    }
    __syncthreads();
  }
  if (r == 0 && col < len) {
    const float4 v = red[0][c4];
    float4* d = reinterpret_cast<float4*>(dst + col);
    if (accumulate) {
      const float4 o = *d;
      *d = make_float4(o.x + v.x, o.y + v.y, o.z + v.z, o.w + v.w);
    } else {
      *d = v;
    }
  }
}

__global__ void __launch_bounds__(1024) slab_reduce_multi_k(SlabTasks T) {
  __shared__ float4 red_v[128][8];
  __shared__ float red_s[16][64];
  int t = 0;
  while (t + 1 < T.ntask && (int)blockIdx.x >= T.start[t + 1]) ++t;
  const int blk = (int)blockIdx.x - T.start[t];
  if (T.vec[t])
    slab_cols_vec(T.src[t], T.dst[t], T.len[t], T.nblk[t], blk, T.accumulate, red_v);
  else
    slab_cols_scalar(T.src[t], T.dst[t], T.len[t], T.nblk[t], blk, T.accumulate, red_s);
}

__global__ void __launch_bounds__(256) colsum_part_k(const float* __restrict__ X, int M, int N, long long ld,
                                                     float* __restrict__ part, int rows_per) {
  __shared__ float red[4][64];
  const int lane = threadIdx.x & 63, wv = threadIdx.x >> 6;
  const int n = blockIdx.x * 64 + lane;
  const int r0 = blockIdx.y * rows_per;
  int r1 = r0 + rows_per;
  if (r1 > M) r1 = M;
  float s = 0.f;
  if (n < N)
    for (int r = r0 + wv; r < r1; r += 4) s += X[(long long)r * ld + n];
  red[wv][lane] = s;
  __syncthreads();
  if (wv == 0 && n < N) part[(long long)blockIdx.y * N + n] = (red[0][lane] + red[1][lane]) + (red[2][lane] + red[3][lane]);
}

__global__ void axpby_k(const float* __restrict__ x, float* __restrict__ y, long long n, float a, float b) {
  for (long long i = blockIdx.x * (long long)blockDim.x + threadIdx.x; i < n; i += (long long)gridDim.x * blockDim.x)
    y[i] = a * x[i] + (b == 0.f ? 0.f : b * y[i]);
}

static inline bool int_index_ok(long long n) { return n + 8192LL * 256 < (1ll << 31); }
static inline int grid_for(long long n, int bs = 256) {
  long long g = (n + bs - 1) / bs;
  if (g > 8192) g = 8192;
  if (g < 1) g = 1;
  return (int)g;
}

}

extern "C" {

int paig_maxpool2_fwd(const float* x, long long x_fs, float* y, long long y_fs, int F, int C, int H, int W,
                      void* stream) {
  if (F <= 0) return 0;
  if (H % 2 == 0 && W % 4 == 0 && x_fs % 4 == 0 && y_fs % 2 == 0 && (long long)F * C * H * W < (1ll << 31) &&
      (uintptr_t)x % 16 == 0 && (uintptr_t)y % 8 == 0) {
    const long long nv = (long long)F * C * (H / 2) * (W / 4);
    hipLaunchKernelGGL(maxpool_fwd_v_k, dim3(grid_for(nv)), dim3(256), 0, (hipStream_t)stream, FView{x, x_fs, 0, 0},
                       FViewW{y, y_fs}, F, C, H, W);
    PAIG_CHECK_LAUNCH();
    return 0;
  }
  long long n = (long long)F * C * (H / 2) * (W / 2);
  if (int_index_ok(n))
    hipLaunchKernelGGL(maxpool_fwd_k<int>, dim3(grid_for(n)), dim3(256), 0, (hipStream_t)stream, FView{x, x_fs, 0, 0},
                     FViewW{y, y_fs}, F, C, H, W);
  else
    hipLaunchKernelGGL(maxpool_fwd_k<long long>, dim3(grid_for(n)), dim3(256), 0, (hipStream_t)stream, FView{x, x_fs, 0, 0},
                     FViewW{y, y_fs}, F, C, H, W);
  PAIG_CHECK_LAUNCH();
  return 0;
}

int paig_maxpool2_fwd_codes(const float* x, long long x_fs, float* y, long long y_fs, unsigned char* code,
                            long long code_fs, int F, int C, int H, int W, void* stream) {
  if (F <= 0) return 0;
  PAIG_REQUIRE(H % 2 == 0 && W % 2 == 0 && code && code_fs >= (long long)(C + 7) / 8 * 8 * (H / 2) * (W / 2) &&
                   (long long)F * C * H * W < (1ll << 31),
               "paig_maxpool2_fwd_codes: needs even H, W, a code frame of C/8 x H/2 x W/2 x 8 bytes (C=%d H=%d W=%d)",
               C, H, W);
  const long long n = (long long)F * C * (H / 2) * (W / 2);
  hipLaunchKernelGGL(maxpool_fwd_codes_k, dim3(grid_for(n)), dim3(256), 0, (hipStream_t)stream, FView{x, x_fs, 0, 0},
                     FViewW{y, y_fs}, code, code_fs, F, C, H, W);
  PAIG_CHECK_LAUNCH();
  return 0;
}

int paig_maxpool2_bwd_relu(const float* x, long long x_fs, const float* dy, long long dy_fs, float* dx, long long dx_fs,
                           int F, int C, int H, int W, void* stream) {
  if (F <= 0) return 0;
  if (H % 2 == 0 && W % 4 == 0 && x_fs % 4 == 0 && dx_fs % 4 == 0 && dy_fs % 2 == 0 &&
      (long long)F * C * H * W < (1ll << 31) && (uintptr_t)x % 16 == 0 && (uintptr_t)dx % 16 == 0 &&
      (uintptr_t)dy % 8 == 0) {
    const long long nv = (long long)F * C * (H / 2) * (W / 4);
    hipLaunchKernelGGL(maxpool_bwd_relu_v_k, dim3(grid_for(nv)), dim3(256), 0, (hipStream_t)stream,
                       FView{x, x_fs, 0, 0}, FView{dy, dy_fs, 0, 0}, FViewW{dx, dx_fs}, F, C, H, W);
    PAIG_CHECK_LAUNCH();
    return 0;
  }
  long long n = (long long)F * C * H * W;
  if (int_index_ok(n))
    hipLaunchKernelGGL(maxpool_bwd_relu_k<int>, dim3(grid_for(n)), dim3(256), 0, (hipStream_t)stream, FView{x, x_fs, 0, 0},
                     FView{dy, dy_fs, 0, 0}, FViewW{dx, dx_fs}, F, C, H, W);
  else
    hipLaunchKernelGGL(maxpool_bwd_relu_k<long long>, dim3(grid_for(n)), dim3(256), 0, (hipStream_t)stream, FView{x, x_fs, 0, 0},
                     FView{dy, dy_fs, 0, 0}, FViewW{dx, dx_fs}, F, C, H, W);
  PAIG_CHECK_LAUNCH();
  return 0;
}

int paig_upsample2_fwd(const float* s, long long s_fs, float* u, long long u_fs, int F, int C, int Hs, int Ws, int Ho,
                       int Wo, void* stream) {
  if (F <= 0) return 0;
  long long n = (long long)F * C * Ho * Wo;
  if (int_index_ok(n))
    hipLaunchKernelGGL(upsample_fwd_k<int>, dim3(grid_for(n)), dim3(256), 0, (hipStream_t)stream, FView{s, s_fs, 0, 0},
                     FViewW{u, u_fs}, F, C, Hs, Ws, Ho, Wo);
  else
    hipLaunchKernelGGL(upsample_fwd_k<long long>, dim3(grid_for(n)), dim3(256), 0, (hipStream_t)stream, FView{s, s_fs, 0, 0},
                     FViewW{u, u_fs}, F, C, Hs, Ws, Ho, Wo);
  PAIG_CHECK_LAUNCH();
  return 0;
}

int paig_upsample2_bwd(const float* du, long long du_fs, const float* s, long long s_fs, float* ds, long long ds_fs,
                       int F, int C, int Hs, int Ws, int Ho, int Wo, int relu_mask, void* stream) {
  if (F <= 0) return 0;
  PAIG_REQUIRE(Ho == 2 * Hs && Wo == 2 * Ws, "upsample_bwd: exact 2x upscale only (Resize(H/2 -> H))");
  if (Ws % 2 == 0 && Wo % 4 == 0 && du_fs % 4 == 0 && ds_fs % 2 == 0 && (!relu_mask || s_fs % 2 == 0) &&
      (long long)F * C * Ho * Wo < (1ll << 31) && (uintptr_t)du % 16 == 0 && (uintptr_t)ds % 8 == 0 &&
      (!relu_mask || (uintptr_t)s % 8 == 0)) {
    const long long nv = (long long)F * C * Hs * (Ws / 2);
    hipLaunchKernelGGL(upsample_bwd_v_k, dim3(grid_for(nv)), dim3(256), 0, (hipStream_t)stream,
                       FView{du, du_fs, 0, 0}, FView{s, s_fs, 0, 0}, FViewW{ds, ds_fs}, F, C, Hs, Ws, relu_mask);
    PAIG_CHECK_LAUNCH();
    return 0;
  }
  long long n = (long long)F * C * Hs * Ws;
  if (int_index_ok(n))
    hipLaunchKernelGGL(upsample_bwd_k<int>, dim3(grid_for(n)), dim3(256), 0, (hipStream_t)stream, FView{du, du_fs, 0, 0},
                     FView{s, s_fs, 0, 0}, FViewW{ds, ds_fs}, F, C, Hs, Ws, Ho, Wo, relu_mask);
  else
    hipLaunchKernelGGL(upsample_bwd_k<long long>, dim3(grid_for(n)), dim3(256), 0, (hipStream_t)stream, FView{du, du_fs, 0, 0},
                     FView{s, s_fs, 0, 0}, FViewW{ds, ds_fs}, F, C, Hs, Ws, Ho, Wo, relu_mask);
  PAIG_CHECK_LAUNCH();
  return 0;
}

int paig_mask_softmax_fwd(const float* logits, const float* x, long long x_fs, int x_grp, long long x_gs,
                          float* masks, float* objs, float* pobjs, int F, int K, int C, int H, int W, void* stream) {
  if (F <= 0) return 0;
  PAIG_REQUIRE(K >= 1 && K <= 7, "mask_softmax: K=%d", K);
  if (pobjs) {
    PAIG_REQUIRE(C <= 3 && H % 2 == 0 && W % 2 == 0, "mask_softmax pooled: C=%d H=%d W=%d", C, H, W);
    hipLaunchKernelGGL(mask_softmax_pool_fwd_k, dim3(grid_for((long long)F * (H / 2) * (W / 2))), dim3(256), 0,
                       (hipStream_t)stream, logits, FView{x, x_fs, x_gs, x_grp}, masks, objs, pobjs, F, K, C, H, W);
  } else {
    const bool v4 = (H * W) % 4 == 0 && C <= 3 && (K == 2 || K == 3) && x_fs % 4 == 0 && x_gs % 4 == 0 &&
                    ((uintptr_t)logits | (uintptr_t)x | (uintptr_t)masks | (uintptr_t)objs) % 16 == 0;
    const dim3 g4(grid_for((long long)F * H * W / 4));
    if (v4 && K == 2)
      hipLaunchKernelGGL(mask_softmax_fwd_v_k<2>, g4, dim3(256), 0, (hipStream_t)stream, logits,
                         FView{x, x_fs, x_gs, x_grp}, masks, objs, F, C, H * W);
    else if (v4 && K == 3)
      hipLaunchKernelGGL(mask_softmax_fwd_v_k<3>, g4, dim3(256), 0, (hipStream_t)stream, logits,
                         FView{x, x_fs, x_gs, x_grp}, masks, objs, F, C, H * W);
    else
      hipLaunchKernelGGL(mask_softmax_fwd_k, dim3(grid_for((long long)F * H * W)), dim3(256), 0, (hipStream_t)stream,
                         logits, FView{x, x_fs, x_gs, x_grp}, masks, objs, F, K, C, H * W);
  }
  PAIG_CHECK_LAUNCH();
  return 0;
}

int paig_mask_softmax_bwd(const float* logits, const float* x, long long x_fs, int x_grp, long long x_gs,
                          const float* masks, const float* dobjs, float* dlogits, int F, int K, int C, int H, int W,
                          int flags, void* stream) {
  if (F <= 0) return 0;
  PAIG_REQUIRE(K >= 1 && K <= 7, "mask_softmax: K=%d", K);
  const bool v4 = !(flags & 2) && (H * W) % 4 == 0 && C <= 3 && (K == 2 || K == 3) && x_fs % 4 == 0 &&
                  x_gs % 4 == 0 &&
                  ((uintptr_t)logits | (uintptr_t)x | (uintptr_t)masks | (uintptr_t)dobjs | (uintptr_t)dlogits) % 16 == 0;
  const dim3 g4(grid_for((long long)F * H * W / 4));
  if (v4 && K == 2)
    hipLaunchKernelGGL(mask_softmax_bwd_v_k<2>, g4, dim3(256), 0, (hipStream_t)stream, logits,
                       FView{x, x_fs, x_gs, x_grp}, masks, dobjs, dlogits, F, C, H * W, flags);
  else if (v4 && K == 3)
    hipLaunchKernelGGL(mask_softmax_bwd_v_k<3>, g4, dim3(256), 0, (hipStream_t)stream, logits,
                       FView{x, x_fs, x_gs, x_grp}, masks, dobjs, dlogits, F, C, H * W, flags);
  else
    hipLaunchKernelGGL(mask_softmax_bwd_k, dim3(grid_for((long long)F * H * W)), dim3(256), 0, (hipStream_t)stream,
                       logits, FView{x, x_fs, x_gs, x_grp}, masks, dobjs, dlogits, F, K, C, H, W, flags);
  PAIG_CHECK_LAUNCH();
  return 0;
}

static bool head_mask_ok(const void* a, const void* b, const void* c, const void* d, const void* e, long long x_fs,
                         long long x_gs, int K, int H, int W) {
  return (H * W) % 4 == 0 && (K == 2 || K == 3) && x_fs % 4 == 0 && x_gs % 4 == 0 &&
         ((uintptr_t)a | (uintptr_t)b | (uintptr_t)c | (uintptr_t)d | (uintptr_t)e) % 16 == 0;
}
static bool head_mask_kind(int CI, int flags, int H, int W, const void* pobjs) {
  if (CI == 8 && flags == 1) return true;
  return CI == 16 && flags == 2 && H % 2 == 0 && W % 4 == 0 && ((uintptr_t)pobjs % 8) == 0;
}

int paig_head_mask_blocks(int F, int H, int W) {
  const long long n = (long long)F * H * W / 4;
  long long g = (n + 255) / 256;
  return (int)(g < 1 ? 1 : (g > 1024 ? 1024 : g));
}

int paig_head_mask_fwd_ex(const float* xl, const float* w, const float* b, const float* x, long long x_fs, int x_grp,
                          long long x_gs, float* masks, float* objs, float* pobjs, int F, int K, int CI, int H, int W,
                          int flags, void* stream) {
  if (F <= 0) return 0;
  PAIG_REQUIRE(head_mask_ok(xl, x, masks, objs, nullptr, x_fs, x_gs, K, H, W),
               "head_mask_fwd: needs K in {2,3}, H*W %% 4 == 0 and 16-byte aligned buffers (K=%d H=%d W=%d)", K, H, W);
  PAIG_REQUIRE(head_mask_kind(CI, flags, H, W, pobjs) && (!(flags & 2) || pobjs),
               "head_mask_fwd: (CI=%d, flags=%d) is neither the ShallowUNet head (8, 1) nor the UNet's (16, 2)", CI,
               flags);
  const FView xv{x, x_fs, x_gs, x_grp};
  hipStream_t st = (hipStream_t)stream;
  if (flags & 2) {
    const dim3 g(grid_for((long long)F * (H / 2) * (W / 4)));
    if (K == 2) hipLaunchKernelGGL((head_mask_pool_fwd_k<2, 16, false>), g, dim3(256), 0, st, xl, w, b, xv, masks, objs, pobjs, F, H, W);
    else hipLaunchKernelGGL((head_mask_pool_fwd_k<3, 16, false>), g, dim3(256), 0, st, xl, w, b, xv, masks, objs, pobjs, F, H, W);
  } else {
    const dim3 g(grid_for((long long)F * H * W / 4));
    if (K == 2) hipLaunchKernelGGL((head_mask_fwd_k<2, 8, true>), g, dim3(256), 0, st, xl, w, b, xv, masks, objs, F, H * W);
    else hipLaunchKernelGGL((head_mask_fwd_k<3, 8, true>), g, dim3(256), 0, st, xl, w, b, xv, masks, objs, F, H * W);
  }
  PAIG_CHECK_LAUNCH();
  return 0;
}

int paig_head_mask_bwd_ex(const float* xl, const float* w, const float* b, const float* x, long long x_fs, int x_grp,
                          long long x_gs, const float* masks, const float* dobjs, float* dxl, float* slab, int F, int K,
                          int CI, int H, int W, int flags, void* stream) {
  if (F <= 0) return 0;
  PAIG_REQUIRE(head_mask_ok(xl, x, masks, (flags & 2) ? nullptr : dobjs, dxl, x_fs, x_gs, K, H, W),
               "head_mask_bwd: needs K in {2,3}, H*W %% 4 == 0 and 16-byte aligned buffers (K=%d H=%d W=%d)", K, H, W);
  PAIG_REQUIRE(head_mask_kind(CI, flags, H, W, dobjs),
               "head_mask_bwd: (CI=%d, flags=%d) is neither the ShallowUNet head (8, 1) nor the UNet's (16, 2)", CI,
               flags);
  const dim3 g(paig_head_mask_blocks(F, H, W));
  const FView xv{x, x_fs, x_gs, x_grp};
  hipStream_t st = (hipStream_t)stream;
  if (flags & 2) {
    if (K == 2) hipLaunchKernelGGL((head_mask_bwd_k<2, 16, false, true>), g, dim3(256), 0, st, xl, w, b, xv, masks, dobjs, dxl, slab, F, H, W);
    else hipLaunchKernelGGL((head_mask_bwd_k<3, 16, false, true>), g, dim3(256), 0, st, xl, w, b, xv, masks, dobjs, dxl, slab, F, H, W);
  } else {
    if (K == 2) hipLaunchKernelGGL((head_mask_bwd_k<2, 8, true, false>), g, dim3(256), 0, st, xl, w, b, xv, masks, dobjs, dxl, slab, F, H, W);
    else hipLaunchKernelGGL((head_mask_bwd_k<3, 8, true, false>), g, dim3(256), 0, st, xl, w, b, xv, masks, dobjs, dxl, slab, F, H, W);
  }
  PAIG_CHECK_LAUNCH();
  return 0;
}

int paig_head_mask_fwd(const float* x12, const float* w, const float* b, const float* x, long long x_fs, int x_grp,
                       long long x_gs, float* masks, float* objs, int F, int K, int H, int W, void* stream) {
  return paig_head_mask_fwd_ex(x12, w, b, x, x_fs, x_grp, x_gs, masks, objs, nullptr, F, K, 8, H, W, 1, stream);
}

int paig_head_mask_bwd(const float* x12, const float* w, const float* b, const float* x, long long x_fs, int x_grp,
                       long long x_gs, const float* masks, const float* dobjs, float* dx12, float* slab, int F, int K,
                       int H, int W, void* stream) {
  return paig_head_mask_bwd_ex(x12, w, b, x, x_fs, x_grp, x_gs, masks, dobjs, dx12, slab, F, K, 8, H, W, 1, stream);
}

int paig_pos_head_fwd(const float* h3, float* pos, int N, int K, float half, void* stream) {
  hipLaunchKernelGGL(pos_head_fwd_k, dim3(grid_for(N * K * 2)), dim3(256), 0, (hipStream_t)stream, h3, pos, N, K, half);
  PAIG_CHECK_LAUNCH();
  return 0;
}

int paig_pos_head_bwd(const float* h3, const float* dpos, float* dh3, int N, int K, float half, void* stream) {
  hipLaunchKernelGGL(pos_head_bwd_k, dim3(grid_for(N * K * 2)), dim3(256), 0, (hipStream_t)stream, h3, dpos, dh3, N, K,
                     half);
  PAIG_CHECK_LAUNCH();
  return 0;
}

int paig_vel_pack(const float* pos, float* X, int B, int Te, int K, int S, int alt, void* stream) {
  hipLaunchKernelGGL(vel_pack_k, dim3(grid_for(K * B * S * 2)), dim3(256), 0, (hipStream_t)stream, pos, X, B, Te, K, S,
                     alt);
  PAIG_CHECK_LAUNCH();
  return 0;
}

int paig_vel_unpack_add(const float* dX, const float* dpos0, float* dpos, int B, int Te, int K, int S, int alt,
                        void* stream) {
  hipLaunchKernelGGL(vel_unpack_add_k, dim3(grid_for(B * S * 2 * K)), dim3(256), 0, (hipStream_t)stream, dX, dpos0,
                     dpos, B, Te, K, S, alt);
  PAIG_CHECK_LAUNCH();
  return 0;
}

int paig_slab_reduce_multi(int ntask, const float* const* src, const int* nblk, const int* len, float* const* dst,
                           int accumulate, void* stream) {
  PAIG_REQUIRE(ntask >= 0 && ntask <= PAIG_MAX_SLAB_TASKS, "slab_reduce_multi: %d tasks", ntask);
  if (ntask == 0) return 0;
  SlabTasks T;
  int blocks = 0;
  for (int t = 0; t < ntask; ++t) {
    PAIG_REQUIRE(len[t] >= 0 && nblk[t] >= 0, "slab_reduce_multi: task %d len %d nblk %d", t, len[t], nblk[t]);
    T.src[t] = src[t];
    T.dst[t] = dst[t];
    T.nblk[t] = nblk[t];
    T.len[t] = len[t];
    T.vec[t] = len[t] % 4 == 0 && ((uintptr_t)src[t] & 15) == 0 && ((uintptr_t)dst[t] & 15) == 0;
    T.start[t] = blocks;
    blocks += cdiv(len[t], T.vec[t] ? 32 : 64);
  }
  T.start[ntask] = blocks;
  T.ntask = ntask;
  T.accumulate = accumulate;
  if (blocks == 0) return 0;
  hipLaunchKernelGGL(slab_reduce_multi_k, dim3(blocks), dim3(1024), 0, (hipStream_t)stream, T);
  PAIG_CHECK_LAUNCH();
  return 0;
}

int paig_slab_reduce(const float* slab, int nblk, long long ld, int len, float* out, int accumulate, void* stream) {
  if (len <= 0) return 0;
  hipLaunchKernelGGL(slab_reduce_k, dim3(cdiv(len, 64)), dim3(256), 0, (hipStream_t)stream, slab, nblk, ld, len, out,
                     accumulate);
  PAIG_CHECK_LAUNCH();
  return 0;
}

size_t paig_colsum_workspace(int M, int N) {
  int rows_per = 256;
  int stripes = cdiv(M, rows_per);
  return (size_t)stripes * N;
}

int paig_colsum(const float* X, int M, int N, long long ld, float* out, int accumulate, float* ws, void* stream) {
  if (N <= 0) return 0;
  int rows_per = 256;
  int stripes = cdiv(M, rows_per);
  if (M <= 0) {
    stripes = 0;
  } else {
    hipLaunchKernelGGL(colsum_part_k, dim3(cdiv(N, 64), stripes), dim3(256), 0, (hipStream_t)stream, X, M, N, ld, ws,
                       rows_per);
    PAIG_CHECK_LAUNCH();
  }
  hipLaunchKernelGGL(slab_reduce_k, dim3(cdiv(N, 64)), dim3(256), 0, (hipStream_t)stream, ws, stripes, (long long)N, N,
                     out, accumulate);
  PAIG_CHECK_LAUNCH();
  return 0;
}

int paig_axpby(const float* x, float* y, long long n, float a, float b, void* stream) {
  if (n <= 0) return 0;
  hipLaunchKernelGGL(axpby_k, dim3(grid_for(n)), dim3(256), 0, (hipStream_t)stream, x, y, n, a, b);
  PAIG_CHECK_LAUNCH();
  return 0;
}

}
```

Baseline: 99980 video-seqs/s.

## Write conv bwd weight-grad slabs in MFMA accumulator order, remap during reduce

The split conv backward kernel can now write per-block weight-gradient partials directly in MFMA fragment order as contiguous f32x4 stores, instead of scattering each element to its (cout, cin, tap) position. The multi-slab reduction kernel gains an index remap that translates fragment order back to the canonical weight layout when it writes the final sum. The intent is to replace scattered global stores in the backward kernel with coalesced vector stores. In exchange the slab rows are padded, and the reduce now does scattered scalar writes to the destination plus extra index arithmetic. Extra timing stamps are added behind a debug macro.

Result: faster. 101,600 video-seqs/s, median of 6 (+1.7%).

```diff
diff --git a/include/paig_hip.h b/include/paig_hip.h
--- a/include/paig_hip.h
+++ b/include/paig_hip.h
@@ -42,6 +42,7 @@
                          float* slab, int nblk_max, int* nblk_out, int F, int Cin, int Cout, int H, int W, int ks,
                          int flags, const float* xmax, int xmax_n, void* stream);
 int paig_conv2d_bwd_supported(int Cin, int Cout, int H, int W, int ks, int flags);
+size_t paig_conv2d_bwd_slab_len(int Cin, int Cout, int ks, int flags);
 int paig_conv2d_bwd(const float* x, long long x_fs, int x_grp, long long x_gs, const float* dy, long long dy_fs,
                     float* dx, long long dx_fs, const float* aux, long long aux_fs, const float* w, float* slab,
                     int nblk_max, int* nblk_out, int F, int Cin, int Cout, int H, int W, int ks, int flags,
@@ -134,6 +135,8 @@
 int paig_slab_reduce(const float* slab, int nblk, long long ld, int len, float* out, int accumulate, void* stream);
 int paig_slab_reduce_multi(int ntask, const float* const* src, const int* nblk, const int* len, float* const* dst,
                            int accumulate, void* stream);
+int paig_slab_reduce_multi_frag(int ntask, const float* const* src, const int* nblk, const int* len,
+                                float* const* dst, const int* cin, const int* cout, int accumulate, void* stream);
 int paig_axpby(const float* x, float* y, long long n, float a, float b, void* stream);
 
 int paig_vfn_fwd(const float* W1, const float* b1, const float* W2, const float* b2, float* hout, float* y,
diff --git a/paig_reproduction_amd/_lib.py b/paig_reproduction_amd/_lib.py
--- a/paig_reproduction_amd/_lib.py
+++ b/paig_reproduction_amd/_lib.py
@@ -34,6 +34,7 @@
     "paig_conv2d_mfma_supported": (I, [I, I, I, I, I, I, I]),
     "paig_debug_fwd_block_cap": (I, [I]),
     "paig_conv2d_bwd_supported": (I, [I, I, I, I, I, I]),
+    "paig_conv2d_bwd_slab_len": (SZ, [I, I, I, I]),
     "paig_conv2d_bwd": (I, [P, LL, I, LL, P, LL, P, LL, P, LL, P, P, I, P, I, I, I, I, I, I, I, P, I, P, LL, P, LL,
                             P, P]),
     "paig_conv2d_fwd_pwc": (I, [P, LL, I, LL, P, LL, P, LL, P, P, I, I, I, I, I, I, I, P, I, P, LL, P, LL, P, P]),
@@ -93,6 +94,7 @@
     "paig_colsum": (I, [P, I, I, LL, P, I, P, P]),
     "paig_slab_reduce": (I, [P, I, LL, I, P, I, P]),
     "paig_slab_reduce_multi": (I, [I, P, P, P, P, I, P]),
+    "paig_slab_reduce_multi_frag": (I, [I, P, P, P, P, P, P, I, P]),
     "paig_axpby": (I, [P, P, LL, F32, F32, P]),
     "paig_vfn_fwd": (I, [P, P, P, P, P, P, P, I, P]),
     "paig_vfn_bwd_blocks": (I, [I]),
@@ -174,7 +176,7 @@
 
 _QUERY = {"paig_last_error", "paig_abi_version", "paig_f16_range_status", "paig_conv2d_mfma_supported",
           "paig_debug_fwd_block_cap",
-          "paig_conv2d_bwd_supported", "paig_velmlp_bwd_blocks",
+          "paig_conv2d_bwd_supported", "paig_conv2d_bwd_slab_len", "paig_velmlp_bwd_blocks",
           "paig_velmlp_slab_len", "paig_head_bwd_blocks", "paig_head_l2_bwd_blocks", "paig_head_mask_blocks", "paig_conv_wprep_size", "paig_gemm_workspace", "paig_colsum_workspace",
           "paig_gemm_parts_size", "paig_gemm_parts", "paig_unet_workspace", "paig_unet_workspace_ex",
           "paig_unet_buffer", "paig_unet_query", "paig_localiser_workspace",
diff --git a/paig_reproduction_amd/csrc/conv_bwd.hip b/paig_reproduction_amd/csrc/conv_bwd.hip
--- a/paig_reproduction_amd/csrc/conv_bwd.hip
+++ b/paig_reproduction_amd/csrc/conv_bwd.hip
@@ -20,7 +20,7 @@
 #endif
 
 #ifdef PAIG_BWD_STAMPS
-__device__ unsigned long long paig_bwd_stamps[4096][4][13];
+__device__ unsigned long long paig_bwd_stamps[4096][4][20];
 #define PAIG_BSTAMP(k)                                      \
   do {                                                      \
     const unsigned long long t_ = __builtin_amdgcn_s_memtime(); \
@@ -84,6 +84,13 @@
   if (CIN == 24 && H == 36 && PM == 0) return false;
   if (H == 18 && ((CIN == 8 && PM == 2) || (CIN == 16 && COUT == 16 && PM == 0))) return false;
   return true;
+}
+
+constexpr int sbwd_frag_len(int CIN, int COUT) {
+  return ceil_div(COUT, 16) * ceil_div(9 * (rup(CIN, 4) / 4), 4) * 256 + COUT;
+}
+constexpr bool sbwd_fragrows(int CIN, int COUT, int H, int PM, bool PF) {
+  return !(CIN == 8 && COUT == 8 && H == 36 && PM == 0 && !PF);
 }
 
 template <int CIN, int COUT, int H, int W, int KS, bool UPS, int PM, bool PF = false>
@@ -118,6 +125,8 @@
   static constexpr int NTF = BAL ? NTX / 4 : ceil_div(NTX, 4), NTR = BAL ? NTX % 4 : 0;
   static constexpr int KB = ceil_div(TPXV, 32);
   static constexpr int NCOL = CIN * KK, SLAB = COUT * NCOL + COUT;
+  static constexpr int SLABF = sbwd_frag_len(CIN, COUT);
+  static constexpr bool FRAG = sbwd_fragrows(CIN, COUT, H, PM, PF);
   static constexpr int UPX = W % 2 == 0 ? 2 : 1, W2 = W / UPX;
   static constexpr int NID = FPT * ROWSD * W2 * CCD, NLD = ceil_div(NID, 256);
   static constexpr int NIX = FPT * ROWS * W2 * CQ, NLX = ceil_div(NIX, 256);
@@ -171,7 +180,7 @@
   const int tid = threadIdx.x, lane = tid & 63, wv = tid >> 6, g = lane >> 4;
   __shared__ float smax[4];
 #ifdef PAIG_BWD_STAMPS
-  unsigned long long st_acc[12] = {0, 0, 0, 0, 0, 0, 0, 0, 0, 0, 0, 0}, st_last = __builtin_amdgcn_s_memtime(), st_n = 0;
+  unsigned long long st_acc[20] = {}, st_last = __builtin_amdgcn_s_memtime(), st_n = 0;
 #endif
 
   auto xplane = [](int cq) { return cq * XPL + ((cq & 1) ? 16 : 0) + ((cq & 2) ? 64 : 0); };
@@ -195,6 +204,7 @@
     }
   };
   zero_xhalo();
+  PAIG_BSTAMP(13);
 
   int ecx = PAIG_A_EXP, ecd = PM == 0 && PAIG_SCALE_MODE < 2 ? 100 : 0;
   float xsc = 1.f, dsc = __builtin_amdgcn_ldexpf(1.f, ecd);
@@ -262,6 +272,7 @@
     }
   }
 
+  PAIG_BSTAMP(14);
   int pbase[MW];
 #pragma unroll
   for (int mt = 0; mt < MW; ++mt) {
@@ -698,7 +709,9 @@
 
   int lt = blockIdx.x;
   auto tile_of =[&](int l) { return l < ntiles ? xcd_tile(l, ntiles) : ntiles; };
+  PAIG_BSTAMP(15);
   issue(tile_of(lt));
+  PAIG_BSTAMP(16);
   if (PM == 0 && xm.p) {
     float m = 0.f;
     for (int i = tid * 4; i < xm.n; i += 1024) {
@@ -712,6 +725,7 @@
     if (m > 0.f) ecx = f16_scale_exp(m);
     __syncthreads();
   }
+  PAIG_BSTAMP(17);
   if constexpr (PM == 0) xsc = __builtin_amdgcn_ldexpf(1.f, ecx);
   else ecx = 0;
 
@@ -961,8 +975,18 @@
 #endif
   }
 
-  float* s = slab + (long long)blockIdx.x * C::SLAB;
+  const bool frag = C::FRAG && (flags & 1024) != 0;
+  float* s = slab + (long long)blockIdx.x * (frag ? C::SLABF : C::SLAB);
   auto put_w = [&](int m, int nt, const f32x4& acc) __attribute__((always_inline)) {
+    if (frag) {
+      f32x4 v = acc;
+      if constexpr (PM == 0) {
+#pragma unroll
+        for (int r = 0; r < 4; ++r) v[r] = __builtin_amdgcn_ldexpf(v[r], -(ecx + ecd));
+      }
+      *reinterpret_cast<f32x4*>(s + ((m * NTX + nt) * 64 + lane) * 4) = v;
+      return;
+    }
     const int col = nt * 16 + (lane & 15), cq = col >> 2;
     const int tap = cq / CQ, ci = (cq % CQ) * 4 + (col & 3);
 #pragma unroll
@@ -978,6 +1002,7 @@
 #pragma unroll
     for (int j = 0; j < NTF; ++j)
       if (wv + j * 4 < NTX) put_w(m, wv + j * 4, accw[m][j]);
+  PAIG_BSTAMP(18);
   if constexpr (NTR > 0) {
     f32x4* Rt = reinterpret_cast<f32x4*>(lds16);
     __syncthreads();
@@ -993,6 +1018,7 @@
       put_w(u / NTR, NTF * 4 + u % NTR, v);
     }
   }
+  PAIG_BSTAMP(19);
   __syncthreads();
   float* Rb = reinterpret_cast<float*>(lds16);
   constexpr int NP = 256 / COUT, NU = FPT * ROWSD * W2;
@@ -1015,14 +1041,14 @@
   if (tid < COUT) {
     float v = 0.f;
     for (int q = 0; q < NP; ++q) v += Rp[tid * NP + q];
-    s[COUT * NCOL + tid] = v;
+    s[(frag ? C::SLABF - COUT : COUT * NCOL) + tid] = v;
   }
   if constexpr (PM == 0) f16_range_note(rmax);
 #ifdef PAIG_BWD_STAMPS
   PAIG_BSTAMP(7);
   if (lane == 0 && blockIdx.x < 4096) {
 #pragma unroll
-    for (int k = 0; k < 12; ++k) paig_bwd_stamps[blockIdx.x][wv][k] = st_acc[k];
+    for (int k = 0; k < 20; ++k) paig_bwd_stamps[blockIdx.x][wv][k] = st_acc[k];
     paig_bwd_stamps[blockIdx.x][wv][12] = st_n;
   }
 #endif
@@ -1064,6 +1090,7 @@
   PAIG_REQUIRE(!xm.p || (xm.n % 4 == 0 && (reinterpret_cast<uintptr_t>(xm.p) & 15) == 0),
                "conv split bwd: xmax needs 16-byte alignment and a multiple of 4 slots (%d)", xm.n);
   PAIG_REQUIRE(!(flags & 2) || aux.p, "conv split bwd: ReLU' mask (flags & 2) without aux");
+  PAIG_REQUIRE(C::FRAG || !(flags & 1024), "conv split bwd: no rows in accumulator order (flags & 1024) for this shape");
   constexpr long long SPAN = (1ll << 31) / (4 * C::FPT) - 8 * 4096;
   PAIG_REQUIRE(x.fs < SPAN && dy.fs < SPAN && aux.fs < SPAN && dpool.fs < SPAN && pcode_fs < 4 * SPAN &&
                    x.fs >= 0 && dy.fs >= 0 && aux.fs >= 0 && dpool.fs >= 0 && pcode_fs >= 0,
@@ -1089,6 +1116,7 @@
 
 int paig_conv2d_bwd_supported(int Cin, int Cout, int H, int W, int ks, int flags) {
   if (H != W || ks != 3 || !(flags & (128 | 256))) return 0;
+  if ((flags & 1024) && !sbwd_fragrows(Cin, Cout, H, flags & 256 ? 2 : 0, (flags & 64) != 0)) return 0;
 #define PAIG_CASE(CI, CO, HH) \
   if (Cin == CI && Cout == CO && H == HH) return 1;
   if (flags & 64) {
@@ -1103,6 +1131,11 @@
   PAIG_BWD_SHAPES(PAIG_CASE)
 #undef PAIG_CASE
   return 0;
+}
+
+size_t paig_conv2d_bwd_slab_len(int Cin, int Cout, int ks, int flags) {
+  if (ks != 3 || Cin <= 0 || Cout <= 0) return 0;
+  return flags & 1024 ? (size_t)sbwd_frag_len(Cin, Cout) : (size_t)Cout * Cin * 9 + Cout;
 }
 
 int paig_conv2d_bwd(const float* x, long long x_fs, int x_grp, long long x_gs, const float* dy, long long dy_fs,
@@ -1122,7 +1155,9 @@
   FViewW vdx{dx, dx_fs};
   XMax xm{const_cast<float*>(xmax), xmax_n};
   const bool b16 = (flags & 256) != 0;
-  const int fl = flags & 6;
+  const int fl = flags & (6 | 1024);
+  PAIG_REQUIRE(!(flags & 1024) || (reinterpret_cast<uintptr_t>(slab) & 15) == 0,
+               "paig_conv2d_bwd: rows in accumulator order (flags & 1024) need a 16-byte aligned slab");
   if (flags & 64) {
     const FView vp{dpool, dpool_fs, 0, 0};
 #define PAIG_CASE(CI, CO, HH)                                                                                     \
diff --git a/paig_reproduction_amd/csrc/unet.hip b/paig_reproduction_amd/csrc/unet.hip
--- a/paig_reproduction_amd/csrc/unet.hip
+++ b/paig_reproduction_amd/csrc/unet.hip
@@ -1,5 +1,6 @@
 #include "common.h"
 
+#include <algorithm>
 #include <vector>
 
 #define UNET_HIP(call)                                                  \
@@ -175,6 +176,10 @@
 
 constexpr int NBLK_MAX = 1024;
 size_t a256(size_t b) { return (b + 255) & ~(size_t)255; }
+int bwd_row_flag(int cin, int cout, int ks) {
+  const size_t plain = paig_conv2d_bwd_slab_len(cin, cout, ks, 0), fr = paig_conv2d_bwd_slab_len(cin, cout, ks, 1024);
+  return plain > 0 && fr <= plain + plain / 8 ? 1024 : 0;
+}
 
 struct ULayout {
   std::vector<size_t> act, grad, slab, wprep0, wprep1, pcode;
@@ -210,7 +215,11 @@
     const UOp& op = p.ops[i];
     if (op.kind != U_CONV) continue;
     const int cin = op.src.n, cout = op.dst.n, ks = op.ks;
-    if (train) L.slab[i] = take((size_t)NBLK_MAX * (cout * cin * ks * ks + cout) * 4);
+    if (train) {
+      size_t row = (size_t)cout * cin * ks * ks + cout;
+      if (bwd_row_flag(cin, cout, ks)) row = std::max(row, paig_conv2d_bwd_slab_len(cin, cout, ks, 1024));
+      L.slab[i] = take((size_t)NBLK_MAX * row * 4);
+    }
     if (cm == 128 && !(flags & PAIG_UNET_EXT_WPREP)) {
       L.wprep0[i] = take((size_t)paig_conv_wprep_size(cin, cout, ks) * 2);
       if (op.src.buf != p.X0) L.wprep1[i] = take((size_t)paig_conv_wprep_size(cout, cin, ks) * 2);
@@ -421,7 +430,7 @@
   };
   auto mark = [&](const Reg& r) { written[r.buf].push_back({r.off, r.n}); };
   std::vector<const float*> s_src;
-  std::vector<int> s_nb, s_len;
+  std::vector<int> s_nb, s_len, s_cin, s_cout;
   std::vector<float*> s_dst;
   std::vector<bool> folded_up(no, false);
   for (int i = first; i >= 0; --i) {
@@ -453,6 +462,7 @@
         const Reg usrc = p.ops[ui].src;
         const View dxv = dview(usrc);
         PAIG_REQUIRE(state(usrc) == 0, "paig_unet_bwd: upsample source gradient already written (op %d)", i);
+        const int rfl = bwd_row_flag(cin, cout, ks);
         int flags2 = cm | 32, alvl;
         const float* aux = nullptr;
         long long aux_fs = 0;
@@ -465,18 +475,20 @@
           }
         pr(0, i, op.conv, PAIG_PROBE_CONV_BWD, cin, cout, Hl, flags2);
         rc = paig_conv2d_bwd(sv.p, sv.fs, sv.grp, sv.gs, dyv.p, dyv.fs, const_cast<float*>(dxv.p), dxv.fs, aux, aux_fs,
-                             w[op.conv], slab, NBLK_MAX, &nb, F, cin, cout, Hl, Hl, ks, flags2, xm, PAIG_XMAX_SLOTS,
+                             w[op.conv], slab, NBLK_MAX, &nb, F, cin, cout, Hl, Hl, ks, flags2 | rfl, xm, PAIG_XMAX_SLOTS,
                              nullptr, 0, nullptr, 0, wp1, stream);
         pr(1, i, op.conv, PAIG_PROBE_CONV_BWD, cin, cout, Hl, flags2);
         if (rc) return rc;
-        s_src.push_back(slab), s_nb.push_back(nb), s_len.push_back(n_w + cout), s_dst.push_back(dwb[op.conv]);
+        s_src.push_back(slab), s_nb.push_back(nb), s_dst.push_back(dwb[op.conv]);
+        s_len.push_back((int)paig_conv2d_bwd_slab_len(cin, cout, ks, rfl));
+        s_cin.push_back(rfl ? cin : 0), s_cout.push_back(rfl ? cout : 0);
         mark(usrc);
         folded_up[ui] = true;
         continue;
       }
       if (op.src.buf != p.X0 && !xfl && cm && !sep && paig_conv2d_bwd_supported(cin, cout, Hl, Hl, ks, cm)) {
         const View dxv = dview(op.src);
-        const int mode = state(op.src);
+        const int mode = state(op.src), rfl = bwd_row_flag(cin, cout, ks);
         PAIG_REQUIRE(mode >= 0, "paig_unet_bwd: partially written gradient region (op %d)", i);
         int flags2 = cm | (mode == 1 ? 4 : 0), alvl;
         const float* aux = nullptr;
@@ -503,11 +515,13 @@
         }
         pr(0, i, op.conv, PAIG_PROBE_CONV_BWD, cin, cout, Hl, flags2);
         rc = paig_conv2d_bwd(sv.p, sv.fs, sv.grp, sv.gs, dyv.p, dyv.fs, const_cast<float*>(dxv.p), dxv.fs, aux, aux_fs,
-                             w[op.conv], slab, NBLK_MAX, &nb, F, cin, cout, Hl, Hl, ks, cm | (flags2 & 70), xm,
+                             w[op.conv], slab, NBLK_MAX, &nb, F, cin, cout, Hl, Hl, ks, cm | (flags2 & 70) | rfl, xm,
                              PAIG_XMAX_SLOTS, dpool, dpool_fs, pcode, pcode_fs, wp1, stream);
         pr(1, i, op.conv, PAIG_PROBE_CONV_BWD, cin, cout, Hl, flags2);
         if (rc) return rc;
-        s_src.push_back(slab), s_nb.push_back(nb), s_len.push_back(n_w + cout), s_dst.push_back(dwb[op.conv]);
+        s_src.push_back(slab), s_nb.push_back(nb), s_dst.push_back(dwb[op.conv]);
+        s_len.push_back((int)paig_conv2d_bwd_slab_len(cin, cout, ks, rfl));
+        s_cin.push_back(rfl ? cin : 0), s_cout.push_back(rfl ? cout : 0);
         mark(op.src);
         continue;
       }
@@ -532,6 +546,7 @@
       pr(1, i, op.conv, PAIG_PROBE_CONV_WGRAD, cin, cout, Hl, xfl | cm | (pf ? 64 : 0));
       if (rc) return rc;
       s_src.push_back(slab), s_nb.push_back(nb), s_len.push_back(n_w + cout), s_dst.push_back(dwb[op.conv]);
+      s_cin.push_back(0), s_cout.push_back(0);
       PAIG_REQUIRE(!pf || op.src.buf != p.X0, "paig_unet_bwd: pool fold on the input layer (op %d)", i);
       if (op.src.buf == p.X0) continue;
       const int ui = p.fused_up[i];
@@ -604,8 +619,10 @@
     if (rc) return rc;
   }
   for (int e = 0; e < n_extra; ++e)
-    s_src.push_back(e_src[e]), s_nb.push_back(e_nb[e]), s_len.push_back(e_len[e]), s_dst.push_back(e_dst[e]);
-  return paig_slab_reduce_multi((int)s_src.size(), s_src.data(), s_nb.data(), s_len.data(), s_dst.data(), 0, stream);
+    s_src.push_back(e_src[e]), s_nb.push_back(e_nb[e]), s_len.push_back(e_len[e]), s_dst.push_back(e_dst[e]),
+        s_cin.push_back(0), s_cout.push_back(0);
+  return paig_slab_reduce_multi_frag((int)s_src.size(), s_src.data(), s_nb.data(), s_len.data(), s_dst.data(),
+                                     s_cin.data(), s_cout.data(), 0, stream);
 }
 
 }
diff --git a/paig_reproduction_amd/csrc/unet_ops.hip b/paig_reproduction_amd/csrc/unet_ops.hip
--- a/paig_reproduction_amd/csrc/unet_ops.hip
+++ b/paig_reproduction_amd/csrc/unet_ops.hip
@@ -762,13 +762,24 @@
   int nblk[PAIG_MAX_SLAB_TASKS];
   int len[PAIG_MAX_SLAB_TASKS];
   int vec[PAIG_MAX_SLAB_TASKS];
+  int cin[PAIG_MAX_SLAB_TASKS];
+  int cout[PAIG_MAX_SLAB_TASKS];
   int start[PAIG_MAX_SLAB_TASKS + 1];
   int ntask;
   int accumulate;
 };
 
+__device__ __forceinline__ int slab_frag_dst(int e, int cin, int cout) {
+  const int CQ = cin / 4, NQ = 9 * CQ, NTX = (NQ + 3) / 4, nfr = (cout + 15) / 16 * NTX * 256;
+  if (e >= nfr) return cout * cin * 9 + (e - nfr);
+  const int r = e & 3, ln = (e >> 2) & 63, f = e >> 8, nt = f % NTX, m = f / NTX;
+  const int col = nt * 16 + (ln & 15), cq = col >> 2, co = m * 16 + (ln >> 4) * 4 + r;
+  if (co >= cout || cq >= NQ) return -1;
+  return (co * cin + (cq % CQ) * 4 + (col & 3)) * 9 + cq / CQ;
+}
+
 __device__ __forceinline__ void slab_cols_scalar(const float* __restrict__ src, float* dst, int len, int nblk,
-                                                 int blk, int accumulate, float (*red)[64]) {
+                                                 int blk, int accumulate, float (*red)[64], int fcin, int fcout) {
   constexpr int NW = 16;
   const int lane = threadIdx.x & 63, wv = threadIdx.x >> 6;
   const int i = blk * 64 + lane;
@@ -789,12 +800,13 @@
     float v = 0.f;
 #pragma unroll
     for (int w = 0; w < NW; ++w) v += red[w][lane];
-    dst[i] = accumulate ? dst[i] + v : v;
+    const int d = fcin > 0 ? slab_frag_dst(i, fcin, fcout) : i;
+    if (d >= 0) dst[d] = accumulate ? dst[d] + v : v;
   }
 }
 
 __device__ __forceinline__ void slab_cols_vec(const float* __restrict__ src0, float* dst, int len, int nblk, int blk,
-                                              int accumulate, float4 (*red)[8]) {
+                                              int accumulate, float4 (*red)[8], int fcin, int fcout) {
   constexpr int NR = 128;
   const int c4 = threadIdx.x & 7, r = threadIdx.x >> 3;
   const int col = blk * 32 + c4 * 4;
@@ -826,7 +838,14 @@
   if (r == 0 && col < len) {
     const float4 v = red[0][c4];
     float4* d = reinterpret_cast<float4*>(dst + col);
-    if (accumulate) {
+    if (fcin > 0) {
+      const float e[4] = {v.x, v.y, v.z, v.w};
+#pragma unroll
+      for (int k = 0; k < 4; ++k) {
+        const int o = slab_frag_dst(col + k, fcin, fcout);
+        if (o >= 0) dst[o] = accumulate ? dst[o] + e[k] : e[k];
+      }
+    } else if (accumulate) {
       const float4 o = *d;
       *d = make_float4(o.x + v.x, o.y + v.y, o.z + v.z, o.w + v.w);
     } else {
@@ -842,9 +861,9 @@
   while (t + 1 < T.ntask && (int)blockIdx.x >= T.start[t + 1]) ++t;
   const int blk = (int)blockIdx.x - T.start[t];
   if (T.vec[t])
-    slab_cols_vec(T.src[t], T.dst[t], T.len[t], T.nblk[t], blk, T.accumulate, red_v);
+    slab_cols_vec(T.src[t], T.dst[t], T.len[t], T.nblk[t], blk, T.accumulate, red_v, T.cin[t], T.cout[t]);
   else
-    slab_cols_scalar(T.src[t], T.dst[t], T.len[t], T.nblk[t], blk, T.accumulate, red_s);
+    slab_cols_scalar(T.src[t], T.dst[t], T.len[t], T.nblk[t], blk, T.accumulate, red_s, T.cin[t], T.cout[t]);
 }
 
 __global__ void __launch_bounds__(256) colsum_part_k(const float* __restrict__ X, int M, int N, long long ld,
@@ -1129,6 +1148,11 @@
 
 int paig_slab_reduce_multi(int ntask, const float* const* src, const int* nblk, const int* len, float* const* dst,
                            int accumulate, void* stream) {
+  return paig_slab_reduce_multi_frag(ntask, src, nblk, len, dst, nullptr, nullptr, accumulate, stream);
+}
+
+int paig_slab_reduce_multi_frag(int ntask, const float* const* src, const int* nblk, const int* len,
+                                float* const* dst, const int* cin, const int* cout, int accumulate, void* stream) {
   PAIG_REQUIRE(ntask >= 0 && ntask <= PAIG_MAX_SLAB_TASKS, "slab_reduce_multi: %d tasks", ntask);
   if (ntask == 0) return 0;
   SlabTasks T;
@@ -1140,6 +1164,15 @@
     T.nblk[t] = nblk[t];
     T.len[t] = len[t];
     T.vec[t] = len[t] % 4 == 0 && ((uintptr_t)src[t] & 15) == 0 && ((uintptr_t)dst[t] & 15) == 0;
+    T.cin[t] = cin && cout ? cin[t] : 0;
+    T.cout[t] = cin && cout ? cout[t] : 0;
+    if (T.cin[t] > 0) {
+      const int ci = T.cin[t], co = T.cout[t];
+      PAIG_REQUIRE(ci % 4 == 0 && co > 0 && co % 8 == 0 && ((uintptr_t)src[t] & 15) == 0 &&
+                       (size_t)len[t] == paig_conv2d_bwd_slab_len(ci, co, 3, 1024),
+                   "slab_reduce_multi: task %d: %d -> %d channels, rows of %d floats", t, ci, co, len[t]);
+      T.vec[t] = (co * ci * 9 + co) % 4 == 0 && ((uintptr_t)dst[t] & 15) == 0;
+    }
     T.start[t] = blocks;
     blocks += cdiv(len[t], T.vec[t] ? 32 : 64);
   }
```
